# sloisel/MultiGridBarrier.jl

Hardware: AMD Instinct MI355X
Metric: Newton iters/sec + wall-clock to converge, 2D P2 p-Laplace L=9 (higher is better)
Workload: dtype f64

## Files before the change

include/mgbhip.h:

```cpp
#ifndef MGBHIP_H
#define MGBHIP_H

#include <stdint.h>

#ifdef __cplusplus
extern "C" {
#endif

#define MGBHIP_OK 0
#define MGBHIP_ERR_INVALID 1
#define MGBHIP_ERR_HIP 2
#define MGBHIP_ERR_NOT_SPD 3
#define MGBHIP_ERR_NONFINITE 4
#define MGBHIP_ERR_CONVERGENCE 5

#define MGBHIP_MAX_PIECES 4
#define MGBHIP_MAX_IDX 10
#define MGBHIP_MAX_LIN 4
#define MGBHIP_MAX_ND 13
#define MGBHIP_MAX_NU 4
#define MGBHIP_MAX_OPS 8

#define MGBHIP_KIND_EP 1
#define MGBHIP_KIND_LINEAR 2
// ... 64 lines not shown
    int (*early_stop_fn)(const double* z, double t, void* user);
    void* user;
} mgbhip_options;

typedef struct {
    int32_t k;
    int32_t L;
    int32_t failure_code;
    double t_final, t_elapsed;
    double solve_seconds;
    int64_t newton_iterations;
    int64_t f0_evals, f1_evals, f2_evals, factorizations;
    int32_t cap_steps;
    int64_t* its;
    double* ts;
    double* kappas;
    double* times;
    double* c_dot_Dz;
} mgbhip_core_result;

int mgbhip_create(mgbhip_ctx** ctx, int device_id, void* hip_stream );
int mgbhip_destroy(mgbhip_ctx* ctx);
const char* mgbhip_last_error(void);
const char* mgbhip_version(void);

int mgbhip_problem_create(mgbhip_ctx* ctx, const mgbhip_problem_desc* desc,
                          mgbhip_problem* share, mgbhip_problem** out);
int mgbhip_problem_destroy(mgbhip_problem* prob);
int mgbhip_problem_set_box(mgbhip_problem* prob, double b, double R);
int mgbhip_problem_set_barrier_weights(mgbhip_problem* prob, const double* bw );
int64_t mgbhip_level_size(const mgbhip_problem* prob, int32_t level);

int mgbhip_f0(mgbhip_problem* prob, int32_t level, const double* s, const double* c,
              const double* z0, double* value);
int mgbhip_f1(mgbhip_problem* prob, int32_t level, const double* s, const double* c,
              const double* z0, double* grad );
int mgbhip_f2(mgbhip_problem* prob, int32_t level, const double* s, const double* c,
              const double* z0, double* values );
int mgbhip_hessian_pattern(mgbhip_problem* prob, int32_t level, int64_t* nnz,
                           const int32_t** rowptr, const int32_t** colidx);
int mgbhip_solve(mgbhip_problem* prob, int32_t level, const double* g, double* x);
int mgbhip_set_hessian(mgbhip_problem* prob, int32_t level, const double* values );
int mgbhip_solve_newton(mgbhip_problem* prob, int32_t level, const double* g, double* x, double* lambda2);
typedef int (*mgbhip_allreduce_fn)(void* user, double* buf, int64_t count, int32_t op, int32_t on_device);
int mgbhip_problem_set_sharding(mgbhip_problem* prob, int32_t level, int64_t n_iface,
                                const int32_t* iface_cols, const double* own_mask );
int mgbhip_problem_set_collective(mgbhip_problem* prob, mgbhip_allreduce_fn allreduce, void* user,
                                  int32_t accepts_device_ptr);
int mgbhip_newton_direction(mgbhip_problem* prob, int32_t level, const double* s, const double* c,
                            const double* z0, double* x, double* lambda2, int32_t* condensed);
int mgbhip_node_barrier(mgbhip_problem* prob, const double* z, double* F , double* Dz );
int mgbhip_node_slack(mgbhip_problem* prob, const double* z, double* slack );

int mgbhip_mgb_core(mgbhip_problem* prob, double* z , const double* c ,
                    const mgbhip_options* opt, mgbhip_core_result* res);
int mgbhip_matched_t(mgbhip_problem* prob, const double* z, const double* c, double t_default,
                     double* t_out);
void mgbhip_default_options(mgbhip_options* opt, int64_t n_nodes);

typedef struct mgbhip_vec mgbhip_vec;
int mgbhip_vec_alloc(mgbhip_ctx* ctx, int64_t len, mgbhip_vec** out);
int mgbhip_vec_free(mgbhip_vec* v);
int64_t mgbhip_vec_len(const mgbhip_vec* v);
int mgbhip_vec_upload(mgbhip_vec* v, const double* host, int64_t len);
int mgbhip_vec_download(const mgbhip_vec* v, double* host, int64_t len);
int mgbhip_vec_fill(mgbhip_vec* v, double value);
int mgbhip_vec_copy(mgbhip_vec* dst, const mgbhip_vec* src);
int mgbhip_vec_axpy(double alpha, const mgbhip_vec* x, mgbhip_vec* y);
int mgbhip_vec_scale(double alpha, mgbhip_vec* x);
int mgbhip_vec_dot(const mgbhip_vec* a, const mgbhip_vec* b, double* out);
int mgbhip_vec_norm(const mgbhip_vec* a, double* out);
int mgbhip_vec_isfinite(const mgbhip_vec* a, int32_t* all_finite);
int mgbhip_f0_d(mgbhip_problem* prob, int32_t level, const mgbhip_vec* s, const mgbhip_vec* c,
                const mgbhip_vec* z0, double* value);
int mgbhip_f1_d(mgbhip_problem* prob, int32_t level, const mgbhip_vec* s, const mgbhip_vec* c,
                const mgbhip_vec* z0, mgbhip_vec* grad);
int mgbhip_f2_d(mgbhip_problem* prob, int32_t level, const mgbhip_vec* s, const mgbhip_vec* c,
                const mgbhip_vec* z0);
int mgbhip_solve_d(mgbhip_problem* prob, int32_t level, const mgbhip_vec* g, mgbhip_vec* x);
int mgbhip_prolong_add(mgbhip_problem* prob, int32_t level, const mgbhip_vec* s, mgbhip_vec* z);

int mgbhip_stage_ms(mgbhip_problem* prob, const char* stage, double* total_ms, int64_t* launches);
int mgbhip_reset_stage_timers(mgbhip_problem* prob, int enable);
int mgbhip_solver_stats(mgbhip_problem* prob, int32_t level, double* out8);
int mgbhip_solver_chain(mgbhip_problem* prob, int32_t level, double* out8);
enum { MGBHIP_PROJ_NONE = 0, MGBHIP_PROJ_LOOP = 1, MGBHIP_PROJ_STAGED = 2, MGBHIP_PROJ_MFMA = 3, MGBHIP_PROJ_ACCUMULATE = 4 };
int mgbhip_level_plan(mgbhip_problem* prob, int32_t level, int32_t* out16);
enum { MGBHIP_LAUNCH_ROW = 16 };
enum { MGBHIP_ASM_NONE = 0, MGBHIP_ASM_GATHER = 1, MGBHIP_ASM_COLUMNS = 2 };
enum { MGBHIP_B0_NA = 0, MGBHIP_B0_GATHER = 1, MGBHIP_B0_DIAG0 = 2, MGBHIP_B0_STEP0 = 3 };
enum { MGBHIP_BWD_NA = 0, MGBHIP_BWD_K8 = 1, MGBHIP_BWD_K16 = 2, MGBHIP_BWD_GENERAL = 3 };
int64_t mgbhip_solver_launches(mgbhip_problem* prob, int32_t level, int32_t* out, int64_t cap);

#define MGBHIP_INTERP_FEM1D 1
#define MGBHIP_INTERP_QK 2
#define MGBHIP_INTERP_P1 3
#define MGBHIP_INTERP_P2 4
#define MGBHIP_INTERP_SPECTRAL1D 5
#define MGBHIP_INTERP_SPECTRAL2D 6
int mgbhip_interpolate(mgbhip_ctx* ctx, int32_t family, int32_t d, int32_t k, int32_t p, int64_t N,
                       const double* x, const double* table, int32_t ncomp, const double* z, int64_t M,
                       const double* pts, double* out, int32_t* elem);
int mgbhip_interpolate_grad(mgbhip_ctx* ctx, int32_t family, int32_t d, int32_t k, int32_t p, int64_t N,
                            const double* x, const double* table, int32_t ncomp, const double* z, int64_t M,
                            const double* pts, double* out ,
                            double* grad , int32_t* elem );

typedef struct mgbhip_locator mgbhip_locator;
int mgbhip_locator_create(mgbhip_ctx* ctx, int32_t family, int32_t d, int32_t k, int32_t p, int64_t N,
                          const double* x, const double* table, int64_t M, const double* pts,
                          mgbhip_locator** out);
int mgbhip_locator_elements(const mgbhip_locator* loc, int32_t* elem );
int mgbhip_locator_evaluate(mgbhip_locator* loc, int32_t ncomp, const double* z ,
                            double* out ,
                            double* grad );
int mgbhip_locator_destroy(mgbhip_locator* loc);

typedef struct mgbhip_contour mgbhip_contour;
int mgbhip_contour_create(mgbhip_ctx* ctx, int32_t family, int32_t d, int32_t k, int32_t p, int64_t N,
                          const double* x, const double* table, int32_t nfield , const double* fields,
                          int32_t nlevels, const double* levels, int32_t refine,
                          mgbhip_contour** out, int64_t* nsimplices);
int mgbhip_contour_fetch(const mgbhip_contour* c, double* points, int32_t* level, int32_t* element,
                         double* carried );
int mgbhip_contour_destroy(mgbhip_contour* c);

int mgbhip_contour_create_embedded(mgbhip_ctx* ctx, int32_t family, int32_t d, int32_t e, int32_t k, int32_t p,
                                   int64_t N, const double* x , const double* table,
                                   int32_t nfield , const double* fields, int32_t nlevels,
                                   const double* levels, int32_t refine, mgbhip_contour** out, int64_t* nsimplices);

typedef struct mgbhip_tessellation mgbhip_tessellation;
int mgbhip_tessellate_create(mgbhip_ctx* ctx, int32_t family, int32_t d, int32_t e, int32_t k, int32_t p, int64_t N,
                             const double* x , const double* table, int32_t nfield ,
                             const double* fields, int32_t refine, mgbhip_tessellation** out, int64_t* ntriangles);
int mgbhip_tessellate_fetch(const mgbhip_tessellation* t, double* points, int32_t* element,
                            double* values );
int mgbhip_tessellate_destroy(mgbhip_tessellation* t);

typedef struct mgbhip_raycast mgbhip_raycast;
int mgbhip_raycast_create(mgbhip_ctx* ctx, int32_t family, int32_t d, int32_t k, int32_t p, int64_t N,
                          const double* x, const double* table, int64_t R, const double* origin, const double* dir,
                          const double* box, double step, double t_min, double t_max,
                          mgbhip_raycast** out, int64_t* nsamples);
int mgbhip_raycast_offsets(const mgbhip_raycast* rc, int64_t* offsets );
int mgbhip_raycast_samples(const mgbhip_raycast* rc, double* pts );
int mgbhip_raycast_lengths(const mgbhip_raycast* rc, double* step , double* length );
int mgbhip_raycast_integrate(mgbhip_raycast* rc, int32_t ncomp, const double* z ,
                             double* out );
int mgbhip_raycast_render(mgbhip_raycast* rc, const double* u , int32_t K, const double* transfer ,
                          double lo, double hi, double* out );
int mgbhip_raycast_destroy(mgbhip_raycast* rc);
int mgbhip_raycast_render_layers(mgbhip_raycast* rc, const double* u , int32_t K,
                                 const double* transfer , double lo, double hi, int32_t nhits,
                                 const double* t_hit , const double* layer ,
                                 double* out );

typedef struct mgbhip_surface mgbhip_surface;
int mgbhip_surface_create(mgbhip_ctx* ctx, int64_t T, const double* points , mgbhip_surface** out);
int mgbhip_surface_trace(mgbhip_surface* s, int64_t R, const double* origin, const double* dir, double t_min,
                         double t_max, int32_t K, double* t, int32_t* tri, double* u, double* v );
int mgbhip_surface_shade(mgbhip_surface* s, int64_t R, int32_t K, const double* dir, const int32_t* tri,
                         const double* u, const double* v, const double* values , int32_t Kt,
                         const double* table , double lo, double hi, double ambient,
                         double* layer );
int mgbhip_surface_destroy(mgbhip_surface* s);
// ... 46 lines not shown
```

multigridbarrier.jl_amd/csrc/api.cpp:

```cpp
#include <chrono>
#include <cmath>
#include <cstring>
#include <algorithm>
#include <limits>
#include <memory>
#include <string>

#include "contour.hpp"
#include "figure.hpp"
#include "interpolate.hpp"
#include "problem.hpp"
#include "raycast.hpp"
#include "stream.hpp"
#include "surface.hpp"
#include "tubes.hpp"

using namespace mgbhip;

mgbhip_problem* problem_create(mgbhip_ctx* ctx, const mgbhip_problem_desc* d, mgbhip_problem* share);
int core_run(mgbhip_problem* P, double* z, const double* c, const mgbhip_options* opt, mgbhip_core_result* res);
int matched_t_run(mgbhip_problem* P, const double* z, const double* c, double t_default, double* t_out);

#ifdef MGB_STEP_PROBE
namespace mgbhip { void mf_debug_probe(long long* out64); }
#endif

static thread_local std::string g_last_error;

struct DeviceGuard {
    int prev = -1, dev = -1;
    explicit DeviceGuard(int d) : dev(d) {
        if (dev < 0) return;
        if (hipGetDevice(&prev) != hipSuccess) prev = -1;
        if (prev != dev) MGB_HIP_CHECK(hipSetDevice(dev));
    }
    ~DeviceGuard() {
        if (dev >= 0 && prev >= 0 && prev != dev) (void)hipSetDevice(prev);
    }
};
static int dev_of(const mgbhip_ctx* c) { return c ? c->device : -1; }
static int dev_of(const mgbhip_problem* p) { return (p && p->ctx) ? p->ctx->device : -1; }
static int dev_of(const mgbhip_vec* v) { return (v && v->ctx) ? v->ctx->device : -1; }

struct mgbhip_locator {
    mgbhip_ctx* ctx = nullptr;
    Locator loc;
};
static int dev_of(const mgbhip_locator* l) { return (l && l->ctx) ? l->ctx->device : -1; }

struct mgbhip_contour {
    mgbhip_ctx* ctx = nullptr;
    Contour con;
};
static int dev_of(const mgbhip_contour* c) { return (c && c->ctx) ? c->ctx->device : -1; }

struct mgbhip_tessellation {
    mgbhip_ctx* ctx = nullptr;
    Tessellation tes;
};
static int dev_of(const mgbhip_tessellation* t) { return (t && t->ctx) ? t->ctx->device : -1; }

struct mgbhip_raycast {
    mgbhip_ctx* ctx = nullptr;
    RayCaster rc;
};
static int dev_of(const mgbhip_raycast* r) { return (r && r->ctx) ? r->ctx->device : -1; }

struct mgbhip_surface {
    mgbhip_ctx* ctx = nullptr;
    Surface sf;
};
static int dev_of(const mgbhip_surface* s) { return (s && s->ctx) ? s->ctx->device : -1; }

struct mgbhip_tubes {
    mgbhip_ctx* ctx = nullptr;
    Tubes tb;
};
static int dev_of(const mgbhip_tubes* s) { return (s && s->ctx) ? s->ctx->device : -1; }

struct mgbhip_stream {
    mgbhip_ctx* ctx = nullptr;
    StreamTracer tr;
};
static int dev_of(const mgbhip_stream* s) { return (s && s->ctx) ? s->ctx->device : -1; }

struct mgbhip_figure {
    mgbhip_ctx* ctx = nullptr;
    Figure fig;
};
static int dev_of(const mgbhip_figure* f) { return (f && f->ctx) ? f->ctx->device : -1; }

#define MGB_API_BEGIN try {
#define MGB_API_BEGIN_ON(h) try { DeviceGuard _guard(dev_of(h));
#define MGB_API_END                                   \
    }                                                 \
    catch (const InvalidArgument& e) {                \
        g_last_error = e.what();                      \
        return MGBHIP_ERR_INVALID;                    \
    }                                                 \
    catch (const HipError& e) {                       \
        g_last_error = e.what();                      \
        return MGBHIP_ERR_HIP;                        \
    }                                                 \
    catch (const std::exception& e) {                 \
// ... 476 lines not shown

int mgbhip_prolong_add(mgbhip_problem* P, int32_t level, const mgbhip_vec* s, mgbhip_vec* z) {
    MGB_API_BEGIN_ON(P)
    check_level(P, level);
    MGB_REQUIRE(s && z && s->ctx == P->ctx && z->ctx == P->ctx, "bad vector");
    const Level& Lv = P->levels[level];
    MGB_REQUIRE(s->len == Lv.m && z->len == Lv.rows, "prolong_add: length mismatch");
    launch_csr_matvec(Lv.rows, Lv.Rptr.p, Lv.Rcol.p, Lv.Rval.p, s->buf.p, z->buf.p, true, false, P->stream());
    P->touch();
    return MGBHIP_OK;
    MGB_API_END
}

static int node_map(mgbhip_problem* P, const double* z, double* F, double* Dz, int mode) {
    MGB_REQUIRE(P && z && F, "null argument");
    hipStream_t st = P->stream();
    P->d_z0.upload(z, (size_t)P->nu * P->n, st);
    ElemParams E = P->base_params(-1, nullptr, P->d_z0.p, nullptr);
    if (Dz) {
        P->d_nodeDz.ensure((size_t)P->n * P->nD);
        E.out_Dz = P->d_nodeDz.p;
    }
    launch_elem(E, mode, st);
    P->d_nodeF.download(F, (size_t)P->n, st);
    if (Dz) P->d_nodeDz.download(Dz, (size_t)P->n * P->nD, st);
    MGB_HIP_CHECK(hipStreamSynchronize(st));
    return MGBHIP_OK;
}

int mgbhip_node_barrier(mgbhip_problem* P, const double* z, double* F, double* Dz) {
    MGB_API_BEGIN_ON(P)
    return node_map(P, z, F, Dz, MODE_NODE_F);
    MGB_API_END
}

int mgbhip_node_slack(mgbhip_problem* P, const double* z, double* slack) {
    MGB_API_BEGIN_ON(P)
    return node_map(P, z, slack, nullptr, MODE_NODE_SLACK);
    MGB_API_END
}

void mgbhip_default_options(mgbhip_options* o, int64_t n_nodes) {
    const double eps = std::numeric_limits<double>::epsilon();
    o->tol = std::sqrt(eps);
    o->t = 0.1;
    o->kappa = 10.0;
    o->maxit = 10000;
    o->max_newton = (int32_t)std::ceil(std::log2(-std::log2(eps)) + 2);
    o->ls_beta = 0.5;
    o->ls_c1 = 0.1;
    o->line_search = 0;
    o->stop_lambda_tol = 0.25 / std::sqrt((double)n_nodes);
    o->stop_theta = 0.9;
    o->finalize = 1;
    o->finalize_theta = 0.9;
    o->early_stop = 0;
    o->stopping_criterion = nullptr;
    o->early_stop_fn = nullptr;
    o->user = nullptr;
}

int mgbhip_mgb_core(mgbhip_problem* P, double* z, const double* c, const mgbhip_options* opt, mgbhip_core_result* res) {
    MGB_API_BEGIN_ON(P)
    MGB_REQUIRE(P && z && c && opt && res, "null argument");
    MGB_REQUIRE(opt->tol > 0 && opt->t > 0 && opt->kappa > 1 && opt->maxit >= 1 && opt->max_newton >= 1, "bad options");
    int rc = core_run(P, z, c, opt, res);
    if (rc == MGBHIP_ERR_CONVERGENCE)
        g_last_error = res->failure_code == 2 ? "Convergence failure in mgb_solve: iteration_limit"
                                              : "Convergence failure in mgb_solve: stall";
    return rc;
    MGB_API_END
}

int mgbhip_matched_t(mgbhip_problem* P, const double* z, const double* c, double t_default, double* t_out) {
    MGB_API_BEGIN_ON(P)
    MGB_REQUIRE(P && z && c && t_out, "null argument");
    return matched_t_run(P, z, c, t_default, t_out);
    MGB_API_END
}

int mgbhip_stage_ms(mgbhip_problem* P, const char* stage, double* total_ms, int64_t* launches) {
    MGB_API_BEGIN_ON(P)
    MGB_REQUIRE(P && stage, "null argument");
    P->ctx->timers.collect();
    auto it = P->ctx->timers.recs.find(stage);
    if (total_ms) *total_ms = it == P->ctx->timers.recs.end() ? 0.0 : it->second.ms;
    if (launches) *launches = it == P->ctx->timers.recs.end() ? 0 : it->second.launches;
    return MGBHIP_OK;
    MGB_API_END
}

int mgbhip_solver_stats(mgbhip_problem* P, int32_t level, double* out) {
    MGB_API_BEGIN
    check_level(P, level);
    MGB_REQUIRE(out != nullptr, "null argument");
    const Level& L = P->levels[level];
    const MfPlan& pl = L.solver.plan;
    out[0] = (double)pl.fronts.size();
    out[1] = (double)pl.max_m;
    out[2] = (double)pl.arena_doubles;
    out[3] = (double)pl.factor_flops;
    out[4] = (double)pl.peeled;
    out[5] = pl.level_ptr.empty() ? 0.0 : (double)(pl.level_ptr.size() - 1);
    out[6] = (double)L.nnz;
    out[7] = (double)L.m;
    return MGBHIP_OK;
    MGB_API_END
}

int mgbhip_solver_chain(mgbhip_problem* P, int32_t level, double* out) {
    MGB_API_BEGIN
    check_level(P, level);
    MGB_REQUIRE(out != nullptr, "null argument");
    MGB_REQUIRE(P->levels[level].solver.analyzed, "mgbhip_solver_chain: the level has not been factored yet");
    P->levels[level].solver.chain_stats(out);
    return MGBHIP_OK;
    MGB_API_END
}

static_assert(MGBHIP_LAUNCH_ROW == mgbhip::MF_LAUNCH_ROW && MGBHIP_ASM_GATHER == mgbhip::MF_ASM_GATHER &&
              MGBHIP_ASM_COLUMNS == mgbhip::MF_ASM_COLS && MGBHIP_B0_GATHER == mgbhip::MF_B0_GATHER &&
              MGBHIP_B0_DIAG0 == mgbhip::MF_B0_DIAG0 && MGBHIP_B0_STEP0 == mgbhip::MF_B0_STEP0 && MGBHIP_BWD_K8 == mgbhip::MF_BWD_K8 &&
              MGBHIP_BWD_K16 == mgbhip::MF_BWD_K16 && MGBHIP_BWD_GENERAL == mgbhip::MF_BWD_GENERAL, "mgbhip.h and mf_launch_plan.hpp disagree");

int64_t mgbhip_solver_launches(mgbhip_problem* P, int32_t level, int32_t* out, int64_t cap) {
    int64_t count = 0;
    const int rc = [&]() -> int {
        MGB_API_BEGIN
        check_level(P, level);
        MGB_REQUIRE(cap >= 0 && (out != nullptr || cap == 0), "bad output buffer");
        MGB_REQUIRE(P->levels[level].solver.analyzed, "mgbhip_solver_launches: the level has not been factored yet");
        count = P->levels[level].solver.launches(out, cap);
        return MGBHIP_OK;
        MGB_API_END
    }();
    return rc == MGBHIP_OK ? count : -(int64_t)rc;
}

#ifdef MGB_STEP_PROBE
int mgbhip_debug_probe(long long* out64) { (void)hipDeviceSynchronize(); mgbhip::mf_debug_probe(out64); return 0; }
#endif

int mgbhip_reset_stage_timers(mgbhip_problem* P, int enable) {
    MGB_API_BEGIN_ON(P)
    MGB_REQUIRE(P, "null argument");
    P->ctx->timers.reset(enable != 0);
    return MGBHIP_OK;
    MGB_API_END
}

static void interpolate_check_geometry(InterpIn& in) {
    const int32_t family = in.family, d = in.d, k = in.k, p = in.p;
    const int64_t N = in.N;
    const double* x = in.x;
    const bool fem = family >= MGBHIP_INTERP_FEM1D && family <= MGBHIP_INTERP_P2;
    if (fem) {
        MGB_REQUIRE(x != nullptr && in.table != nullptr, "interpolate: FEM families need node coordinates and a table");
        MGB_REQUIRE(k >= 1 && k <= INTERP_MAX_DEGREE, "interpolate: element degree out of range");
    }
    switch (family) {
        case MGBHIP_INTERP_FEM1D:
            MGB_REQUIRE(d == 1 && p == k + 1, "interpolate: fem1d needs d = 1, p = k + 1");
            in.table_len = k + 1;
            for (int64_t e = 1; e < N && in.sorted; ++e) in.sorted = x[e * p] >= x[(e - 1) * p];
            break;
        case MGBHIP_INTERP_QK: {
            MGB_REQUIRE(d == 2 || d == 3, "interpolate: Q_k needs d = 2 or 3");
            int64_t s = 1;
            for (int a = 0; a < d; ++a) s *= k + 1;
            MGB_REQUIRE(p == s, "interpolate: Q_k needs p = (k + 1)^d");
            in.table_len = k + 1;
            break;
        }
        case MGBHIP_INTERP_P1:
        case MGBHIP_INTERP_P2:
            MGB_REQUIRE(d == 2, "interpolate: triangles need d = 2");
            MGB_REQUIRE(family == MGBHIP_INTERP_P1 ? p == 3 : (p == 6 || p == 7), "interpolate: bad nodes per triangle");
            in.table_len = (int64_t)p * 10;
            break;
        case MGBHIP_INTERP_SPECTRAL1D:
            MGB_REQUIRE(d == 1 && N == 1 && k >= 0 && p == k + 1, "interpolate: spectral1d needs d = 1, N = 1, p = n");
            in.table = nullptr;
            break;
        case MGBHIP_INTERP_SPECTRAL2D:
            MGB_REQUIRE(d == 2 && N == 1 && k >= 0 && (int64_t)p == (int64_t)(k + 1) * (k + 1),
                        "interpolate: spectral2d needs d = 2, N = 1, p = n^2");
            in.table = nullptr;
            break;
        default:
            throw InvalidArgument("interpolate: unknown family");
    }
    MGB_REQUIRE((int64_t)p * N < (int64_t)INT32_MAX && in.M < (int64_t)INT32_MAX, "interpolate: sizes exceed 32-bit indexing");
}

static void interpolate_checked(mgbhip_ctx* ctx, int32_t family, int32_t d, int32_t k, int32_t p, int64_t N,
                                const double* x, const double* table, int32_t ncomp, const double* z, int64_t M,
                                const double* pts, double* out, double* grad, int32_t* elem) {
    const bool need_out = grad == nullptr;
    MGB_REQUIRE(ctx != nullptr, "null context");
    MGB_REQUIRE(N > 0, "interpolate: no elements (N = 0)");
    MGB_REQUIRE(M >= 0 && ncomp >= 1 && p >= 1, "interpolate: bad sizes");
    MGB_REQUIRE(z != nullptr && (M == 0 || (pts != nullptr && (out != nullptr || !need_out))), "null argument");
    InterpIn in;
    in.family = family; in.d = d; in.k = k; in.p = p; in.N = N; in.ncomp = ncomp; in.M = M;
    in.x = x; in.table = table; in.z = z; in.pts = pts; in.out = out; in.grad = grad; in.elem = elem;
    interpolate_check_geometry(in);
    MGB_REQUIRE(M * ncomp * (grad ? d : 1) < (int64_t)INT32_MAX, "interpolate: sizes exceed 32-bit indexing");
    interpolate_run(in, ctx->stream);
}

int mgbhip_interpolate(mgbhip_ctx* ctx, int32_t family, int32_t d, int32_t k, int32_t p, int64_t N, const double* x,
                       const double* table, int32_t ncomp, const double* z, int64_t M, const double* pts, double* out,
                       int32_t* elem) {
    MGB_API_BEGIN_ON(ctx)
    interpolate_checked(ctx, family, d, k, p, N, x, table, ncomp, z, M, pts, out, nullptr, elem);
    return MGBHIP_OK;
    MGB_API_END
}

int mgbhip_interpolate_grad(mgbhip_ctx* ctx, int32_t family, int32_t d, int32_t k, int32_t p, int64_t N,
                            const double* x, const double* table, int32_t ncomp, const double* z, int64_t M,
                            const double* pts, double* out, double* grad, int32_t* elem) {
    MGB_API_BEGIN_ON(ctx)
    MGB_REQUIRE(grad != nullptr, "interpolate_grad: null gradient array");
    interpolate_checked(ctx, family, d, k, p, N, x, table, ncomp, z, M, pts, out, grad, elem);
    return MGBHIP_OK;
    MGB_API_END
}

// ... 576 lines not shown
```

multigridbarrier.jl_amd/csrc/driver.cpp:

```cpp
#include <chrono>
#include <cstdio>
#include <cstdlib>
#include <cmath>
#include <cstring>
#include <functional>
#include <limits>

#include "problem.hpp"

using namespace mgbhip;

namespace {

constexpr double EPS = std::numeric_limits<double>::epsilon();

bool debug_on() {
    static const bool on = [] { const char* e = getenv("MGBHIP_DEBUG"); return e && e[0] == '1'; }();
    return on;
}
#define DBG(...) do { if (debug_on()) { fprintf(stderr, __VA_ARGS__); } } while (0)

struct Stop {
    double lambda_tol;
    double theta;
    int (*fn)(double, double, double, double, double, double, void*) = nullptr;
    void* user = nullptr;
    bool operator()(double ymin, double ynext, double gmin, double gnorm_next, double ndecmin, double ndec) const {
        if (fn) return fn(ymin, ynext, gmin, gnorm_next, ndecmin, ndec, user) != 0;
        const bool exact = (ynext >= ymin) && (gnorm_next >= theta * gmin);
        if (lambda_tol >= 0) return (ndec < lambda_tol) || exact;
        return exact;
    }
};

struct NewtonResult {
    int k = 0;
    bool converged = false;
    double y = 0;
};

struct VecStats { double sumsq, bad; };

VecStats vec_stats(mgbhip_problem* P, int level, const double* d_v, int64_t len) {
    hipStream_t st = P->stream();
    launch_vec_stats(d_v, len, P->d_scratch.p, P->d_scal.p + 2, st, P->own_mask(level));
    P->read_scalars(2, 2);
    if (P->sharded()) P->allreduce_host(P->pin.d + 2, 2, 0);
    return VecStats{P->pin.d[2], P->pin.d[3]};
}

double dev_dot(mgbhip_problem* P, int level, const double* a, const double* b, int64_t len) {
    hipStream_t st = P->stream();
    launch_dot(a, b, len, P->d_scratch.p, P->d_scal.p + 4, st, P->own_mask(level));
    P->read_scalars(4, 1);
    if (P->sharded()) P->allreduce_host(P->pin.d + 4, 1, 0);
    return P->pin.d[4];
}

struct NewtonCtx {
    mgbhip_problem* P;
    int level;
    const double* d_zJ;
    const double* d_c;
    int64_t m;
    double F0(const double* d_s) { return P->eval_f0(level, d_s, d_zJ, d_c); }
    void F1(const double* d_s, double* d_out, double* d_part) { P->eval_f1(level, d_s, d_zJ, d_c, d_out, P->sharded() ? d_part : nullptr); }
    const double* rhs_of_g() const { return P->sharded() ? P->d_gpart.p : P->d_g.p; }
    void F2(const double* d_s) { P->eval_f2(level, d_s, d_zJ, d_c, false, rhs_of_g()); }
};

bool trial_values(NewtonCtx& C, double& ynext, double& gnorm_next, int32_t* moved = nullptr, const double* step = nullptr) {
    mgbhip_problem* P = C.P;
    hipStream_t st = P->stream();
    const bool onfly = step && P->can_fuse_step(C.level);
    if (step) {
        ++P->step_stamp;
        if (!onfly) launch_step(P->d_x.p, P->d_nv.p, *step, P->d_xn.p, C.m, P->d_flag.p, P->step_stamp, st);
        P->touch();
        if (onfly) { P->trial_x = P->d_x.p; P->trial_dir = P->d_nv.p; P->trial_alpha = *step; }
    }
    const bool fused = !P->dense;
    static const bool fuse_restrict = [] { const char* e = getenv("MGBHIP_NO_FUSED_RESTRICT"); return !(e && e[0] == '1'); }();
    P->trial_fuse = mgbhip_problem::TrialFuse();
    if (fused && fuse_restrict) {
        P->trial_fuse.want = true;
        if (onfly) {
            P->trial_fuse.x = P->d_x.p; P->trial_fuse.n = P->d_nv.p; P->trial_fuse.s = *step; P->trial_fuse.xn = P->d_xn.p;
            P->trial_fuse.moved = P->d_flag.p; P->trial_fuse.stamp = P->step_stamp;
        }
    }
    P->eval_f01_launch(C.level, P->d_xn.p, C.d_zJ, C.d_c, P->d_gn.p, P->sharded() ? P->d_gnpart.p : nullptr, fused);
    const bool restrict_fused = P->trial_fuse.done;
    P->trial_fuse.want = false;
    if (onfly) {
        P->trial_x = nullptr; P->trial_dir = nullptr;
        if (!restrict_fused) launch_step(P->d_x.p, P->d_nv.p, *step, P->d_xn.p, C.m, P->d_flag.p, P->step_stamp, st);
    }
    const double seq = P->next_seq();
    launch_trial_finish(P->d_gn.p, C.m, P->d_scratch.p, fused ? P->d_partials.p : nullptr, elem_grid(P->p, P->N), P->d_scal.p,
                        P->d_flag.p, P->pin.dev, st, P->own_mask(C.level), seq, restrict_fused);
    P->wait_results(seq);
    P->pin.i[0] = P->pin.d[4] == (double)P->step_stamp ? 1 : 0;
    if (P->sharded()) {
        P->pin.d[1] = (double)P->pin.i[0];
        P->allreduce_host(P->pin.d, 4, 0);
        P->pin.i[0] = P->pin.d[1] != 0.0 ? 1 : 0;
    }
    if (moved) *moved = P->pin.i[0];
    ynext = P->pin.d[0];
    if (!std::isfinite(ynext)) return false;
    if (P->pin.d[3] != 0.0 || !std::isfinite(P->pin.d[2])) return false;
    gnorm_next = std::sqrt(P->pin.d[2]);
    return true;
}

bool linesearch_backtracking(NewtonCtx& C, const mgbhip_options& opt, double y, double inc, double& ynext,
                             double& gnorm_next) {
    mgbhip_problem* P = C.P;
    hipStream_t st = P->stream();
    double s = 1.0;
    bool have = false;
    while (s > 0.0) {
        double yn, gn;
        int32_t moved = 0;
        if (trial_values(C, yn, gn, &moved, &s)) {
            have = true;
            ynext = yn;
            gnorm_next = gn;
            const bool stalled = (moved == 0);
            if (stalled || yn <= y - opt.ls_c1 * inc * s) return true;
        }
        s *= opt.ls_beta;
    }
    return have;
}

bool linesearch_illinois(NewtonCtx& C, const mgbhip_options& opt, double inc, double& ynext, double& gnorm_next) {
    mgbhip_problem* P = C.P;
    hipStream_t st = P->stream();
    struct Reject {};
    auto phi = [&](double sigma) -> double {
        launch_step(P->d_x.p, P->d_nv.p, sigma, P->d_xn.p, C.m, P->d_flag.p, ++P->step_stamp, st);
        P->touch();
        const double f = C.F0(P->d_xn.p);
        if (!std::isfinite(f)) throw Reject();
        C.F1(P->d_xn.p, P->d_gn.p, P->d_gnpart.p);
        const double v = dev_dot(P, C.level, P->d_gn.p, P->d_nv.p, C.m);
        if (!std::isfinite(v)) throw Reject();
        return v;
    };
    double s = 1.0;
    bool have = false;
    while (s > 0.0) {
        try {
            double a = 0.0, b = s, fa = inc, fb = phi(s), root = b;
            bool done = false;
            if (fa == 0) { root = a; done = true; }
            else if (fa * fb >= 0) { root = b; done = true; }
            for (int it = 0; it < 10000 && !done; ++it) {
                const double c = (a * fb - b * fa) / (fb - fa);
                const double fc = phi(c);
                if (c <= std::fmin(a, b) || c >= std::fmax(a, b) || fc * fa == 0 || fc * fb == 0) { root = c; done = true; break; }
                if (fb * fc < 0) { a = b; fa = fb; } else { fa /= 2; }
                b = c; fb = fc;
            }
            if (!done) throw Reject();
            launch_step(P->d_x.p, P->d_nv.p, root, P->d_xn.p, C.m, P->d_flag.p, ++P->step_stamp, st);
        P->touch();
            double yn, gn;
            if (!trial_values(C, yn, gn)) throw Reject();
            ynext = yn;
            gnorm_next = gn;
            return true;
        } catch (Reject&) {
        }
        s *= opt.ls_beta;
    }
    return have;
}

NewtonResult newton(NewtonCtx& C, const mgbhip_options& opt, const Stop& stop, int maxit) {
    mgbhip_problem* P = C.P;
    hipStream_t st = P->stream();
    NewtonResult R;
    P->d_x.zero(st, (size_t)C.m);
    P->touch();
    double y = C.F0(P->d_x.p);
    if (!std::isfinite(y)) throw InvalidArgument("newton: initial objective value is not finite");
    double ymin = y;
    if (P->sharded()) { P->d_gpart.ensure((size_t)C.m); P->d_gnpart.ensure((size_t)C.m); }
    C.F1(P->d_x.p, P->d_g.p, P->d_gpart.p);
    VecStats gs = vec_stats(P, C.level, P->d_g.p, C.m);
    if (gs.bad != 0.0 || !std::isfinite(gs.sumsq)) throw InvalidArgument("newton: initial gradient has non-finite entries");
    double gnorm = std::sqrt(gs.sumsq);
    double gmin = gnorm;
    double incmin = INFINITY;
    int k = 0;
    bool converged = false;
    Level& L = P->levels[C.level];
    struct RobustReset {
        MfSolver& s;
        ~RobustReset() { s.robust = false; }
    } robust_reset{L.solver};
    while (k < maxit && !converged) {
        ++k;
        C.F2(P->d_x.p);
        auto t0 = std::chrono::steady_clock::now();
        int fstatus = MGBHIP_OK;
        int leaf_flag = 0;
        for (int attempt = 0; attempt < 2; ++attempt) {
            P->factor(C.level, C.rhs_of_g());
            P->trisolve_carried(C.level, P->d_nv.p);
            const double seq = P->next_seq();
            launch_dir_finish(P->d_nv.p, P->d_g.p, C.m, P->d_scratch.p, P->d_scal.p, L.solver.status_flags_rw(), P->pin.dev, st,
                              P->own_mask(C.level), seq);
            L.solver.flags_cleared();
            P->wait_results(seq);
            P->pin.i[1] = P->pin.d[5] != 0.0 ? 1 : 0;
            leaf_flag |= P->pin.d[6] != 0.0 ? 1 : 0;
            P->pin.i[2] = leaf_flag;
            fstatus = MfSolver::status_from(P->pin.i + 1, L.solver.factored_condensed);
            if (P->sharded()) {
                P->pin.d[5] = fstatus != MGBHIP_OK ? 1.0 : 0.0;
                P->allreduce_host(P->pin.d + 2, 4, 0);
                fstatus = P->pin.d[5] != 0.0 ? MGBHIP_ERR_NOT_SPD : MGBHIP_OK;
            }
            const bool at_floor = std::fabs(P->pin.d[4]) <= EPS * std::fmax(std::fabs(y), 1.0);
            const bool suspicious = fstatus != MGBHIP_OK || P->pin.d[3] != 0.0 || !std::isfinite(P->pin.d[2]) ||
                                    (!(P->pin.d[4] > 0) && !at_floor);
            if (!suspicious || attempt == 1 || !L.solver.has_inverse_path() || L.solver.robust) break;
            DBG("newton[lev %d] k=%d: direction rejected (status %d, lambda^2=%.3e): refactoring with the substitution kernels\n",
                C.level, k, fstatus, P->pin.d[4]);
            L.solver.robust = true;
            L.factored = false;
        }
        if (fstatus != MGBHIP_OK && P->lu_fallback(C.level, P->d_g.p, P->d_nv.p)) {
            DBG("newton[lev %d] k=%d: LDL' met a zero pivot; direction from the pivoted LU fallback\n", C.level, k);
            launch_dir_finish(P->d_nv.p, P->d_g.p, C.m, P->d_scratch.p, P->d_scal.p, L.solver.status_flags_rw(), P->pin.dev, st,
                              P->own_mask(C.level));
            L.solver.flags_cleared();
            MGB_HIP_CHECK(hipStreamSynchronize(st));
            fstatus = MGBHIP_OK;
        }
        P->cnt.solve_seconds += std::chrono::duration<double>(std::chrono::steady_clock::now() - t0).count();
        if (fstatus != MGBHIP_OK) {
            DBG("newton[lev %d] k=%d: Cholesky met a non-positive pivot (y=%.17g |g|=%.6e)\n", C.level, k, y, gnorm);
            converged = false;
            break;
        }
        if (P->pin.d[3] != 0.0 || !std::isfinite(P->pin.d[2])) throw InvalidArgument("newton: Newton direction has non-finite entries");
        const double inc = P->pin.d[4];
        DBG("newton[lev %d] k=%d y=%.17g |g|=%.6e lambda^2=%.6e\n", C.level, k, y, gnorm, inc);
        if (inc <= 0) {
            converged = std::fabs(inc) <= EPS * std::fmax(std::fabs(y), 1.0);
            break;
        }
        double ynext = y, gnorm_next = gnorm;
        bool moved = (opt.line_search == 1) ? linesearch_illinois(C, opt, inc, ynext, gnorm_next)
                                            : linesearch_backtracking(C, opt, y, inc, ynext, gnorm_next);
        if (!moved) {
            ynext = y;
            gnorm_next = gnorm;
// ... 248 lines not shown
```

multigridbarrier.jl_amd/csrc/kernels.hip:

```cpp
#include <hip/hip_runtime.h>

#include <algorithm>
#include <mutex>

#include "kernels.hpp"
#include "dense.hpp"

namespace mgbhip {

namespace {

template <int CTRL>
__device__ __forceinline__ double dpp_mov_f64(double v) {
    const long long b = __double_as_longlong(v);
    const int lo = __builtin_amdgcn_mov_dpp((int)(b & 0xffffffffll), CTRL, 0xF, 0xF, true);
    const int hi = __builtin_amdgcn_mov_dpp((int)(b >> 32), CTRL, 0xF, 0xF, true);
    return __longlong_as_double(((long long)hi << 32) | (unsigned int)lo);
}
__device__ __forceinline__ double z_at(const ElemParams& P, int64_t i) {
    double v = P.z0[i];
    if (P.zsel) {
        const int32_t c = P.zsel[i];
        if (c >= 0) v += P.zx ? __builtin_fma(-P.zalpha, P.zx[c], P.zs[c]) : P.zs[c];
        if (P.zout) P.zout[i] = v;
// ... 661 lines not shown
                for (int q = 0; q < P; ++q) acc -= Xus[q * P + i] * t[q];
                up[i] = acc;
            }
#pragma unroll
            for (int q = 0; q < P; ++q) bj -= Xbeta[q] * t[q];
            if (j == PB) {
                bj -= Pm.leaf_g[ld.interior];
#pragma unroll
                for (int q = 0; q < P; ++q) corner -= Xbeta[q] * Xbeta[q] * Xinv[q];
#pragma unroll
                for (int i = 0; i < P; ++i) Xc[i] = up[i];
                Xs[0] = bj;
                Xs[1] = up[PB];
            }
        }
        __builtin_amdgcn_fence(__ATOMIC_RELEASE, "wavefront");
        __builtin_amdgcn_wave_barrier();
        __builtin_amdgcn_fence(__ATOMIC_ACQUIRE, "wavefront");
        {
            const int m = (int)(ld.packed & 15u);
            const bool pk = Pm.leaf_packed != 0;
            int pos[P];
#pragma unroll
            for (int i = 0; i < P; ++i) pos[i] = (int)((ld.packed >> (4 + 4 * i)) & 15u);
            double d7 = 1.0, bb = 0.0, inv7 = 1.0, f = 0.0, xc[P];
#pragma unroll
            for (int i = 0; i < P; ++i) xc[i] = 0.0;
            if (active) {
                d7 = Xs[1];
                bb = Xs[0];
                inv7 = 1.0 / d7;
#pragma unroll
                for (int i = 0; i < P; ++i) xc[i] = Xc[i];
                f = (j < PB) ? xc[j] * inv7 : 0.0;
                bad = bad || (j == PB && ((d7 == 0.0) || !isfinite(d7)));
            }
            double* Fg = Pm.leaf_arena + ld.F_off;
            double* S = Fg;
            if (pk) {
                __syncthreads();
                S = sh + (size_t)el * 120;
            }
            auto at = [&](int rr, int cc) -> int { return pk ? cc * m - (cc * (cc - 1)) / 2 + (rr - cc) : rr + cc * m; };
            if (active) {
                S[at(j, j)] = ssj;
#pragma unroll
                for (int rr = 0; rr < P; ++rr)
                    if (rr > j) S[at(rr, j)] = 0.0;
                S[at(P, j)] = usc[PB] * inv;
#pragma unroll
                for (int i = 0; i < PB; ++i)
                    if (pos[i] != 15) S[at(pos[i], j)] = usc[i] * inv;
                S[at(m - 1, j)] = beta * inv;
                if (j == PB) {
                    S[at(P, P)] = d7;
#pragma unroll
                    for (int i = 0; i < PB; ++i)
                        if (pos[i] != 15) S[at(pos[i], P)] = xc[i] * inv7;
                    S[at(m - 1, P)] = bb * inv7;
                    S[at(m - 1, m - 1)] = corner - bb * bb * inv7;
                } else if (pos[j] != 15) {
#pragma unroll
                    for (int i = 0; i < PB; ++i)
                        if (pos[i] != 15 && pos[i] >= pos[j]) S[at(pos[i], pos[j])] = up[i] - xc[i] * f;
                    S[at(m - 1, pos[j])] = bj - bb * f;
                }
            }
            if (pk) {
                __builtin_amdgcn_fence(__ATOMIC_RELEASE, "wavefront");
                __builtin_amdgcn_wave_barrier();
                __builtin_amdgcn_fence(__ATOMIC_ACQUIRE, "wavefront");
                if (e < Pm.N) {
                    const LeafDesc l2 = Pm.leaf_desc[e];
                    const int mm = (int)(l2.packed & 15u);
                    double* dstF = Pm.leaf_arena + l2.F_off;
                    for (int t = r; t < mm * (mm + 1) / 2; t += G) dstF[t] = S[t];
                }
            }
        }
        if (bad) atomicOr(Pm.leaf_status, 1);
    }
}

template <int NY, int P, class Sig>
__global__ __launch_bounds__(256) void elem_f01_fast(const ElemParams Pm) {
    constexpr int G = (P <= 2) ? 2 : (P <= 4) ? 4 : (P <= 8) ? 8 : (P <= 16) ? 16 : (P <= 32) ? 32 : 64;
    constexpr int EPB = 256 / G;
    constexpr int PP = P * P;
    extern __shared__ double sh[];
    const int tid = threadIdx.x;
    const int el = tid / G;
    const int r = tid % G;
    const int nu = Sig::rt ? Pm.nu : 2;
    auto DST = [&](int k) -> int { return Sig::rt ? Pm.D_state[k] : Sig::state(k); };
    auto DSG = [&](int k) -> int { return Sig::rt ? Pm.D_stage[k] : Sig::stage(k); };
    const int64_t e0 = (int64_t)blockIdx.x * EPB;
    const int64_t e = e0 + el;
    const bool active = (e < Pm.N) && (r < P);
    const int64_t n = Pm.n;
    const int64_t node = e * P + r;

    double* zl = sh;
    double* opL = zl + 256 * nu;
    double* YL = opL + (size_t)Pm.nstage * EPB * PP;
    {
        int64_t lim = (Pm.N - e0) * PP;
        if (lim > (int64_t)EPB * PP) lim = (int64_t)EPB * PP;
        constexpr int NIT = (EPB * PP + 255) / 256;
        for (int o = 0; o < Pm.nstage; ++o) {
            const double* src = Pm.stage_ptr[o] + e0 * PP;
            double* dst = opL + (size_t)o * EPB * PP;
            double v[NIT];
#pragma unroll
            for (int u = 0; u < NIT; ++u) {
                const int i = tid + 256 * u;
                v[u] = i < lim ? src[i] : 0.0;
            }
#pragma unroll
            for (int u = 0; u < NIT; ++u) {
                const int i = tid + 256 * u;
                if (i < lim) dst[i] = v[u];
            }
        }
    }
    double ck[NY];
    double wv = 0.0, bwv = 0.0;
    if (active) {
        for (int a = 0; a < nu; ++a) zl[(el * nu + a) * G + r] = z_at(Pm, (int64_t)a * n + node);
#pragma unroll
        for (int k = 0; k < NY; ++k) ck[k] = Pm.c[node + n * k];
        wv = Pm.w[node];
        bwv = Pm.bw ? Pm.bw[node] : 0.0;
    }
    __syncthreads();
    const double* opE = opL + (size_t)el * PP;
    auto OP = [&](int k, int rr, int cc) -> double { return opE[(size_t)DSG(k) * EPB * PP + cc * P + rr]; };
    double y[NY];
#pragma unroll
    for (int k = 0; k < NY; ++k) {
        double v = 0.0;
        if (active) {
            const double* za = zl + (el * nu + DST(k)) * G;
            if (DSG(k) < 0) v = za[r];
            else {
#pragma unroll
                for (int cc = 0; cc < P; ++cc) v += OP(k, r, cc) * za[cc];
            }
        }
        y[k] = v;
    }
    double val = 0.0;
    if (active) {
        double F0v, F, g[NY], H[NY * NY];
        cone_eval<NY, 0>(Pm.cone, node, n, y, F0v, g, H);
        cone_eval<NY, 1>(Pm.cone, node, n, y, F, g, H);
        const double bar = Pm.bw ? ((bwv == 0.0) ? 0.0 : bwv * F0v) : Pm.invn * F0v;
        double lin = 0.0;
#pragma unroll
        for (int k = 0; k < NY; ++k) {
            lin += ck[k] * y[k];
            const double sc = Pm.bw ? ((bwv == 0.0) ? 0.0 : bwv * g[k]) : Pm.invn * g[k];
            YL[(el * NY + k) * G + r] = sc + wv * ck[k];
        }
        val = bar + wv * lin;
    }
    __syncthreads();
    if (active) {
        const int i = r;
        for (int a = 0; a < nu; ++a) {
            double acc = 0.0;
#pragma unroll
            for (int k = 0; k < NY; ++k) {
                if (DST(k) != a) continue;
                const double* Yk = YL + (el * NY + k) * G;
                if (DSG(k) < 0) {
                    acc += Yk[i];
                } else {
#pragma unroll
                    for (int rr = 0; rr < P; ++rr) acc += OP(k, rr, i) * Yk[rr];
                }
            }
            Pm.out_ret[(int64_t)a * n + node] = acc;
        }
    }
    __syncthreads();
    const double tot = block_sum_256(val, sh);
    if (tid == 0) Pm.out_partial[blockIdx.x] = tot;
}

struct DSum {
    double s = 0.0, c = 0.0;
    __device__ __forceinline__ void add(double x) {
#ifdef MGB_PLAIN_SUMS
        s += x;
        return;
#endif
        const double t = s + x;
        const double bp = t - s;
        c += (s - (t - bp)) + (x - bp);
        s = t;
    }
    __device__ __forceinline__ void merge(double s2, double c2) { add(s2); c += c2; }
    __device__ __forceinline__ double value() const { return s + c; }
};
__device__ __forceinline__ void dsum_wave_reduce(DSum& a) {
    for (int off = 32; off > 0; off >>= 1) {
        const double s2 = __shfl_down(a.s, off, 64), c2 = __shfl_down(a.c, off, 64);
        a.merge(s2, c2);
    }
}


__global__ __launch_bounds__(256) void reduce_partials_kernel(const double* __restrict__ partials, int64_t count,
                                                              double* __restrict__ out) {
    __shared__ double red[256];
    const int tid = threadIdx.x;
    double s = 0.0;
    for (int64_t i = tid; i < count; i += 256) s += partials[i];
    red[tid] = s;
    __syncthreads();
    for (int off = 128; off > 0; off >>= 1) {
        if (tid < off) red[tid] += red[tid + off];
        __syncthreads();
    }
    if (tid == 0) out[0] = red[0];
}

template <int MODE>
__global__ __launch_bounds__(256) void block_reduce_kernel(const double* __restrict__ a, const double* __restrict__ b,
                                                           int64_t n, double* __restrict__ partials,
                                                           const double* __restrict__ mask) {
    __shared__ double red[256];
    __shared__ double red2[256];
    const int tid = threadIdx.x;
    double s = 0.0, bad = 0.0;
    for (int64_t i = (int64_t)blockIdx.x * 256 + tid; i < n; i += (int64_t)gridDim.x * 256) {
        const double v = a[i];
        const double w = mask ? mask[i] : 1.0;
        if (MODE == 0) s += mask ? w * (v * b[i]) : v * b[i];
        else {
            s += mask ? w * (v * v) : v * v;
            bad += isfinite(v) ? 0.0 : 1.0;
        }
    }
    red[tid] = s;
    red2[tid] = bad;
    __syncthreads();
    for (int off = 128; off > 0; off >>= 1) {
        if (tid < off) { red[tid] += red[tid + off]; red2[tid] += red2[tid + off]; }
        __syncthreads();
    }
    if (tid == 0) {
        partials[blockIdx.x] = red[0];
        if (MODE == 1) partials[gridDim.x + blockIdx.x] = red2[0];
    }
}

__global__ __launch_bounds__(256) void restrict_trial_kernel(int64_t rows, const int32_t* __restrict__ ptr, const int32_t* __restrict__ col,
                                                             const double* __restrict__ val, const double* __restrict__ ret,
                                                             double* __restrict__ g, double* __restrict__ partials,
                                                             const double* __restrict__ x, const double* __restrict__ nn, double s,
                                                             double* __restrict__ xn, int32_t* __restrict__ moved, int32_t stamp) {
    __shared__ double red[256];
    __shared__ double red2[256];
    __shared__ int any_moved;
    const int tid = threadIdx.x;
    if (tid == 0) any_moved = 0;
    __syncthreads();
    double ss = 0.0, bad = 0.0;
    bool m = false;
    for (int64_t i = (int64_t)blockIdx.x * 256 + tid; i < rows; i += (int64_t)gridDim.x * 256) {
        double acc = 0.0;
        for (int32_t q = ptr[i]; q < ptr[i + 1]; ++q) acc += val[q] * ret[col[q]];
        g[i] = acc;
        ss += acc * acc;
        bad += isfinite(acc) ? 0.0 : 1.0;
        if (xn) {
            const double xi = x[i];
            const double v = __builtin_fma(-s, nn[i], xi);
            xn[i] = v;
            m = m || (v != xi);
        }
    }
    red[tid] = ss;
    red2[tid] = bad;
    if (m) any_moved = 1;
    __syncthreads();
    for (int off = 128; off > 0; off >>= 1) {
        if (tid < off) { red[tid] += red[tid + off]; red2[tid] += red2[tid + off]; }
        __syncthreads();
    }
    if (tid == 0) {
        partials[blockIdx.x] = red[0];
        partials[gridDim.x + blockIdx.x] = red2[0];
        if (any_moved) *moved = stamp;
    }
}

__global__ __launch_bounds__(256) void dir_stats_kernel(const double* __restrict__ v, const double* __restrict__ g, int64_t n,
                                                        double* __restrict__ partials, const double* __restrict__ mask) {
    __shared__ double red[3][256];
    const int tid = threadIdx.x;
    double s = 0.0, bad = 0.0, d = 0.0;
    for (int64_t i = (int64_t)blockIdx.x * 256 + tid; i < n; i += (int64_t)gridDim.x * 256) {
        const double x = v[i];
        const double w = mask ? mask[i] : 1.0;
        s += mask ? w * (x * x) : x * x;
        bad += isfinite(x) ? 0.0 : 1.0;
        d += mask ? w * (g[i] * x) : g[i] * x;
    }
    red[0][tid] = s; red[1][tid] = bad; red[2][tid] = d;
    __syncthreads();
    for (int off = 128; off > 0; off >>= 1) {
        if (tid < off) {
            red[0][tid] += red[0][tid + off];
            red[1][tid] += red[1][tid + off];
            red[2][tid] += red[2][tid + off];
        }
        __syncthreads();
    }
    if (tid == 0) {
        partials[blockIdx.x] = red[0][0];
        partials[gridDim.x + blockIdx.x] = red[1][0];
        partials[2 * gridDim.x + blockIdx.x] = red[2][0];
    }
}

struct FinishJob { const double* src; int64_t count; int32_t out; };
struct FinishParams {
    FinishJob job[4];
    int32_t njobs;
    double* out;
    int32_t* ints;
    int32_t nints, ints_out, reset;
    double* host;
    int32_t host_lo, host_n;
    double seq;
};
__global__ __launch_bounds__(256) void finish_kernel(const FinishParams P) {
    __shared__ double red[256];
    __shared__ double res[16];
    const int tid = threadIdx.x;
    if (tid < P.nints) {
        res[P.ints_out + tid] = (double)P.ints[tid];
        if (P.reset) P.ints[tid] = 0;
    }
    for (int o = 0; o < P.njobs; ++o) {
        const double* __restrict__ src = P.job[o].src;
        const int64_t cnt = P.job[o].count;
        double s = 0.0;
        for (int64_t i = tid; i < cnt; i += 256) s += src[i];
        red[tid] = s;
        __syncthreads();
        for (int off = 128; off > 0; off >>= 1) {
            if (tid < off) red[tid] += red[tid + off];
            __syncthreads();
        }
        if (tid == 0) res[P.job[o].out] = red[0];
        __syncthreads();
    }
    __syncthreads();
    if (tid < 16) {
        bool mine = false;
        for (int o = 0; o < P.njobs; ++o) mine = mine || (P.job[o].out == tid);
        if (tid >= P.ints_out && tid < P.ints_out + P.nints) mine = true;
        if (mine) P.out[tid] = res[tid];
        if (P.host && tid >= P.host_lo && tid < P.host_lo + P.host_n) P.host[tid] = mine ? res[tid] : P.out[tid];
    }
    if (P.host && P.seq != 0.0) {
        __threadfence_system();
        __syncthreads();
        if (tid == 0) {
            __hip_atomic_store(P.host + 15, P.seq, __ATOMIC_RELEASE, __HIP_MEMORY_SCOPE_SYSTEM);
        }
    }
}


template <bool ADD>
__global__ __launch_bounds__(256) void csr_matvec_row_kernel(int64_t rows, const int32_t* __restrict__ ptr,
                                                             const int32_t* __restrict__ col,
                                                             const double* __restrict__ val,
                                                             const double* __restrict__ x, double* __restrict__ y) {
    const int64_t i = (int64_t)blockIdx.x * 256 + threadIdx.x;
    if (i >= rows) return;
    double s = 0.0;
    for (int32_t q = ptr[i]; q < ptr[i + 1]; ++q) s += val[q] * x[col[q]];
    y[i] = ADD ? y[i] + s : s;
}

template <bool ADD>
__global__ __launch_bounds__(256) void csr_matvec_wave_kernel(int64_t rows, const int32_t* __restrict__ ptr,
                                                              const int32_t* __restrict__ col,
                                                              const double* __restrict__ val,
                                                              const double* __restrict__ x, double* __restrict__ y) {
    const int lane = threadIdx.x & 63;
    const int64_t i = (int64_t)blockIdx.x * 4 + (threadIdx.x >> 6);
    if (i >= rows) return;
    DSum a;
    for (int32_t q = ptr[i] + lane; q < ptr[i + 1]; q += 64) a.add(val[q] * x[col[q]]);
    dsum_wave_reduce(a);
    if (lane == 0) y[i] = ADD ? y[i] + a.value() : a.value();
}

constexpr int CHUNK = 4096;
__global__ __launch_bounds__(256) void csr_matvec_chunk_kernel(const int32_t* __restrict__ ptr,
                                                               const int32_t* __restrict__ col,
                                                               const double* __restrict__ val,
                                                               const double* __restrict__ x,
                                                               double* __restrict__ partial, int nchunk) {
    __shared__ double red[256];
    const int row = blockIdx.y, ch = blockIdx.x, tid = threadIdx.x;
    const int32_t q0 = ptr[row] + ch * CHUNK;
    const int32_t q1 = min(ptr[row + 1], q0 + CHUNK);
    __shared__ double redc[256];
    DSum a;
    for (int32_t q = q0 + tid; q < q1; q += 256) a.add(val[q] * x[col[q]]);
    red[tid] = a.s;
    redc[tid] = a.c;
    __syncthreads();
    for (int off = 128; off > 0; off >>= 1) {
        if (tid < off) {
            DSum b;
            b.s = red[tid]; b.c = redc[tid];
            b.merge(red[tid + off], redc[tid + off]);
            red[tid] = b.s; redc[tid] = b.c;
        }
        __syncthreads();
    }
    if (tid == 0) {
        partial[2 * ((int64_t)row * nchunk + ch)] = red[0];
        partial[2 * ((int64_t)row * nchunk + ch) + 1] = redc[0];
    }
}

__global__ __launch_bounds__(256) void csr_matvec_chunk_sum_kernel(int64_t rows, const double* __restrict__ partial,
                                                                   int nchunk, double* __restrict__ y) {
    const int lane = threadIdx.x & 63;
    const int64_t i = (int64_t)blockIdx.x * 4 + (threadIdx.x >> 6);
    if (i >= rows) return;
    DSum a;
    for (int c = lane; c < nchunk; c += 64) a.merge(partial[2 * (i * nchunk + c)], partial[2 * (i * nchunk + c) + 1]);
    dsum_wave_reduce(a);
    if (lane == 0) y[i] = a.value();
}

__global__ __launch_bounds__(256) void prolong_kernel(int64_t rows, const int32_t* __restrict__ ptr,
                                                      const int32_t* __restrict__ col,
                                                      const double* __restrict__ val,
                                                      const double* __restrict__ s, const double* __restrict__ z0,
                                                      double* __restrict__ zfull) {
    const int64_t i = (int64_t)blockIdx.x * 256 + threadIdx.x;
    if (i >= rows) return;
    double v = z0[i];
    for (int32_t q = ptr[i]; q < ptr[i + 1]; ++q) v += val[q] * s[col[q]];
    zfull[i] = v;
}

__global__ __launch_bounds__(256) void step_kernel(const double* __restrict__ x, const double* __restrict__ nn,
                                                   double s, double* __restrict__ xn, int64_t len,
                                                   int32_t* __restrict__ moved, int32_t stamp) {
    const int64_t i = (int64_t)blockIdx.x * 256 + threadIdx.x;
    bool m = false;
    if (i < len) {
        const double xi = x[i];
        const double v = __builtin_fma(-s, nn[i], xi);
        xn[i] = v;
        m = (v != xi);
    }
    __shared__ int any_moved;
    if (threadIdx.x == 0) any_moved = 0;
    __syncthreads();
    if (m) any_moved = 1;
    __syncthreads();
    if (threadIdx.x == 0 && any_moved) *moved = stamp;
}

__global__ __launch_bounds__(256) void scale_copy_kernel(const double* __restrict__ src, double alpha,
                                                         double* __restrict__ dst, int64_t len) {
    const int64_t i = (int64_t)blockIdx.x * 256 + threadIdx.x;
    if (i < len) dst[i] = alpha * src[i];
}

__global__ __launch_bounds__(256) void border_tail_kernel(const double* __restrict__ g, double* __restrict__ tail, int64_t m) {
    const int64_t i = (int64_t)blockIdx.x * 256 + threadIdx.x;
    if (i < m) tail[i] = -1.0 * g[i];
    else if (i == m) tail[i] = -1.0;
}

__global__ __launch_bounds__(256) void axpy_kernel(double alpha, const double* __restrict__ x,
                                                   double* __restrict__ y, int64_t len) {
    const int64_t i = (int64_t)blockIdx.x * 256 + threadIdx.x;
    if (i < len) y[i] += alpha * x[i];
}

__global__ __launch_bounds__(256) void fill_kernel(double value, double* __restrict__ y, int64_t len) {
    const int64_t i = (int64_t)blockIdx.x * 256 + threadIdx.x;
    if (i < len) y[i] = value;
}


__global__ __launch_bounds__(256) void gather_assemble_kernel(int64_t nq, const int32_t* __restrict__ qmap,
                                                              const int32_t* __restrict__ cptr,
                                                              const int32_t* __restrict__ cidx,
                                                              const double* __restrict__ slab,
                                                              double* __restrict__ Hval) {
    const int64_t qi = (int64_t)blockIdx.x * 256 + threadIdx.x;
    if (qi >= nq) return;
    const int64_t q = qmap ? qmap[qi] : qi;
    const int32_t beg = cptr[q], end = cptr[q + 1];
    if (end - beg <= 4) {
        double s = 0.0;
        for (int32_t t = beg; t < end; ++t) s += slab[cidx ? cidx[t] : t];
        Hval[q] = s;
        return;
    }
    DSum a;
    for (int32_t t = beg; t < end; ++t) a.add(slab[cidx ? cidx[t] : t]);
    Hval[q] = a.value();
}

__global__ __launch_bounds__(256) void gather_shared_kernel(int64_t nshared, const int32_t* __restrict__ sh_q,
                                                            const int32_t* __restrict__ cptr, const int32_t* __restrict__ cidx,
                                                            const double* __restrict__ slab, double* __restrict__ out) {
    const int64_t i = (int64_t)blockIdx.x * 256 + threadIdx.x;
    if (i >= nshared) return;
    const int32_t q = sh_q[i];
    const int32_t beg = cptr[q], end = cptr[q + 1];
    if (end - beg <= 4) {
        double a[4];
#pragma unroll
        for (int u = 0; u < 4; ++u) a[u] = (beg + u < end) ? slab[cidx[beg + u]] : 0.0;
        double s = 0.0;
#pragma unroll
        for (int u = 0; u < 4; ++u)
            if (beg + u < end) s += a[u];
        out[i] = s;
        return;
    }
    DSum acc;
    for (int32_t t = beg; t < end; t += 4) {
        double a[4];
#pragma unroll
        for (int u = 0; u < 4; ++u) a[u] = (t + u < end) ? slab[cidx[t + u]] : 0.0;
#pragma unroll
        for (int u = 0; u < 4; ++u)
            if (t + u < end) acc.add(a[u]);
    }
    out[i] = acc.value();
}

// ... 436 lines not shown
    (void)hipFuncSetAttribute((const void*)elem_kernel<NY, MODE_F01>, hipFuncAttributeMaxDynamicSharedMemorySize, big);
    (void)hipGetLastError();
}

}

int elem_group(int p) {
    int g = 1;
    while (g < p) g <<= 1;
    return g < 2 ? 2 : g;
}

int64_t elem_grid(int p, int64_t N) {
    if (p > 64) return dense_grid((int64_t)p * N);
    const int epb = 256 / elem_group(p);
    return (N + epb - 1) / epb;
}

size_t elem_lds_bytes(const ElemParams& P, int mode) {
    const int G = elem_group(P.p);
    const int EPB = 256 / G;
    size_t d = 256 * (size_t)P.nu + (size_t)P.nstage * EPB * P.p * P.p;
    if (mode == MODE_F1 || mode == MODE_F01) d += 256 * (size_t)P.nD;
    if (mode == MODE_F2) d += 256 * (size_t)(P.nD * (P.nD + 1) / 2);
    if (d < 256) d = 256;
    return d * sizeof(double);
}

template <int NY>
static bool is_default_signature(const ElemParams& P) {
    if (P.nu != 2 || P.nD != NY || P.ymask != (((1 << NY) - 1) & ~1)) return false;
    for (int k = 0; k < NY; ++k) {
        if (P.D_state[k] != (k == NY - 1 ? 1 : 0)) return false;
        if (P.D_stage[k] != ((k == 0 || k == NY - 1) ? -1 : k - 1)) return false;
    }
    return true;
}

template <int NY, int PN>
static bool try_f2_fast(const ElemParams& P, hipStream_t st) {
    if (P.nD != NY || P.p != PN) return false;
    for (int k = 0; k < NY; ++k)
        if (P.D_stage[k] == -2) return false;
    const int G = elem_group(PN);
    const int EPB = 256 / G;
    const size_t lds = (256 * (size_t)P.nu + (size_t)P.nstage * EPB * PN * PN + (size_t)EPB * (NY * (NY + 1) / 2) * G) *
                       sizeof(double);
    if (lds > 160 * 1024) return false;
    static bool attr = [] {
        (void)hipFuncSetAttribute((const void*)elem_f2_fast<NY, PN, SigRuntime>, hipFuncAttributeMaxDynamicSharedMemorySize, 160 * 1024);
        (void)hipFuncSetAttribute((const void*)elem_f2_fast<NY, PN, SigDefault<NY>>, hipFuncAttributeMaxDynamicSharedMemorySize, 160 * 1024);
        (void)hipGetLastError();
        return true;
    }();
    (void)attr;
    if (is_default_signature<NY>(P))
        hipLaunchKernelGGL((elem_f2_fast<NY, PN, SigDefault<NY>>), dim3((unsigned)elem_grid(PN, P.N)), dim3(256), lds, st, P);
    else
        hipLaunchKernelGGL((elem_f2_fast<NY, PN, SigRuntime>), dim3((unsigned)elem_grid(PN, P.N)), dim3(256), lds, st, P);
    return true;
}

bool launch_elem_f2_condense(const ElemParams& P, hipStream_t st) {
    constexpr int NY = 4, PN = 7;
    if (P.wide || P.nD != NY || P.p != PN || P.nu != 2 || P.nstage != 2 || !is_default_signature<NY>(P)) return false;
    for (int k = 0; k < NY; ++k)
        if (P.D_stage[k] == -2) return false;
    MGB_REQUIRE(P.leaf_desc && P.leaf_arena && P.leaf_g && P.leaf_status, "condensing f2: leaf arguments missing");
    const int G = elem_group(PN);
    const int EPB = 256 / G;
    const size_t lds = (256 * (size_t)P.nu + (size_t)P.nstage * EPB * PN * PN + (size_t)EPB * (NY * (NY + 1) / 2) * G) * sizeof(double);
    static bool attr = [] {
        (void)hipFuncSetAttribute((const void*)elem_f2_fast<NY, PN, SigDefault<NY>, true>, hipFuncAttributeMaxDynamicSharedMemorySize, 160 * 1024);
        (void)hipGetLastError();
        return true;
    }();
    (void)attr;
    hipLaunchKernelGGL((elem_f2_fast<NY, PN, SigDefault<NY>, true>), dim3((unsigned)elem_grid(PN, P.N)), dim3(256), lds, st, P);
    MGB_HIP_CHECK(hipGetLastError());
    return true;
}

template <int NY, int PN>
static bool try_f01_fast(const ElemParams& P, hipStream_t st) {
    if (P.nD != NY || P.p != PN) return false;
    for (int k = 0; k < NY; ++k)
        if (P.D_stage[k] == -2) return false;
    const int G = elem_group(PN);
    const int EPB = 256 / G;
    size_t lds = (256 * (size_t)P.nu + (size_t)P.nstage * EPB * PN * PN + (size_t)EPB * NY * G) * sizeof(double);
    if (lds < 256 * sizeof(double)) lds = 256 * sizeof(double);
    if (lds > 160 * 1024) return false;
    static bool attr = [] {
        (void)hipFuncSetAttribute((const void*)elem_f01_fast<NY, PN, SigRuntime>, hipFuncAttributeMaxDynamicSharedMemorySize, 160 * 1024);
        (void)hipFuncSetAttribute((const void*)elem_f01_fast<NY, PN, SigDefault<NY>>, hipFuncAttributeMaxDynamicSharedMemorySize, 160 * 1024);
        (void)hipGetLastError();
        return true;
    }();
    (void)attr;
    if (is_default_signature<NY>(P))
        hipLaunchKernelGGL((elem_f01_fast<NY, PN, SigDefault<NY>>), dim3((unsigned)elem_grid(PN, P.N)), dim3(256), lds, st, P);
    else
        hipLaunchKernelGGL((elem_f01_fast<NY, PN, SigRuntime>), dim3((unsigned)elem_grid(PN, P.N)), dim3(256), lds, st, P);
    return true;
}

size_t wide_lds_bytes(int p, int nu, int nD, int nstage, int mode) {
    const int G = elem_group(p);
    const int threads = (mode == MODE_F2) ? WIDE_F2_THREADS : 256;
    const int EPB = threads / G;
    size_t d = (size_t)threads * nu + (size_t)nstage * EPB * p * p;
    if (mode == MODE_F1 || mode == MODE_F01) d += (size_t)threads * nD;
    if (mode == MODE_F2) d += (size_t)threads * (nD * (nD + 1) / 2);
    if (d < 256) d = 256;
    return d * sizeof(double);
}

static void launch_elem_wide(const ElemParams& P, int mode, hipStream_t st) {
    static std::once_flag once;
    std::call_once(once, [] {
        const int big = 160 * 1024;
        (void)hipFuncSetAttribute((const void*)elem_wide_kernel<MODE_F0>, hipFuncAttributeMaxDynamicSharedMemorySize, big);
        (void)hipFuncSetAttribute((const void*)elem_wide_kernel<MODE_F1>, hipFuncAttributeMaxDynamicSharedMemorySize, big);
        (void)hipFuncSetAttribute((const void*)elem_wide_kernel<MODE_F2>, hipFuncAttributeMaxDynamicSharedMemorySize, big);
        (void)hipFuncSetAttribute((const void*)elem_wide_kernel<MODE_NODE_F>, hipFuncAttributeMaxDynamicSharedMemorySize, big);
        (void)hipFuncSetAttribute((const void*)elem_wide_kernel<MODE_NODE_SLACK>, hipFuncAttributeMaxDynamicSharedMemorySize, big);
        (void)hipFuncSetAttribute((const void*)elem_wide_kernel<MODE_F01>, hipFuncAttributeMaxDynamicSharedMemorySize, big);
        (void)hipGetLastError();
    });
    const int G = elem_group(P.p);
    int lgG = 0;
    while ((1 << lgG) < G) ++lgG;
    const int threads = (mode == MODE_F2) ? WIDE_F2_THREADS : 256;
    const int EPB = threads / G;
    const dim3 grid((unsigned)((P.N + EPB - 1) / EPB)), blk((unsigned)threads);
    const size_t lds = wide_lds_bytes(P.p, P.nu, P.nD, P.nstage, mode);
    MGB_REQUIRE(lds <= 160 * 1024, "wide element kernel LDS budget exceeded");
    switch (mode) {
        case MODE_F0: hipLaunchKernelGGL((elem_wide_kernel<MODE_F0>), grid, blk, lds, st, P, lgG); break;
        case MODE_F1: hipLaunchKernelGGL((elem_wide_kernel<MODE_F1>), grid, blk, lds, st, P, lgG); break;
        case MODE_F2: hipLaunchKernelGGL((elem_wide_kernel<MODE_F2>), grid, blk, lds, st, P, lgG); break;
        case MODE_NODE_F: hipLaunchKernelGGL((elem_wide_kernel<MODE_NODE_F>), grid, blk, lds, st, P, lgG); break;
        case MODE_NODE_SLACK: hipLaunchKernelGGL((elem_wide_kernel<MODE_NODE_SLACK>), grid, blk, lds, st, P, lgG); break;
        case MODE_F01: hipLaunchKernelGGL((elem_wide_kernel<MODE_F01>), grid, blk, lds, st, P, lgG); break;
        default: throw InvalidArgument("launch_elem: bad mode");
    }
    MGB_HIP_CHECK(hipGetLastError());
}

void launch_elem(const ElemParams& P, int mode, hipStream_t st) {
    if (P.p > 64) {
        launch_dense_eval(P, mode, st);
        return;
    }
    MGB_REQUIRE(P.p >= 1 && P.p <= 64, "element kernels support 1 <= p <= 64 nodes per element");
    MGB_REQUIRE(P.nD >= 1 && P.nD <= MGBHIP_MAX_ND, "nD out of range");
    if (P.wide) {
        launch_elem_wide(P, mode, st);
        return;
    }
    MGB_REQUIRE(P.nD <= 10, "narrow element kernels: nD out of range");
    if (mode == MODE_F2) {
        if (try_f2_fast<4, 7>(P, st) || try_f2_fast<3, 2>(P, st) || try_f2_fast<5, 8>(P, st) ||
            try_f2_fast<4, 6>(P, st) || try_f2_fast<7, 7>(P, st) || try_f2_fast<6, 2>(P, st) ||
            try_f2_fast<8, 8>(P, st) || try_f2_fast<7, 6>(P, st)) {
            MGB_HIP_CHECK(hipGetLastError());
            return;
        }
    }
    if (mode == MODE_F01) {
        if (try_f01_fast<4, 7>(P, st) || try_f01_fast<3, 2>(P, st) || try_f01_fast<5, 8>(P, st) ||
            try_f01_fast<4, 6>(P, st) || try_f01_fast<7, 7>(P, st) || try_f01_fast<6, 2>(P, st) ||
            try_f01_fast<8, 8>(P, st) || try_f01_fast<7, 6>(P, st)) {
            MGB_HIP_CHECK(hipGetLastError());
            return;
        }
    }
    static std::once_flag once;
    std::call_once(once, [] {
        set_lds_attr<1>(); set_lds_attr<2>(); set_lds_attr<3>(); set_lds_attr<4>();
        set_lds_attr<5>(); set_lds_attr<6>(); set_lds_attr<7>(); set_lds_attr<8>();
        set_lds_attr<9>(); set_lds_attr<10>();
    });
    const int G = elem_group(P.p);
    int lgG = 0;
    while ((1 << lgG) < G) ++lgG;
    const dim3 grid((unsigned)elem_grid(P.p, P.N));
    const size_t lds = elem_lds_bytes(P, mode);
    MGB_REQUIRE(lds <= 160 * 1024, "element kernel LDS budget exceeded");
    switch (P.nD) {
        case 1: launch_elem_ny<1>(P, mode, lgG, grid, lds, st); break;
        case 2: launch_elem_ny<2>(P, mode, lgG, grid, lds, st); break;
        case 3: launch_elem_ny<3>(P, mode, lgG, grid, lds, st); break;
        case 4: launch_elem_ny<4>(P, mode, lgG, grid, lds, st); break;
        case 5: launch_elem_ny<5>(P, mode, lgG, grid, lds, st); break;
        case 6: launch_elem_ny<6>(P, mode, lgG, grid, lds, st); break;
        case 7: launch_elem_ny<7>(P, mode, lgG, grid, lds, st); break;
        case 8: launch_elem_ny<8>(P, mode, lgG, grid, lds, st); break;
        case 9: launch_elem_ny<9>(P, mode, lgG, grid, lds, st); break;
        case 10: launch_elem_ny<10>(P, mode, lgG, grid, lds, st); break;
    }
    MGB_HIP_CHECK(hipGetLastError());
}

void launch_reduce_partials(const double* partials, int64_t count, double* out, hipStream_t st) {
    hipLaunchKernelGGL(reduce_partials_kernel, dim3(1), dim3(256), 0, st, partials, count, out);
    MGB_HIP_CHECK(hipGetLastError());
}


static int reduce_blocks(int64_t n) {
    int64_t b = (n + 255) / 256;
    if (b > 1024) b = 1024;
    if (b < 1) b = 1;
    return (int)b;
}

int64_t reduce_scratch_doubles(int64_t n) { return 3 * (int64_t)reduce_blocks(n); }

__global__ __launch_bounds__(256) void index_gather_kernel(const double* __restrict__ v, const int32_t* __restrict__ idx,
                                                           int64_t cnt, double* __restrict__ out) {
    const int64_t i = (int64_t)blockIdx.x * 256 + threadIdx.x;
    if (i < cnt) out[i] = v[idx[i]];
}
__global__ __launch_bounds__(256) void index_scatter_kernel(const double* __restrict__ in, const int32_t* __restrict__ idx,
                                                            int64_t cnt, double* __restrict__ v) {
    const int64_t i = (int64_t)blockIdx.x * 256 + threadIdx.x;
    if (i < cnt) v[idx[i]] = in[i];
}
void launch_index_gather(const double* v, const int32_t* idx, int64_t cnt, double* out, hipStream_t st) {
    if (cnt == 0) return;
    hipLaunchKernelGGL(index_gather_kernel, dim3((unsigned)((cnt + 255) / 256)), dim3(256), 0, st, v, idx, cnt, out);
    MGB_HIP_CHECK(hipGetLastError());
}
void launch_index_scatter(const double* in, const int32_t* idx, int64_t cnt, double* v, hipStream_t st) {
    if (cnt == 0) return;
    hipLaunchKernelGGL(index_scatter_kernel, dim3((unsigned)((cnt + 255) / 256)), dim3(256), 0, st, in, idx, cnt, v);
    MGB_HIP_CHECK(hipGetLastError());
}

static void launch_finish(const FinishParams& F, hipStream_t st) {
    hipLaunchKernelGGL(finish_kernel, dim3(1), dim3(256), 0, st, F);
    MGB_HIP_CHECK(hipGetLastError());
}

void launch_vec_stats(const double* v, int64_t n, double* scratch, double* stats, hipStream_t st, const double* mask,
                      const int32_t* ints, int nints) {
    const int nb = reduce_blocks(n);
    hipLaunchKernelGGL(block_reduce_kernel<1>, dim3(nb), dim3(256), 0, st, v, (const double*)nullptr, n, scratch, mask);
    FinishParams F{};
    F.job[0] = FinishJob{scratch, nb, 0};
    F.job[1] = FinishJob{scratch + nb, nb, 1};
    F.njobs = 2;
    F.out = stats;
    F.ints = const_cast<int32_t*>(ints); F.nints = nints; F.ints_out = 2; F.reset = 0;
    launch_finish(F, st);
}

void launch_dir_stats(const double* v, const double* g, int64_t n, double* scratch, double* stats3, hipStream_t st,
                      const double* mask, const int32_t* ints, int nints) {
    const int nb = reduce_blocks(n);
    hipLaunchKernelGGL(dir_stats_kernel, dim3(nb), dim3(256), 0, st, v, g, n, scratch, mask);
    FinishParams F{};
    F.job[0] = FinishJob{scratch, nb, 0};
    F.job[1] = FinishJob{scratch + nb, nb, 1};
    F.job[2] = FinishJob{scratch + 2 * nb, nb, 2};
    F.njobs = 3;
    F.out = stats3;
    F.ints = const_cast<int32_t*>(ints); F.nints = nints; F.ints_out = 3; F.reset = 0;
    launch_finish(F, st);
}

__global__ void publish_kernel(const double* __restrict__ src, int n, double* __restrict__ host, double* __restrict__ stamp, double seq) {
    const int tid = threadIdx.x;
    if (tid < n) host[tid] = src[tid];
    __threadfence_system();
    __syncthreads();
    if (tid == 0) __hip_atomic_store(stamp, seq, __ATOMIC_RELEASE, __HIP_MEMORY_SCOPE_SYSTEM);
}

void launch_publish(const double* src, int n, double* host_block, int host_lo, double seq, hipStream_t st) {
    hipLaunchKernelGGL(publish_kernel, dim3(1), dim3(64), 0, st, src, n, host_block + host_lo, host_block + 15, seq);
    MGB_HIP_CHECK(hipGetLastError());
}

void launch_dir_finish(const double* v, const double* g, int64_t n, double* scratch, double* scal, int32_t* status2, double* host,
                       hipStream_t st, const double* mask, double seq) {
    const int nb = reduce_blocks(n);
    hipLaunchKernelGGL(dir_stats_kernel, dim3(nb), dim3(256), 0, st, v, g, n, scratch, mask);
    FinishParams F{};
    F.job[0] = FinishJob{scratch, nb, 2};
    F.job[1] = FinishJob{scratch + nb, nb, 3};
    F.job[2] = FinishJob{scratch + 2 * nb, nb, 4};
    F.njobs = 3;
    F.out = scal;
    F.ints = status2; F.nints = 2; F.ints_out = 5; F.reset = 1;
    F.host = host; F.host_lo = 2; F.host_n = 5;
    F.seq = seq;
    launch_finish(F, st);
}

void launch_trial_finish(const double* g, int64_t n, double* scratch, const double* f0_partials, int64_t f0_count, double* scal,
                         int32_t* moved, double* host, hipStream_t st, const double* mask, double seq, bool partials_ready) {
    const int nb = reduce_blocks(n);
    if (!partials_ready) hipLaunchKernelGGL(block_reduce_kernel<1>, dim3(nb), dim3(256), 0, st, g, (const double*)nullptr, n, scratch, mask);
    FinishParams F{};
    int nj = 0;
    if (f0_partials) F.job[nj++] = FinishJob{f0_partials, f0_count, 0};
    F.job[nj++] = FinishJob{scratch, nb, 2};
    F.job[nj++] = FinishJob{scratch + nb, nb, 3};
    F.njobs = nj;
    F.out = scal;
    F.ints = moved; F.nints = 1; F.ints_out = 4; F.reset = 0;
    F.host = host; F.host_lo = 0; F.host_n = 5;
    F.seq = seq;
    launch_finish(F, st);
}

void launch_dot(const double* a, const double* b, int64_t n, double* scratch, double* out, hipStream_t st, const double* mask) {
    const int nb = reduce_blocks(n);
    hipLaunchKernelGGL(block_reduce_kernel<0>, dim3(nb), dim3(256), 0, st, a, b, n, scratch, mask);
    FinishParams F{};
    F.job[0] = FinishJob{scratch, nb, 0};
    F.njobs = 1;
    F.out = out;
    launch_finish(F, st);
}

void launch_csr_matvec(int64_t rows, const int32_t* ptr, const int32_t* col, const double* val,
                       const double* x, double* y, bool add, bool long_rows, hipStream_t st) {
    if (rows == 0) return;
    if (long_rows) {
        const dim3 grid((unsigned)((rows + 3) / 4));
        if (add) hipLaunchKernelGGL(csr_matvec_wave_kernel<true>, grid, dim3(256), 0, st, rows, ptr, col, val, x, y);
        else hipLaunchKernelGGL(csr_matvec_wave_kernel<false>, grid, dim3(256), 0, st, rows, ptr, col, val, x, y);
    } else {
        const dim3 grid((unsigned)((rows + 255) / 256));
        if (add) hipLaunchKernelGGL(csr_matvec_row_kernel<true>, grid, dim3(256), 0, st, rows, ptr, col, val, x, y);
        else hipLaunchKernelGGL(csr_matvec_row_kernel<false>, grid, dim3(256), 0, st, rows, ptr, col, val, x, y);
    }
    MGB_HIP_CHECK(hipGetLastError());
}

int csr_chunks(int64_t max_row_len) { return (int)((max_row_len + CHUNK - 1) / CHUNK); }

void launch_restrict_trial(int64_t rows, const int32_t* ptr, const int32_t* col, const double* val, const double* ret, double* g,
                            double* scratch, const double* x, const double* nn, double s, double* xn, int32_t* moved, int32_t stamp,
                            hipStream_t st) {
    if (rows == 0) return;
    const int nb = reduce_blocks(rows);
    hipLaunchKernelGGL(restrict_trial_kernel, dim3(nb), dim3(256), 0, st, rows, ptr, col, val, ret, g, scratch, x, nn, s, xn, moved, stamp);
    MGB_HIP_CHECK(hipGetLastError());
}

void launch_csr_matvec_chunked(int64_t rows, const int32_t* ptr, const int32_t* col, const double* val,
                               const double* x, double* y, double* scratch, int nchunk, hipStream_t st) {
    if (rows == 0) return;
    hipLaunchKernelGGL(csr_matvec_chunk_kernel, dim3((unsigned)nchunk, (unsigned)rows), dim3(256), 0, st, ptr, col, val, x,
                       scratch, nchunk);
    hipLaunchKernelGGL(csr_matvec_chunk_sum_kernel, dim3((unsigned)((rows + 3) / 4)), dim3(256), 0, st, rows, scratch,
                       nchunk, y);
    MGB_HIP_CHECK(hipGetLastError());
}

void launch_prolong(int64_t rows, const int32_t* ptr, const int32_t* col, const double* val, const double* s,
                    const double* z0, double* zfull, hipStream_t st) {
    if (rows == 0) return;
    hipLaunchKernelGGL(prolong_kernel, dim3((unsigned)((rows + 255) / 256)), dim3(256), 0, st, rows, ptr, col, val, s,
                       z0, zfull);
    MGB_HIP_CHECK(hipGetLastError());
}

void launch_step(const double* x, const double* n, double s, double* xn, int64_t len, int32_t* moved, int32_t stamp,
                 hipStream_t st) {
    if (len == 0) return;
    hipLaunchKernelGGL(step_kernel, dim3((unsigned)((len + 255) / 256)), dim3(256), 0, st, x, n, s, xn, len, moved, stamp);
    MGB_HIP_CHECK(hipGetLastError());
}

void launch_scale_copy(const double* src, double alpha, double* dst, int64_t len, hipStream_t st) {
    if (len == 0) return;
    hipLaunchKernelGGL(scale_copy_kernel, dim3((unsigned)((len + 255) / 256)), dim3(256), 0, st, src, alpha, dst, len);
    MGB_HIP_CHECK(hipGetLastError());
}

void launch_border_tail(const double* g, double* tail, int64_t m, hipStream_t st) {
    hipLaunchKernelGGL(border_tail_kernel, dim3((unsigned)((m + 1 + 255) / 256)), dim3(256), 0, st, g, tail, m);
    MGB_HIP_CHECK(hipGetLastError());
}

void launch_axpy(double alpha, const double* x, double* y, int64_t len, hipStream_t st) {
    if (len == 0) return;
    hipLaunchKernelGGL(axpy_kernel, dim3((unsigned)((len + 255) / 256)), dim3(256), 0, st, alpha, x, y, len);
    MGB_HIP_CHECK(hipGetLastError());
}

void launch_fill(double value, double* y, int64_t len, hipStream_t st) {
    if (len == 0) return;
    hipLaunchKernelGGL(fill_kernel, dim3((unsigned)((len + 255) / 256)), dim3(256), 0, st, value, y, len);
    MGB_HIP_CHECK(hipGetLastError());
}

void launch_gather_assemble(int64_t nnz, const int32_t* cptr, const int32_t* cidx, const double* slab,
                            double* Hval, bool long_lists, hipStream_t st, int32_t chunk, int32_t nchunk, double* part,
                            const int32_t* qmap, int64_t nq) {
    if (nnz == 0) return;
    if (!qmap) nq = nnz;
    if (nq == 0) return;
    if (long_lists && nchunk > 1) {
        hipLaunchKernelGGL(gather_assemble_chunk_kernel, dim3((unsigned)((nq * nchunk + 3) / 4)), dim3(256), 0, st, nq, qmap, chunk,
                           nchunk, cptr, cidx, slab, part);
        hipLaunchKernelGGL(gather_assemble_chunk_reduce, dim3((unsigned)((nq + 3) / 4)), dim3(256), 0, st, nq, qmap, nchunk, part, Hval);
    } else if (long_lists)
        hipLaunchKernelGGL(gather_assemble_wave_kernel, dim3((unsigned)((nq + 3) / 4)), dim3(256), 0, st, nq, qmap, cptr,
                           cidx, slab, Hval);
    else
        hipLaunchKernelGGL(gather_assemble_kernel, dim3((unsigned)((nq + 255) / 256)), dim3(256), 0, st, nq, qmap, cptr,
                           cidx, slab, Hval);
    MGB_HIP_CHECK(hipGetLastError());
}

void launch_gather_shared(int64_t nshared, const int32_t* sh_q, const int32_t* cptr, const int32_t* cidx, const double* slab,
                          double* out, hipStream_t st) {
    if (nshared == 0) return;
    hipLaunchKernelGGL(gather_shared_kernel, dim3((unsigned)((nshared + 255) / 256)), dim3(256), 0, st, nshared, sh_q, cptr, cidx,
                       slab, out);
    MGB_HIP_CHECK(hipGetLastError());
}

size_t panel_accumulate_lds(int p, int nu, int ctmax) {
    const size_t per_wave = (size_t)p * ctmax + (size_t)(nu * (nu + 1) / 2) * p * p + (size_t)nu * p * ctmax + ctmax;
    return 4 * per_wave * sizeof(double);
}

bool panel_accumulate_fits(int p, int nu, int ctmax) {
    return p * ctmax <= 4 * 256 && (nu * (nu + 1) / 2) * p * p <= 3 * 256 && ctmax <= 256;
}

size_t panel_stage_doubles(int p, int nu, int ctmax) {
    return (size_t)p * ctmax + (size_t)(nu * (nu + 1) / 2) * p * p + (size_t)nu * p * ctmax + ctmax;
}

void launch_panel_accumulate(const PanelParams& P, const int32_t* ecols, int32_t m, int32_t nstream, int32_t nsplit,
                             int32_t chunk, int32_t ctmax, double* partial, double* H, hipStream_t st) {
    if (m == 0) return;
    const size_t lds = ((size_t)chunk + panel_stage_doubles(P.p, P.nu, ctmax)) * sizeof(double);
    MGB_REQUIRE(lds <= PANEL_ACC_LDS_MAX, "coarse-level accumulator + panels exceed the LDS budget");
    MGB_REQUIRE(panel_accumulate_fits(P.p, P.nu, ctmax), "coarse-level panels exceed the register staging of the accumulation kernel");
    static std::once_flag once;
    std::call_once(once, [] {
        (void)hipFuncSetAttribute((const void*)panel_accumulate_kernel, hipFuncAttributeMaxDynamicSharedMemorySize,
                                  (int)PANEL_ACC_LDS_MAX);
        (void)hipGetLastError();
    });
    hipLaunchKernelGGL(panel_accumulate_kernel, dim3((unsigned)nstream, (unsigned)nsplit), dim3(256), lds, st, P, ecols, m,
                       ctmax, chunk, partial);
    hipLaunchKernelGGL(accumulate_reduce_kernel, dim3((unsigned)(((int64_t)m * m + 255) / 256)), dim3(256), 0, st, m,
                       nstream, partial, H);
    MGB_HIP_CHECK(hipGetLastError());
// ... 53 lines not shown
```

multigridbarrier.jl_amd/csrc/kernels.hpp:

```cpp
#pragma once
#include "common.hpp"
#include "cone.hpp"

namespace mgbhip {

enum ElemMode { MODE_F0 = 0, MODE_F1 = 1, MODE_F2 = 2, MODE_NODE_F = 3, MODE_NODE_SLACK = 4,
                MODE_F01 = 5 };

struct LeafDesc {
    int64_t F_off;
    int32_t interior;
    uint32_t packed;
};

struct ElemParams {
    int32_t p, nu, nD, nstage;
    int32_t ymask;
    int64_t N, n;
    const double* ops[MGBHIP_MAX_OPS];
    const double* stage_ptr[MGBHIP_MAX_OPS];
    int32_t D_state[MGBHIP_MAX_ND];
    int32_t D_op[MGBHIP_MAX_ND];
    int32_t D_stage[MGBHIP_MAX_ND];
    const double* w;
    const double* c;
    const double* z0;
    const double* bw;
    double invn;
    ConeDev cone;
    double* out_partial;
    double* out_ret;
    double* out_hel;
    double* out_F;
    double* out_Dz;
    int32_t diag_mask;
    int64_t blk_off[MGBHIP_MAX_NU * (MGBHIP_MAX_NU + 1) / 2];
    double* dn_Dz;
    double* dn_Y;
    const LeafDesc* leaf_desc;
    double* leaf_arena;
    const double* leaf_g;
    int64_t leaf_slack0;
    int32_t* leaf_status;
    int32_t leaf_packed;
    const int32_t* zsel;
    const double* zs;
    double* zout;
    const double* zx;
    double zalpha;
    int32_t wide;
};
static_assert(sizeof(ElemParams) <= 4096 - 64, "ElemParams must stay well inside the kernel argument limit");

bool launch_elem_f2_condense(const ElemParams& P, hipStream_t st);

inline int hel_blocks(int nu) { return nu * (nu + 1) / 2; }
inline int hel_block_index(int a, int b, int nu) { return a * nu - a * (a - 1) / 2 + (b - a); }
inline int64_t hel_layout(int nu, int64_t N, int p, int diag_mask, int64_t* off) {
    int64_t total = 0;
    for (int blk = 0; blk < hel_blocks(nu); ++blk) {
        off[blk] = total;
        total += ((diag_mask >> blk) & 1) ? N * p : N * (int64_t)p * p;
    }
    return total;
}

int elem_group(int p);
constexpr int WIDE_F2_THREADS = 128;
size_t wide_lds_bytes(int p, int nu, int nD, int nstage, int mode);
int64_t elem_grid(int p, int64_t N);
size_t elem_lds_bytes(const ElemParams& P, int mode);
void launch_elem(const ElemParams& P, int mode, hipStream_t st);

void launch_reduce_partials(const double* partials, int64_t count, double* out, hipStream_t st);
void launch_vec_stats(const double* v, int64_t n, double* scratch, double* stats, hipStream_t st, const double* mask = nullptr,
                      const int32_t* ints = nullptr, int nints = 0);
void launch_dir_stats(const double* v, const double* g, int64_t n, double* scratch, double* stats3, hipStream_t st,
                      const double* mask = nullptr, const int32_t* ints = nullptr, int nints = 0);
void launch_dot(const double* a, const double* b, int64_t n, double* scratch, double* out, hipStream_t st, const double* mask = nullptr);
void launch_restrict_trial(int64_t rows, const int32_t* ptr, const int32_t* col, const double* val, const double* ret, double* g,
                            double* scratch, const double* x, const double* nn, double s, double* xn, int32_t* moved, int32_t stamp,
                            hipStream_t st);
void launch_publish(const double* src, int n, double* host_block, int host_lo, double seq, hipStream_t st);
void launch_dir_finish(const double* v, const double* g, int64_t n, double* scratch, double* scal, int32_t* status2, double* host,
                       hipStream_t st, const double* mask = nullptr, double seq = 0.0);
void launch_trial_finish(const double* g, int64_t n, double* scratch, const double* f0_partials, int64_t f0_count, double* scal,
                         int32_t* moved, double* host, hipStream_t st, const double* mask = nullptr, double seq = 0.0,
                         bool partials_ready = false);
void launch_index_gather(const double* v, const int32_t* idx, int64_t cnt, double* out, hipStream_t st);
void launch_index_scatter(const double* in, const int32_t* idx, int64_t cnt, double* v, hipStream_t st);
int64_t reduce_scratch_doubles(int64_t n);

void launch_csr_matvec(int64_t rows, const int32_t* ptr, const int32_t* col, const double* val,
                       const double* x, double* y, bool add, bool long_rows, hipStream_t st);
int csr_chunks(int64_t max_row_len);
void launch_csr_matvec_chunked(int64_t rows, const int32_t* ptr, const int32_t* col, const double* val,
                               const double* x, double* y, double* scratch, int nchunk, hipStream_t st);
void launch_prolong(int64_t rows, const int32_t* ptr, const int32_t* col, const double* val, const double* s,
                    const double* z0, double* zfull, hipStream_t st);
void launch_step(const double* x, const double* n, double s, double* xn, int64_t len, int32_t* moved, int32_t stamp,
                 hipStream_t st);
void launch_scale_copy(const double* src, double alpha, double* dst, int64_t len, hipStream_t st);
void launch_border_tail(const double* g, double* tail, int64_t m, hipStream_t st);
void launch_axpy(double alpha, const double* x, double* y, int64_t len, hipStream_t st);
void launch_fill(double value, double* y, int64_t len, hipStream_t st);

void launch_gather_shared(int64_t nshared, const int32_t* sh_q, const int32_t* cptr, const int32_t* cidx, const double* slab,
                          double* out, hipStream_t st);
void launch_gather_assemble(int64_t nnz, const int32_t* cptr, const int32_t* cidx, const double* slab,
                            double* Hval, bool long_lists, hipStream_t st, int32_t chunk = 0, int32_t nchunk = 0,
                            double* part = nullptr, const int32_t* qmap = nullptr, int64_t nq = 0);

struct PanelParams {
    int32_t p, nu;
    int64_t N;
    const int32_t* ecol_ptr;
    const double* panels;
    const int32_t* eoff;
    const double* hel;
    double* slab;
    int32_t cmax;
    int32_t upper_only;
    const int32_t* spos;
};
bool launch_panel_project_mfma(const PanelParams& P, hipStream_t st);
void launch_invert_lists(const int32_t* cidx, int64_t total, int32_t* spos, hipStream_t st);
void launch_panel_project(const PanelParams& P, hipStream_t st);
constexpr size_t PANEL_ACC_LDS_MAX = 144 * 1024;
size_t panel_accumulate_lds(int p, int nu, int ctmax);
size_t panel_stage_doubles(int p, int nu, int ctmax);
bool panel_accumulate_fits(int p, int nu, int ctmax);
void launch_panel_accumulate(const PanelParams& P, const int32_t* ecols, int32_t m, int32_t nstream, int32_t nsplit,
                             int32_t chunk, int32_t ctmax, double* partial, double* H, hipStream_t st);
void launch_panel_project_staged(const PanelParams& P, int32_t ctmax, hipStream_t st);

}
```

multigridbarrier.jl_amd/csrc/problem.cpp:

```cpp
#include "problem.hpp"
#include "plan_device.hpp"
#include "dense.hpp"

#include <algorithm>
#include <chrono>
#include <cmath>
#include <cstdio>
#include <atomic>
#include <exception>
#include <cstdlib>
#include <string>
#include <thread>
#include <cstring>
#include <numeric>

using namespace mgbhip;

static constexpr int64_t ACC_MAX_M = 384;



static void upload_csr(const mgbhip_csr& R, Level& L, hipStream_t st) {
    MGB_REQUIRE(R.rows >= 0 && R.cols >= 0 && R.rowptr && (R.rowptr[R.rows] == 0 || (R.colidx && R.values)),
                "bad prolongation CSR");
// ... 157 lines not shown
    P->cone.npieces = C.npieces;
    P->cone.feasibility = C.feasibility;
    P->cone.NC = C.NC;
    P->cone.box_b = 1.0;
    P->cone.box_R = 1.0;
    const int ny_piece = C.feasibility ? C.NC - 1 : d->nD;
    if (C.feasibility) MGB_REQUIRE(C.NC >= 2 && C.NC <= d->nD, "phase-I wrapper: bad NC");
    for (int k = 0; k < C.npieces; ++k) {
        const mgbhip_piece& s = C.pieces[k];
        PieceDev& t = P->cone.pc[k];
        MGB_REQUIRE(s.kind == MGBHIP_KIND_EP || s.kind == MGBHIP_KIND_LINEAR, "unknown functor family");
        MGB_REQUIRE(s.ni >= 1 && s.ni <= MGBHIP_MAX_IDX, "functor index list too long for this build (MGBHIP_MAX_IDX)");
        t.kind = s.kind;
        t.ni = s.ni;
        t.nc = (s.kind == MGBHIP_KIND_EP) ? s.ni : s.nc;
        MGB_REQUIRE(t.nc >= 1, "functor constraint count must be positive");
        if (s.kind == MGBHIP_KIND_LINEAR)
            MGB_REQUIRE(s.ni <= MGBHIP_MAX_LIN && t.nc <= MGBHIP_MAX_LIN,
                        "linear piece exceeds MGBHIP_MAX_LIN (4 constraint rows on 4 indexed rows)");
        if (s.kind == MGBHIP_KIND_EP) MGB_REQUIRE(s.ni >= 2, "Euclidean power cone needs nz >= 2");
        for (int c = 0; c < MGBHIP_MAX_IDX; ++c) {
            t.idx[c] = c < s.ni ? s.idx[c] : 0;
            if (c < s.ni) MGB_REQUIRE(s.idx[c] >= 0 && s.idx[c] < ny_piece, "functor index outside the D rows");
        }
        if (!s.A) MGB_REQUIRE(t.nc == t.ni, "identity A needs a square constraint matrix");
        t.A = upload_grid(P.get(), s.A, (size_t)P->n * t.nc * t.ni);
        t.b = upload_grid(P.get(), s.b, (size_t)P->n * t.nc);
        t.p = upload_grid(P.get(), s.p, (size_t)P->n);
        t.mu = upload_grid(P.get(), s.mu, (size_t)P->n);
        t.select = upload_grid(P.get(), s.select, (size_t)P->n);
        t.p_const = s.p_const;
        t.mu_const = s.mu_const;
        if (s.kind == MGBHIP_KIND_EP && !s.p) MGB_REQUIRE(s.p_const >= 1.0, "power cone exponent must be >= 1");
    }
    if (d->barrier_weights) {
        P->bw.upload(d->barrier_weights, (size_t)P->n, st);
        P->has_bw = true;
    }
    if (dbg2) fprintf(stderr, "[mgbhip] problem_create: operators, weights and cone grids on the device after %.3f s\n", since0());
    P->levels.resize(d->L);
    for (int l = 0; l < d->L; ++l) MGB_REQUIRE(d->R[l].rows == (int64_t)P->nu * P->n, "prolongation row count must be nu*n");
    {
        std::vector<std::exception_ptr> errors((size_t)d->L);
        std::atomic<int> next{0};
        auto worker = [&] {
            (void)hipSetDevice(ctx->device);
            for (int l = next.fetch_add(1); l < d->L; l = next.fetch_add(1)) {
                try {
                    const double t0 = since0();
                    upload_csr(d->R[l], P->levels[l], st);
                    if (dbg2) fprintf(stderr, "[mgbhip] problem_create: level %d (nnz %lld) %.3f -> %.3f s\n", l,
                                      (long long)d->R[l].rowptr[d->R[l].rows], t0, since0());
                } catch (...) {
                    errors[(size_t)l] = std::current_exception();
                }
            }
        };
        const int nthreads = std::min(d->L, 8);
        std::vector<std::thread> pool;
        for (int t = 1; t < nthreads; ++t) pool.emplace_back(worker);
        worker();
        for (auto& t : pool) t.join();
        for (const auto& e : errors)
            if (e) std::rethrow_exception(e);
    }
    if (dbg2) fprintf(stderr, "[mgbhip] problem_create: %d levels uploaded after %.3f s\n", d->L, since0());
    int64_t mmax = 1;
    for (auto& L : P->levels) mmax = std::max(mmax, L.m);
    const size_t zn = (size_t)P->nu * P->n;
    P->d_z.alloc(zn);
    P->d_z0.alloc(zn);
    P->d_zfull.alloc(zn);
    P->d_c.alloc((size_t)P->n * P->nD);
    P->d_c0.alloc((size_t)P->n * P->nD);
    P->d_ret.alloc(zn);
    if (P->dense) {
        P->d_dnDz.alloc((size_t)P->n * P->nD);
        P->d_dnY.alloc((size_t)P->n * (P->nD * (P->nD + 1) / 2));
        P->d_hel.alloc(1);
    } else {
        P->hel_cap = (int64_t)P->N * hel_blocks(P->nu) * P->p * P->p;
        P->d_hel.alloc((size_t)P->hel_cap);
    }
    P->d_partials.alloc((size_t)elem_grid(P->p, P->N));
    P->d_scal.alloc(16);
    P->d_scratch.alloc((size_t)reduce_scratch_doubles(std::max<int64_t>(mmax, (int64_t)zn)));
    P->d_nodeF.alloc((size_t)P->n);
    P->d_x.alloc(mmax); P->d_g.alloc(mmax); P->d_nv.alloc(mmax + 1); P->d_xn.alloc(mmax);
    P->d_gn.alloc(mmax); P->d_tmp.alloc(std::max<size_t>(mmax, zn));
    {
        size_t tch = 1;
        for (auto& L : P->levels) tch = std::max(tch, (size_t)L.T_chunks * (size_t)L.m);
        P->d_tchunk.alloc(2 * tch);
    }
    P->d_flag.alloc(4);
    MGB_HIP_CHECK(hipStreamSynchronize(st));
    if (dbg2) fprintf(stderr, "[mgbhip] problem_create: done after %.3f s\n", since0());
    return P.release();
}


void mgbhip_problem::ensure_plan_dense(int level) {
    Level& L = levels[level];
    hipStream_t st = stream();
    const int64_t m = L.m, nn = n;
    MGB_REQUIRE(m * m < (int64_t)INT32_MAX, "dense Hessian exceeds 32-bit indexing");
    L.hHptr.resize(m + 1);
    L.hHcol.resize((size_t)(m * m));
    for (int64_t i = 0; i <= m; ++i) L.hHptr[i] = (int32_t)(i * m);
    for (int64_t i = 0; i < m; ++i)
        for (int64_t j = 0; j < m; ++j) L.hHcol[i * m + j] = (int32_t)j;
    L.nnz = m * m;
    L.Hptr.upload(L.hHptr, st);
    L.Hcol.upload(L.hHcol, st);
    L.Hval.alloc((size_t)(L.nnz + L.m + 1));
    L.selection = false;
    const int64_t ld = (int64_t)nD * nn;
    L.denseDR.alloc((size_t)std::max<int64_t>(ld * m, 1));
    L.denseW.alloc((size_t)std::max<int64_t>(ld * m, 1));
    MGB_HIP_CHECK(hipMemsetAsync(L.denseW.p, 0, sizeof(double) * (size_t)std::max<int64_t>(ld * m, 1), st));
    std::vector<DevBuf<double>> Rd(nu);
    std::vector<double> host((size_t)(nn * m));
    DevBuf<double> opT;
    opT.alloc((size_t)(nn * nn));
    for (int k = 0; k < nD; ++k) {
        const int a = D_state[k];
        if (!Rd[a].p) {
            std::fill(host.begin(), host.end(), 0.0);
            for (int64_t r = 0; r < nn; ++r) {
                const int64_t row = (int64_t)a * nn + r;
                for (int32_t q = L.hRptr[row]; q < L.hRptr[row + 1]; ++q) host[(size_t)(r + nn * L.hRcol[q])] += L.hRval[q];
            }
            Rd[a].upload(host.data(), host.size(), st);
            MGB_HIP_CHECK(hipStreamSynchronize(st));
        }
        double* dst = L.denseDR.p + (int64_t)k * nn;
        const double* op = store->ops[D_op[k]].p;
        if (m == 0) continue;
        if (store->identity[D_op[k]]) {
            MGB_HIP_CHECK(hipMemcpy2DAsync(dst, sizeof(double) * ld, Rd[a].p, sizeof(double) * nn, sizeof(double) * nn,
                                           (size_t)m, hipMemcpyDeviceToDevice, st));
        } else {
            launch_dense_transpose((int)nn, op, opT.p, st);
            launch_dense_gemm_tn((int)nn, (int)m, (int)nn, opT.p, nn, nullptr, Rd[a].p, nn, dst, ld, false, false, st);
        }
    }
    MGB_HIP_CHECK(hipStreamSynchronize(st));
    L.planned = true;
}

void mgbhip_problem::ensure_plan(int level) {
    Level& L = levels[level];
    if (L.planned) return;
    if (dense) { ensure_plan_dense(level); return; }
    const auto t_plan0 = std::chrono::steady_clock::now();
    struct PlanTimer {
        std::chrono::steady_clock::time_point t0; int level;
        ~PlanTimer() {
            if (const char* dbg = getenv("MGBHIP_DEBUG"); dbg && atoi(dbg) >= 2)
                fprintf(stderr, "[mgbhip] assembly plan level %d built in %.2f s\n", level,
                        std::chrono::duration<double>(std::chrono::steady_clock::now() - t0).count());
        }
    } plan_timer{t_plan0, level};
    hipStream_t st = stream();
    const int64_t NE = N;
    const int pp = p;
    const int64_t nn = n;
// ... 367 lines not shown

void mgbhip_problem::eval_f0_launch(int level, const double* d_s, const double* d_zz, const double* d_cc) {
    hipStream_t st = stream();
    StageScope sc(ctx->timers, level + 1 == (int)levels.size() ? "f0" : "f0_coarse");
    ElemParams E = base_params(level, d_s, d_zz, d_cc);
    launch_elem(E, MODE_F0, st);
    launch_reduce_partials(d_partials.p, elem_grid(p, N), d_scal.p, st);
    cnt.f0++;
}

double mgbhip_problem::eval_f0(int level, const double* d_s, const double* d_zz, const double* d_cc) {
    hipStream_t st = stream();
    eval_f0_launch(level, d_s, d_zz, d_cc);
    read_scalars(0, 1);
    if (sharded()) allreduce_host(pin.d, 1, 0);
    return pin.d[0];
}

void mgbhip_problem::allreduce_host(double* h, int64_t count, int op) {
    MGB_REQUIRE(coll_fn != nullptr, "no collective installed");
    if (coll_fn(coll_user, h, count, op, 0) != 0) throw mgbhip::InvalidArgument("the caller's allreduce failed");
}

void mgbhip_problem::allreduce_device(double* d, int64_t count, int op) {
    MGB_REQUIRE(coll_fn != nullptr, "no collective installed");
    hipStream_t st = stream();
    if (coll_device) {
        MGB_HIP_CHECK(hipStreamSynchronize(st));
        if (coll_fn(coll_user, d, count, op, 1) != 0) throw mgbhip::InvalidArgument("the caller's allreduce failed");
        return;
    }
    coll_host.resize((size_t)count);
    MGB_HIP_CHECK(hipMemcpyAsync(coll_host.data(), d, sizeof(double) * (size_t)count, hipMemcpyDeviceToHost, st));
    MGB_HIP_CHECK(hipStreamSynchronize(st));
    allreduce_host(coll_host.data(), count, op);
    MGB_HIP_CHECK(hipMemcpyAsync(d, coll_host.data(), sizeof(double) * (size_t)count, hipMemcpyHostToDevice, st));
    MGB_HIP_CHECK(hipStreamSynchronize(st));
}

void mgbhip_problem::reduce_interface(int level, double* d_g, double* d_part) {
    Level& L = levels[level];
    if (!L.sharded) return;
    hipStream_t st = stream();
    if (d_part) MGB_HIP_CHECK(hipMemcpyAsync(d_part, d_g, sizeof(double) * (size_t)L.m, hipMemcpyDeviceToDevice, st));
    const int64_t ni = (int64_t)L.h_iface.size();
    if (ni == 0) return;
    L.iface_buf.ensure((size_t)ni);
    launch_index_gather(d_g, L.d_iface.p, ni, L.iface_buf.p, st);
    allreduce_device(L.iface_buf.p, ni, 0);
    launch_index_scatter(L.iface_buf.p, L.d_iface.p, ni, d_g, st);
}

void mgbhip_problem::eval_f1(int level, const double* d_s, const double* d_zz, const double* d_cc, double* d_gout, double* d_part) {
    hipStream_t st = stream();
    const Level& L = levels[level];
    {
        StageScope sc(ctx->timers, level + 1 == (int)levels.size() ? "f1" : "f1_coarse");
        ElemParams E = base_params(level, d_s, d_zz, d_cc);
        launch_elem(E, MODE_F1, st);
    }
    {
        StageScope sc(ctx->timers, "restrict");
        if (L.T_chunks > 0)
            launch_csr_matvec_chunked(L.m, L.Tptr.p, L.Tcol.p, L.Tval.p, d_ret.p, d_gout, d_tchunk.p, L.T_chunks, st);
        else
            launch_csr_matvec(L.m, L.Tptr.p, L.Tcol.p, L.Tval.p, d_ret.p, d_gout, false, L.T_long, st);
    }
    if (L.sharded) reduce_interface(level, d_gout, d_part);
    cnt.f1++;
}

void mgbhip_problem::eval_f01_launch(int level, const double* d_s, const double* d_zz, const double* d_cc, double* d_gout,
                                     double* d_part, bool defer_f0_sum) {
    if (dense) {
        eval_f0_launch(level, d_s, d_zz, d_cc);
        eval_f1(level, d_s, d_zz, d_cc, d_gout, d_part);
        return;
    }
    hipStream_t st = stream();
    const Level& L = levels[level];
    {
        StageScope sc(ctx->timers, level + 1 == (int)levels.size() ? "f01" : "f01_coarse");
        ElemParams E = base_params(level, d_s, d_zz, d_cc);
        launch_elem(E, MODE_F01, st);
        if (!defer_f0_sum) launch_reduce_partials(d_partials.p, elem_grid(p, N), d_scal.p, st);
    }
    {
        StageScope sc(ctx->timers, "restrict");
        trial_fuse.done = false;
        if (trial_fuse.want && L.T_chunks == 0 && !L.T_long && !sharded()) {
            launch_restrict_trial(L.m, L.Tptr.p, L.Tcol.p, L.Tval.p, d_ret.p, d_gout, d_scratch.p, trial_fuse.x, trial_fuse.n, trial_fuse.s,
                                  trial_fuse.xn, trial_fuse.moved, trial_fuse.stamp, st);
            trial_fuse.done = true;
        } else if (L.T_chunks > 0)
            launch_csr_matvec_chunked(L.m, L.Tptr.p, L.Tcol.p, L.Tval.p, d_ret.p, d_gout, d_tchunk.p, L.T_chunks, st);
        else
            launch_csr_matvec(L.m, L.Tptr.p, L.Tcol.p, L.Tval.p, d_ret.p, d_gout, false, L.T_long, st);
    }
    if (L.sharded) reduce_interface(level, d_gout, d_part);
    cnt.f0++;
    cnt.f1++;
}

bool mgbhip_problem::try_enable_condensed(int level) {
    Level& L = levels[level];
    static const bool off = [] { const char* e = getenv("MGBHIP_NO_CONDENSE"); return e && e[0] == '1'; }();
    if (off || dense || !L.selection || !L.direct || nu != 2 || p != 7 || L.hRptr.empty()) return false;
    if (!L.solver.analyzed || !L.solver.has_direct_map()) return false;
    const int64_t slack0 = L.m - n;
    if (slack0 < 0 || L.rows != 2 * n) return false;
    std::vector<int32_t> ucol((size_t)n, -1);
    for (int64_t node = 0; node < n; ++node) {
        const int32_t b = L.hRptr[node], e = L.hRptr[node + 1];
        if (e - b > 1) return false;
        if (e - b == 1) ucol[(size_t)node] = L.hRcol[b];
        const int64_t rs = n + node;
        if (L.hRptr[rs + 1] - L.hRptr[rs] != 1 || (int64_t)L.hRcol[L.hRptr[rs]] != slack0 + node) return false;
    }
    const bool ok = L.solver.enable_condensed(N, p, ucol.data(), slack0, L.nnz, hel_cap + L.nshared, stream());
    if (const char* dbg = getenv("MGBHIP_DEBUG"); dbg && atoi(dbg) >= 2)
        fprintf(stderr, "[mgbhip] level %d: condensed leaves %s\n", level, ok ? "enabled" : "not applicable");
    return ok;
}

void mgbhip_problem::eval_f2(int level, const double* d_s, const double* d_zz, const double* d_cc, bool materialize,
                             const double* rhs) {
    ensure_plan(level);
    hipStream_t st = stream();
    Level& L = levels[level];
    int E_ymask = 0;
    if (L.condense && !materialize && rhs != nullptr && L.selection && L.direct && !dense) {
        StageScope sc(ctx->timers, level + 1 == (int)levels.size() ? "f2" : "f2_coarse");
        ElemParams E = base_params(level, d_s, d_zz, d_cc);
        E.leaf_desc = L.solver.leaf_desc();
        E.leaf_arena = L.solver.arena();
        E.leaf_g = rhs;
        E.leaf_slack0 = L.m - n;
        E.leaf_status = L.solver.leaf_status();
        E.leaf_packed = L.solver.leaves_packed() ? 1 : 0;
        if (!L.solver.leaf_flag_zero()) MGB_HIP_CHECK(hipMemsetAsync(E.leaf_status, 0, sizeof(int32_t), st));
        L.solver.leaf_flag_used();
        if (launch_elem_f2_condense(E, st)) {
            L.have_H = true;
            L.H_in_slab = true;
            L.H_condensed = true;
            L.condensed_rhs = rhs;
            hel_level = level;
            L.factored = false;
            cnt.f2++;
            return;
        }
        zf_stamp = -1;
    }
    L.H_condensed = false;
    L.proj_kernel = MGBHIP_PROJ_NONE;
    {
        StageScope sc(ctx->timers, level + 1 == (int)levels.size() ? "f2" : "f2_coarse");
        ElemParams E = base_params(level, d_s, d_zz, d_cc);
        E_ymask = E.ymask;
        E.diag_mask = (L.selection && !dense) ? diag_mask_sel : 0;
        hel_layout(nu, N, p, E.diag_mask, E.blk_off);
        launch_elem(E, MODE_F2, st);
    }
    {
        StageScope sc(ctx->timers, level + 1 == (int)levels.size() ? "assemble" : "assemble_coarse");
        if (dense) {
            int klo = nD, khi = -1;
            for (int k = 0; k < nD; ++k)
                if ((E_ymask >> k) & 1) { klo = std::min(klo, k); khi = std::max(khi, k); }
            const int64_t ld = (int64_t)nD * n;
            if (khi < klo) {
                MGB_HIP_CHECK(hipMemsetAsync(L.Hval.p, 0, sizeof(double) * (size_t)L.nnz, st));
            } else {
                launch_dense_weight(nD, klo, khi, n, L.m, ld, L.denseDR.p, d_dnY.p, L.denseW.p, st);
                launch_dense_gemm_tn((int)L.m, (int)L.m, (int)((khi - klo + 1) * n), L.denseDR.p + (int64_t)klo * n, ld,
// ... 229 lines not shown
```

multigridbarrier.jl_amd/csrc/problem.hpp:

```cpp
#pragma once
#include <mutex>
#include <memory>
#include <string>
#include <vector>

#include "../../include/mgbhip.h"
#include "common.hpp"
#include "kernels.hpp"
#include "mf_solver.hpp"

struct mgbhip_ctx {
    int device = 0;
    hipStream_t stream = nullptr;
    bool own_stream = false;
    mgbhip::StageTimers timers;
    mgbhip::DevBuf<double> vscratch, vscal;
};

struct mgbhip_vec {
    mgbhip_ctx* ctx = nullptr;
    mgbhip::DevBuf<double> buf;
    int64_t len = 0;
};

namespace mgbhip {

struct OpStore {
    std::vector<DevBuf<double>> ops;
    std::vector<bool> identity;
    DevBuf<double> w;
};

struct Level {
    int64_t rows = 0, m = 0;
    std::vector<int32_t> hRptr, hRcol;
    std::vector<double> hRval;
    DevBuf<int32_t> Rptr, Rcol, Tptr, Tcol;
    DevBuf<double> Rval, Tval;
    bool T_long = false, R_long = false;
    int32_t max_row = 0, max_col = 0;
    bool R_unit = false;
    DevBuf<int32_t> Rsel;
    int32_t T_chunks = 0;
    bool planned = false;
    bool selection = false;
    bool acc = false;
    int32_t acc_waves = 0, acc_ctmax = 0;
    int32_t acc_split = 1, acc_chunk = 0;
    DevBuf<double> acc_copies;
    std::vector<int32_t> hHptr, hHcol;
    DevBuf<int32_t> Hptr, Hcol, cptr, cidx, ecol_ptr, ecols, eoff;
    DevBuf<int32_t> spos;
    bool sorted_slab = false;
    DevBuf<double> Hval, panels, slab;
    int64_t slab_doubles = 0;
    int32_t cmax = 1;
    bool long_lists = false;
    int64_t list_total = 0;
    int32_t proj_kernel = 0;
    int32_t gather_chunk = 0, gather_nchunk = 0;
    DevBuf<double> gather_part;
    DevBuf<int32_t> upq;
    int64_t nup = 0;
    int64_t nnz = 0;
    DevBuf<double> denseDR, denseW;
    MfSolver solver;
    bool have_H = false, factored = false;
    bool direct = false;
    int64_t nshared = 0;
    DevBuf<int32_t> sh_q;
    std::vector<int32_t> h_vmap;
    bool H_in_slab = false;
    bool sharded = false;
    std::vector<int32_t> h_iface;
    DevBuf<int32_t> d_iface;
    DevBuf<double> own, iface_buf;
    bool condense_tried = false, condense = false;
    bool H_condensed = false;
    const double* condensed_rhs = nullptr;
    int border_state2 = 0;
    int border_state = 0;
};

struct Counters {
    int64_t f0 = 0, f1 = 0, f2 = 0, factor = 0, newton = 0;
    double solve_seconds = 0;
};

}

struct mgbhip_problem {
    mgbhip_ctx* ctx = nullptr;
    int32_t p = 0, nu = 0, nD = 0;
    int64_t N = 0, n = 0;
    int32_t diag_mask_sel = 0;
    bool dense = false;
    bool wide = false;
    std::shared_ptr<mgbhip::OpStore> store;
    int32_t D_state[MGBHIP_MAX_ND], D_op[MGBHIP_MAX_ND], D_stage[MGBHIP_MAX_ND];
    int32_t nstage = 0;
    const double* stage_ptr[MGBHIP_MAX_OPS];
    mgbhip::ConeDev cone;
    std::vector<mgbhip::DevBuf<double>> cone_grids;
    mgbhip::DevBuf<double> bw;
    bool has_bw = false;
    std::vector<mgbhip::Level> levels;
    std::vector<double> hx;
    int32_t xdim = 0;
    mgbhip::DevBuf<double> d_z, d_z0, d_zfull, d_c, d_ret, d_hel, d_partials, d_scal, d_scratch, d_nodeF, d_nodeDz, d_dnDz, d_dnY, d_tchunk;
    mgbhip::DevBuf<double> d_x, d_g, d_nv, d_xn, d_gn, d_tmp, d_c0;
    mgbhip::DevBuf<int32_t> d_flag;
    int32_t step_stamp = 0;
    mgbhip::PinnedBuf pin;
    mgbhip::Counters cnt;
    int64_t zstamp = 0;
    mutable int64_t zf_stamp = -1;
    mutable int zf_level = -1;
    mutable const double* zf_s = nullptr;
    mutable const double* zf_z = nullptr;
    void touch() { ++zstamp; }
    mgbhip_allreduce_fn coll_fn = nullptr;
    void* coll_user = nullptr;
    bool coll_device = false;
    bool sharded() const { return coll_fn != nullptr; }
    std::vector<double> coll_host;
    void allreduce_host(double* h, int64_t count, int op);
    void allreduce_device(double* d, int64_t count, int op);
    void reduce_interface(int level, double* d_g, double* d_part);
    const double* own_mask(int level) const { return levels[level].sharded ? levels[level].own.p : nullptr; }
    mgbhip::DevBuf<double> d_gpart, d_gnpart;

    mgbhip::ElemParams base_params(int level, const double* d_s, const double* d_zz, const double* d_cc) const;
    hipStream_t stream() const { return ctx->stream; }
    void ensure_plan(int level);
    void ensure_analysis(int level);
    void ensure_direct(int level);
    void prepare_all();
    double next_seq() { return ++result_seq; }
    void wait_results(double seq);
    const double* trial_x = nullptr;
    const double* trial_dir = nullptr;
    double trial_alpha = 0.0;
    bool can_fuse_step(int level) const;
    struct TrialFuse { bool want = false, done = false; const double* x = nullptr; const double* n = nullptr; double s = 0.0;
                       double* xn = nullptr; int32_t* moved = nullptr; int32_t stamp = 0; } trial_fuse;
    void read_scalars(int lo, int n);
    double result_seq = 0.0;
    std::mutex shared_mutex;
    bool prepared = false;
    void ensure_plan_dense(int level);
    double eval_f0(int level, const double* d_s, const double* d_zz, const double* d_cc);
    void eval_f0_launch(int level, const double* d_s, const double* d_zz, const double* d_cc);
    void eval_f1(int level, const double* d_s, const double* d_zz, const double* d_cc, double* d_gout, double* d_part = nullptr);
    void eval_f01_launch(int level, const double* d_s, const double* d_zz, const double* d_cc, double* d_gout, double* d_part = nullptr,
                         bool defer_f0_sum = false);
    void eval_f2(int level, const double* d_s, const double* d_zz, const double* d_cc, bool materialize = true,
                 const double* rhs = nullptr);
    bool try_enable_condensed(int level);
    int64_t hel_cap = 0;
    int hel_level = -1;
    void factor(int level, const double* rhs = nullptr);
    void trisolve(int level, const double* d_g, double* d_xout);
    void trisolve_carried(int level, double* d_xout_np1);
    bool lu_fallback(int level, const double* d_g, double* d_xout);
    mgbhip::DevBuf<double> d_lu;
    mgbhip::DevBuf<int32_t> d_lustat;
    int64_t lu_fallbacks = 0;
};
```

multigridbarrier.jl_amd/device.py:

```python
from __future__ import annotations

import ctypes as C
import os
import weakref
from typing import List, Optional

import numpy as np
import scipy.sparse as sp

from .blockmatrices import BlockColumn, BlockDiag
from .convex import KIND_EP, KIND_LINEAR, Convex
from .multigrid import AMG
from .problem import MGBProblem

MAX_PIECES, MAX_IDX, MAX_ND, MAX_NU, MAX_OPS = 4, 10, 13, 4, 8
MAX_LIN = 4
OK, ERR_INVALID, ERR_HIP, ERR_NOT_SPD, ERR_NONFINITE, ERR_CONVERGENCE = range(6)


class Device:
    """reference: src/device.jl:18"""


class CPUDevice(Device):
    """Marker only: the native CPU path is the reference itself (src/device.jl:25)."""


class HIPDevice(Device):
    """The MI355X backend (the reference's `CUDADevice` slot, src/device.jl:32)."""


_DEFAULT = [HIPDevice]


def default_device():
    return _DEFAULT[0]


def default_device_set(D):
    _DEFAULT[0] = D
    return D



_dp = C.POINTER(C.c_double)
_ip = C.POINTER(C.c_int32)


class _Piece(C.Structure):
    _fields_ = [("kind", C.c_int32), ("ni", C.c_int32), ("nc", C.c_int32), ("idx", C.c_int32 * MAX_IDX),
                ("A", _dp), ("b", _dp), ("p", _dp), ("mu", _dp), ("p_const", C.c_double),
                ("mu_const", C.c_double), ("select", _dp)]


class _Cone(C.Structure):
    _fields_ = [("npieces", C.c_int32), ("pieces", _Piece * MAX_PIECES), ("feasibility", C.c_int32),
                ("NC", C.c_int32)]


class _CSR(C.Structure):
    _fields_ = [("rows", C.c_int64), ("cols", C.c_int64), ("rowptr", _ip), ("colidx", _ip), ("values", _dp)]


class _Desc(C.Structure):
    _fields_ = [("p", C.c_int32), ("N", C.c_int64), ("nu", C.c_int32), ("nD", C.c_int32), ("n_ops", C.c_int32),
                ("ops", _dp * MAX_OPS), ("D_state", C.c_int32 * MAX_ND), ("D_op", C.c_int32 * MAX_ND),
                ("w", _dp), ("L", C.c_int32), ("R", C.POINTER(_CSR)), ("cone", _Cone),
                ("barrier_weights", _dp), ("x", _dp), ("dim", C.c_int32)]


class Options(C.Structure):
    _fields_ = [("tol", C.c_double), ("t", C.c_double), ("kappa", C.c_double), ("maxit", C.c_int32),
                ("max_newton", C.c_int32), ("ls_beta", C.c_double), ("ls_c1", C.c_double),
                ("line_search", C.c_int32), ("stop_lambda_tol", C.c_double), ("stop_theta", C.c_double),
                ("finalize", C.c_int32), ("finalize_theta", C.c_double), ("early_stop", C.c_int32),
                ("stopping_criterion", C.c_void_p), ("early_stop_fn", C.c_void_p), ("user", C.c_void_p)]


STOP_FN = C.CFUNCTYPE(C.c_int, C.c_double, C.c_double, C.c_double, C.c_double, C.c_double, C.c_double, C.c_void_p)
EARLY_FN = C.CFUNCTYPE(C.c_int, C.POINTER(C.c_double), C.c_double, C.c_void_p)
ALLREDUCE_FN = C.CFUNCTYPE(C.c_int, C.c_void_p, C.c_void_p, C.c_int64, C.c_int32, C.c_int32)


class _CoreResult(C.Structure):
    _fields_ = [("k", C.c_int32), ("L", C.c_int32), ("failure_code", C.c_int32), ("t_final", C.c_double),
                ("t_elapsed", C.c_double), ("solve_seconds", C.c_double), ("newton_iterations", C.c_int64),
                ("f0_evals", C.c_int64), ("f1_evals", C.c_int64), ("f2_evals", C.c_int64),
                ("factorizations", C.c_int64), ("cap_steps", C.c_int32), ("its", C.POINTER(C.c_int64)),
                ("ts", _dp), ("kappas", _dp), ("times", _dp), ("c_dot_Dz", _dp)]


EXPORTS = [
    "mgbhip_create", "mgbhip_destroy", "mgbhip_last_error", "mgbhip_version", "mgbhip_problem_create",
    "mgbhip_problem_destroy", "mgbhip_problem_set_box", "mgbhip_problem_set_barrier_weights",
    "mgbhip_level_size", "mgbhip_f0", "mgbhip_f1", "mgbhip_f2", "mgbhip_hessian_pattern", "mgbhip_solve",
    "mgbhip_set_hessian", "mgbhip_solve_newton", "mgbhip_newton_direction", "mgbhip_problem_set_sharding",
    "mgbhip_problem_set_collective",
    "mgbhip_node_barrier", "mgbhip_node_slack", "mgbhip_mgb_core", "mgbhip_matched_t",
    "mgbhip_default_options", "mgbhip_stage_ms", "mgbhip_reset_stage_timers", "mgbhip_solver_stats", "mgbhip_solver_chain",
    "mgbhip_vec_alloc", "mgbhip_vec_free", "mgbhip_vec_len", "mgbhip_vec_upload", "mgbhip_vec_download",
    "mgbhip_vec_fill", "mgbhip_vec_copy", "mgbhip_vec_axpy", "mgbhip_vec_scale", "mgbhip_vec_dot",
    "mgbhip_vec_norm", "mgbhip_vec_isfinite", "mgbhip_f0_d", "mgbhip_f1_d", "mgbhip_f2_d", "mgbhip_solve_d",
    "mgbhip_prolong_add", "mgbhip_level_plan", "mgbhip_solver_launches", "mgbhip_interpolate", "mgbhip_interpolate_grad",
    "mgbhip_locator_create", "mgbhip_locator_elements", "mgbhip_locator_evaluate", "mgbhip_locator_destroy",
    "mgbhip_contour_create", "mgbhip_contour_fetch", "mgbhip_contour_destroy", "mgbhip_contour_create_embedded",
    "mgbhip_tessellate_create", "mgbhip_tessellate_fetch", "mgbhip_tessellate_destroy",
    "mgbhip_raycast_create", "mgbhip_raycast_offsets", "mgbhip_raycast_samples", "mgbhip_raycast_lengths",
    "mgbhip_raycast_integrate", "mgbhip_raycast_render", "mgbhip_raycast_destroy", "mgbhip_raycast_render_layers",
    "mgbhip_surface_create", "mgbhip_surface_trace", "mgbhip_surface_shade", "mgbhip_surface_destroy",
    "mgbhip_stream_create", "mgbhip_stream_set_field", "mgbhip_stream_trace", "mgbhip_stream_destroy",
    "mgbhip_tubes_create", "mgbhip_tubes_trace", "mgbhip_tubes_shade", "mgbhip_tubes_destroy",
    "mgbhip_figure_create", "mgbhip_figure_render", "mgbhip_figure_render_rgba8", "mgbhip_figure_counts",
    "mgbhip_figure_destroy",
]


def library_path() -> str:
    here = os.path.dirname(os.path.abspath(__file__))
    return os.environ.get("MGBHIP_LIB") or os.path.join(here, "lib", "libmgbhip.so")


_LIB = None


def load_library():
    global _LIB
    if _LIB is not None:
        return _LIB
    path = library_path()
    if not os.path.exists(path):
        raise RuntimeError(f"{path} not found: build it with `make -C multigridbarrier.jl_amd/csrc` "
                           "(or __graft_entry__.build()); this package has no CPU fallback")
    lib = C.CDLL(path)
    lib.mgbhip_last_error.restype = C.c_char_p
    lib.mgbhip_version.restype = C.c_char_p
    lib.mgbhip_level_size.restype = C.c_int64
    lib.mgbhip_level_size.argtypes = [C.c_void_p, C.c_int32]
    lib.mgbhip_create.argtypes = [C.POINTER(C.c_void_p), C.c_int, C.c_void_p]
    lib.mgbhip_destroy.argtypes = [C.c_void_p]
    lib.mgbhip_problem_create.argtypes = [C.c_void_p, C.POINTER(_Desc), C.c_void_p, C.POINTER(C.c_void_p)]
    lib.mgbhip_problem_destroy.argtypes = [C.c_void_p]
    lib.mgbhip_problem_set_box.argtypes = [C.c_void_p, C.c_double, C.c_double]
    lib.mgbhip_problem_set_barrier_weights.argtypes = [C.c_void_p, _dp]
    for name in ("mgbhip_f0", "mgbhip_f1", "mgbhip_f2"):
        getattr(lib, name).argtypes = [C.c_void_p, C.c_int32, _dp, _dp, _dp, _dp]
    lib.mgbhip_hessian_pattern.argtypes = [C.c_void_p, C.c_int32, C.POINTER(C.c_int64), C.POINTER(_ip), C.POINTER(_ip)]
    lib.mgbhip_solve.argtypes = [C.c_void_p, C.c_int32, _dp, _dp]
    lib.mgbhip_set_hessian.argtypes = [C.c_void_p, C.c_int32, _dp]
    lib.mgbhip_solve_newton.argtypes = [C.c_void_p, C.c_int32, _dp, _dp, _dp]
    lib.mgbhip_newton_direction.argtypes = [C.c_void_p, C.c_int32, _dp, _dp, _dp, _dp, _dp, _ip]
    lib.mgbhip_problem_set_sharding.argtypes = [C.c_void_p, C.c_int32, C.c_int64, _ip, _dp]
    lib.mgbhip_problem_set_collective.argtypes = [C.c_void_p, C.c_void_p, C.c_void_p, C.c_int32]
    lib.mgbhip_node_barrier.argtypes = [C.c_void_p, _dp, _dp, _dp]
    lib.mgbhip_node_slack.argtypes = [C.c_void_p, _dp, _dp]
    lib.mgbhip_mgb_core.argtypes = [C.c_void_p, _dp, _dp, C.POINTER(Options), C.POINTER(_CoreResult)]
    lib.mgbhip_matched_t.argtypes = [C.c_void_p, _dp, _dp, C.c_double, _dp]
    lib.mgbhip_default_options.argtypes = [C.POINTER(Options), C.c_int64]
    lib.mgbhip_default_options.restype = None
    lib.mgbhip_stage_ms.argtypes = [C.c_void_p, C.c_char_p, _dp, C.POINTER(C.c_int64)]
    lib.mgbhip_reset_stage_timers.argtypes = [C.c_void_p, C.c_int]
    lib.mgbhip_solver_stats.argtypes = [C.c_void_p, C.c_int32, _dp]
    lib.mgbhip_solver_chain.argtypes = [C.c_void_p, C.c_int32, _dp]
    lib.mgbhip_level_plan.argtypes = [C.c_void_p, C.c_int32, _ip]
    lib.mgbhip_solver_launches.argtypes = [C.c_void_p, C.c_int32, _ip, C.c_int64]
    lib.mgbhip_solver_launches.restype = C.c_int64
    vp = C.c_void_p
    lib.mgbhip_vec_alloc.argtypes = [vp, C.c_int64, C.POINTER(vp)]
    lib.mgbhip_vec_free.argtypes = [vp]
    lib.mgbhip_vec_len.argtypes = [vp]
    lib.mgbhip_vec_len.restype = C.c_int64
    lib.mgbhip_vec_upload.argtypes = [vp, _dp, C.c_int64]
    lib.mgbhip_vec_download.argtypes = [vp, _dp, C.c_int64]
    lib.mgbhip_vec_fill.argtypes = [vp, C.c_double]
    lib.mgbhip_vec_copy.argtypes = [vp, vp]
    lib.mgbhip_vec_axpy.argtypes = [C.c_double, vp, vp]
    lib.mgbhip_vec_scale.argtypes = [C.c_double, vp]
    lib.mgbhip_vec_dot.argtypes = [vp, vp, _dp]
    lib.mgbhip_vec_norm.argtypes = [vp, _dp]
    lib.mgbhip_vec_isfinite.argtypes = [vp, C.POINTER(C.c_int32)]
    lib.mgbhip_f0_d.argtypes = [vp, C.c_int32, vp, vp, vp, _dp]
    lib.mgbhip_f1_d.argtypes = [vp, C.c_int32, vp, vp, vp, vp]
    lib.mgbhip_f2_d.argtypes = [vp, C.c_int32, vp, vp, vp]
    lib.mgbhip_solve_d.argtypes = [vp, C.c_int32, vp, vp]
    lib.mgbhip_prolong_add.argtypes = [vp, C.c_int32, vp, vp]
    lib.mgbhip_interpolate.argtypes = [vp, C.c_int32, C.c_int32, C.c_int32, C.c_int32, C.c_int64, _dp, _dp, C.c_int32,
                                       _dp, C.c_int64, _dp, _dp, _ip]
    lib.mgbhip_interpolate_grad.argtypes = [vp, C.c_int32, C.c_int32, C.c_int32, C.c_int32, C.c_int64, _dp, _dp,
                                            C.c_int32, _dp, C.c_int64, _dp, _dp, _dp, _ip]
    lib.mgbhip_locator_create.argtypes = [vp, C.c_int32, C.c_int32, C.c_int32, C.c_int32, C.c_int64, _dp, _dp, C.c_int64,
                                          _dp, C.POINTER(vp)]
    lib.mgbhip_locator_elements.argtypes = [vp, _ip]
    lib.mgbhip_locator_evaluate.argtypes = [vp, C.c_int32, _dp, _dp, _dp]
    lib.mgbhip_locator_destroy.argtypes = [vp]
    lib.mgbhip_contour_create.argtypes = [vp, C.c_int32, C.c_int32, C.c_int32, C.c_int32, C.c_int64, _dp, _dp, C.c_int32,
                                          _dp, C.c_int32, _dp, C.c_int32, C.POINTER(vp), C.POINTER(C.c_int64)]
    lib.mgbhip_contour_create_embedded.argtypes = [vp, C.c_int32, C.c_int32, C.c_int32, C.c_int32, C.c_int32, C.c_int64, _dp,
                                                   _dp, C.c_int32, _dp, C.c_int32, _dp, C.c_int32, C.POINTER(vp),
                                                   C.POINTER(C.c_int64)]
    lib.mgbhip_tessellate_create.argtypes = [vp, C.c_int32, C.c_int32, C.c_int32, C.c_int32, C.c_int32, C.c_int64, _dp, _dp,
                                             C.c_int32, _dp, C.c_int32, C.POINTER(vp), C.POINTER(C.c_int64)]
    lib.mgbhip_tessellate_fetch.argtypes = [vp, _dp, _ip, _dp]
    lib.mgbhip_tessellate_destroy.argtypes = [vp]
    lib.mgbhip_contour_fetch.argtypes = [vp, _dp, _ip, _ip, _dp]
    lib.mgbhip_contour_destroy.argtypes = [vp]
    lib.mgbhip_raycast_create.argtypes = [vp, C.c_int32, C.c_int32, C.c_int32, C.c_int32, C.c_int64, _dp, _dp, C.c_int64,
                                          _dp, _dp, _dp, C.c_double, C.c_double, C.c_double, C.POINTER(vp),
                                          C.POINTER(C.c_int64)]
    lib.mgbhip_raycast_offsets.argtypes = [vp, C.POINTER(C.c_int64)]
    lib.mgbhip_raycast_samples.argtypes = [vp, _dp]
    lib.mgbhip_raycast_lengths.argtypes = [vp, _dp, _dp]
    lib.mgbhip_raycast_integrate.argtypes = [vp, C.c_int32, _dp, _dp]
    lib.mgbhip_raycast_render.argtypes = [vp, _dp, C.c_int32, _dp, C.c_double, C.c_double, _dp]
    lib.mgbhip_raycast_destroy.argtypes = [vp]
    lib.mgbhip_raycast_render_layers.argtypes = [vp, _dp, C.c_int32, _dp, C.c_double, C.c_double, C.c_int32, _dp, _dp, _dp]
    lib.mgbhip_surface_create.argtypes = [vp, C.c_int64, _dp, C.POINTER(vp)]
    lib.mgbhip_surface_trace.argtypes = [vp, C.c_int64, _dp, _dp, C.c_double, C.c_double, C.c_int32, _dp, _ip, _dp, _dp]
    lib.mgbhip_surface_shade.argtypes = [vp, C.c_int64, C.c_int32, _dp, _ip, _dp, _dp, _dp, C.c_int32, _dp, C.c_double,
                                         C.c_double, C.c_double, _dp]
    lib.mgbhip_surface_destroy.argtypes = [vp]
    lib.mgbhip_tubes_create.argtypes = [vp, C.c_int64, _dp, _dp, C.POINTER(vp)]
    lib.mgbhip_tubes_trace.argtypes = [vp, C.c_int64, _dp, _dp, C.c_double, C.c_double, C.c_int32, _dp, _ip, _dp]
    lib.mgbhip_tubes_shade.argtypes = [vp, C.c_int64, C.c_int32, _dp, _dp, _dp, _ip, _dp, _dp, C.c_int32, _dp, C.c_double,
                                       C.c_double, C.c_double, _dp]
    lib.mgbhip_tubes_destroy.argtypes = [vp]
    lib.mgbhip_stream_create.argtypes = [vp, C.c_int32, C.c_int32, C.c_int32, C.c_int32, C.c_int64, _dp, _dp, C.c_int32, _dp,
                                         C.POINTER(vp)]
    lib.mgbhip_stream_set_field.argtypes = [vp, _dp]
    lib.mgbhip_stream_trace.argtypes = [vp, C.c_int64, _dp, C.c_double, C.c_int32, C.c_int32, C.c_double, _dp, _ip, _ip]
    lib.mgbhip_stream_destroy.argtypes = [vp]
    lib.mgbhip_figure_create.argtypes = [vp, C.c_int32, C.c_int32, C.c_int32, C.c_int32, C.c_int64, _dp, _dp, C.c_int64,
                                         _dp, _dp, _dp, C.c_double, C.c_int32, C.c_int32, _dp, C.c_int32, _ip, _dp,
                                         C.c_int32, _dp, _dp, C.c_double, C.c_double, C.c_double, C.c_int32,
                                         C.POINTER(vp)]
    lib.mgbhip_figure_render.argtypes = [vp, _dp, _dp]
    lib.mgbhip_figure_render_rgba8.argtypes = [vp, _dp, _dp, C.POINTER(C.c_uint8)]
    lib.mgbhip_figure_counts.argtypes = [vp, C.POINTER(C.c_int64), C.POINTER(C.c_int64)]
    lib.mgbhip_figure_destroy.argtypes = [vp]
    _LIB = lib
    return lib


class MGBHipError(RuntimeError):
    def __init__(self, status, message):
# ... 299 lines not shown

    def solve_newton(self, level: int, g, check: bool = True):
        g = _f64(g)
        x = np.empty_like(g)
        lam = C.c_double()
        status = self.lib.mgbhip_solve_newton(self.handle, level, _ptr(g), _ptr(x), C.cast(C.byref(lam), _dp))
        if check:
            _check(self.lib, status)
        return x, lam.value, status

    def newton_direction(self, level: int, s, c, z0):
        s, c, z0 = _f64(s), np.asfortranarray(c, dtype=np.float64), _f64(z0)
        x = np.empty(self.level_sizes[level])
        lam, cond = C.c_double(), C.c_int32()
        _check(self.lib, self.lib.mgbhip_newton_direction(self.handle, level, _ptr(s), _ptr(c), _ptr(z0), _ptr(x),
                                                          C.cast(C.byref(lam), _dp), C.byref(cond)))
        return x, lam.value, bool(cond.value)

    def node_barrier(self, z, want_Dz: bool = False):
        z = _f64(z)
        F = np.empty(self.n)
        Dz = np.empty((self.n, self.nD), order="F") if want_Dz else None
        _check(self.lib, self.lib.mgbhip_node_barrier(self.handle, _ptr(z), _ptr(F), _ptr(Dz)))
        return (F, Dz) if want_Dz else F

    def node_slack(self, z) -> np.ndarray:
        z = _f64(z)
        out = np.empty(self.n)
        _check(self.lib, self.lib.mgbhip_node_slack(self.handle, _ptr(z), _ptr(out)))
        return out

    def set_sharding(self, shards, collective, accepts_device_ptr: bool = False):
        for level, sh in enumerate(shards):
            ic = np.ascontiguousarray(sh.iface, dtype=np.int32)
            own = _f64(sh.own)
            _check(self.lib, self.lib.mgbhip_problem_set_sharding(self.handle, level, ic.size, ic.ctypes.data_as(_ip), _ptr(own)))
        self._collective = collective
        _check(self.lib, self.lib.mgbhip_problem_set_collective(self.handle, C.cast(collective, C.c_void_p), None,
                                                               1 if accepts_device_ptr else 0))

    def set_box(self, b: float, R: float):
        _check(self.lib, self.lib.mgbhip_problem_set_box(self.handle, float(b), float(R)))

    def set_barrier_weights(self, bw):
        a = None if bw is None else _f64(bw)
        _check(self.lib, self.lib.mgbhip_problem_set_barrier_weights(self.handle, _ptr(a)))

    def default_options(self, n_nodes: Optional[int] = None) -> Options:
        o = Options()
        self.lib.mgbhip_default_options(C.byref(o), int(self.n if n_nodes is None else n_nodes))
        return o

    def mgb_core(self, z, c, opt: Options, cap_steps: int = 256):
        z = _f64(z).copy()
        c = np.asfortranarray(c, dtype=np.float64)
        L = len(self.level_sizes)
        its = np.zeros((L, cap_steps), dtype=np.int64, order="F")
        ts, kappas, times, cdz = (np.zeros(cap_steps) for _ in range(4))
        r = _CoreResult()
        r.cap_steps = cap_steps
        r.its = its.ctypes.data_as(C.POINTER(C.c_int64))
        r.ts, r.kappas, r.times, r.c_dot_Dz = _ptr(ts), _ptr(kappas), _ptr(times), _ptr(cdz)
        status = self.lib.mgbhip_mgb_core(self.handle, _ptr(z), _ptr(c), C.byref(opt), C.byref(r))
        if status not in (OK, ERR_CONVERGENCE):
            _check(self.lib, status)
        k = min(r.k, cap_steps)
        diag = dict(its=its[:, :k].copy(), ts=ts[:k].copy(), kappas=kappas[:k].copy(), times=times[:k].copy(),
                    c_dot_Dz=cdz[:k].copy(), t_elapsed=r.t_elapsed, t_final=r.t_final,
                    solve_seconds=r.solve_seconds, newton_iterations=int(r.newton_iterations),
                    f0_evals=int(r.f0_evals), f1_evals=int(r.f1_evals), f2_evals=int(r.f2_evals),
                    factorizations=int(r.factorizations), failure_code=int(r.failure_code), k=int(r.k))
        return status, z, diag

    def matched_t(self, z, c, t_default: float) -> float:
        z = _f64(z)
        c = np.asfortranarray(c, dtype=np.float64)
        out = C.c_double()
        _check(self.lib, self.lib.mgbhip_matched_t(self.handle, _ptr(z), _ptr(c), float(t_default), C.cast(C.byref(out), _dp)))
        return out.value

    def reset_stage_timers(self, enable: bool = True):
        _check(self.lib, self.lib.mgbhip_reset_stage_timers(self.handle, 1 if enable else 0))

    def stage_ms(self, stage: str):
        ms, cnt = C.c_double(), C.c_int64()
        _check(self.lib, self.lib.mgbhip_stage_ms(self.handle, stage.encode(), C.cast(C.byref(ms), _dp), C.byref(cnt)))
        return ms.value, cnt.value

    def solver_stats(self, level: int) -> dict:
        out = np.zeros(8)
        _check(self.lib, self.lib.mgbhip_solver_stats(self.handle, level, _ptr(out)))
        keys = ("fronts", "max_front", "arena_doubles", "factor_flops", "peeled", "tree_levels", "nnz", "unknowns")
        return dict(zip(keys, out.tolist()))

    def solver_chain(self, level: int) -> dict:
        out = np.zeros(8)
        _check(self.lib, self.lib.mgbhip_solver_chain(self.handle, level, _ptr(out)))
        keys = ("pivot_blocks_on_critical_path", "large_front_tree_levels", "launches_per_factorization",
                "launches_per_backward_sweep", "arena_doubles", "factor_flops", "extra_trailing_doubles", "reserved")
        return dict(zip(keys, out.tolist()))

    PLAN_KEYS = ("R_unit", "R_long", "T_long", "T_chunks", "selection", "acc", "acc_split", "long_lists", "gather_chunk",
                 "gather_nchunk", "projection", "max_row", "max_col", "cmax", "mean_list", "planned")
    PROJECTION = ("none", "loop", "staged", "mfma", "accumulate")

    def level_plan(self, level: int) -> dict:
        out = (C.c_int32 * 16)()
        _check(self.lib, self.lib.mgbhip_level_plan(self.handle, level, out))
        d = dict(zip(self.PLAN_KEYS, (int(v) for v in out)))
        d["projection"] = self.PROJECTION[d["projection"]]
        d["direct"] = bool(d["selection"] & 2)
        d["selection"] = bool(d["selection"] & 1)
        for k in ("R_unit", "R_long", "T_long", "acc", "long_lists", "planned"):
            d[k] = bool(d[k])
        return d

    LAUNCH_KEYS = ("level", "first", "count", "cls", "max_m", "max_k", "max_child", "tiny", "wave", "inv", "iface", "packed",
                   "assembly", "block0", "backward")
    ASSEMBLY = ("none", "gather", "columns")
    BLOCK0 = ("n/a", "gather", "diag0", "step0")
    BACKWARD = ("n/a", "k8", "k16", "general")

    @classmethod
    def launch_rows(cls, raw) -> list:
        rows = []
        for r in np.asarray(raw, dtype=np.int64).reshape(-1, 16):
            d = dict(zip(cls.LAUNCH_KEYS, (int(v) for v in r)))
            for k in ("tiny", "wave", "inv", "iface", "packed"):
                d[k] = bool(d[k])
            d["assembly"], d["block0"], d["backward"] = cls.ASSEMBLY[d["assembly"]], cls.BLOCK0[d["block0"]], cls.BACKWARD[d["backward"]]
            rows.append(d)
        return rows

    def solver_launches(self, level: int) -> list:
        n = self.lib.mgbhip_solver_launches(self.handle, level, None, 0)
        if n < 0:
            _check(self.lib, int(-n))
        out = (C.c_int32 * (16 * max(int(n), 1)))()
        n = self.lib.mgbhip_solver_launches(self.handle, level, out, n)
        if n < 0:
            _check(self.lib, int(-n))
        return self.launch_rows(np.frombuffer(out, dtype=np.int32)[:16 * int(n)])

    def close(self):
        if self.handle:
            self.lib.mgbhip_problem_destroy(self.handle)
            self.handle = None

    def __del__(self):
        try:
            self.close()
        except Exception:
            pass


def dense_as_block(M: AMG) -> AMG:
    if isinstance(M.D_fine[0], BlockColumn):
        return M
    n = M.w.size
    geom = M.geometry
    ops = {k: BlockDiag(np.asarray(v, dtype=np.float64).reshape(n, n, 1)) for k, v in geom.operators.items()}
    from dataclasses import replace
    g2 = replace(geom, operators=ops)
    nu = len(M.state_names)
    D_fine = [BlockColumn(ops[name], state, nu) for (state, name) in M.D_spec]
    return AMG(geometry=g2, x=M.x, w=M.w, R_fine=M.R_fine, D_fine=D_fine, state_names=M.state_names, D_spec=M.D_spec)
# ... 47 lines not shown
```

Baseline: 676.5.

## Screen backtracking line-search candidates in the same f0 evaluation launch

Each line-search trial now also evaluates the barrier objective at the next few backtracked step sizes inside the same element kernel, whether the step is applied on the fly or through a candidate prolongation kernel. Per-candidate partial sums and moved flags are reduced alongside the main trial. A new host-side walk then skips trials already known to fail the Armijo test, with deferred re-evaluation so the final state stays consistent. This cuts the number of sequential trial launches and host round trips per rejected step, at the cost of extra per-trial arithmetic, registers and shared-memory reductions in the f01 kernel.

```diff
diff --git a/include/mgbhip.h b/include/mgbhip.h
--- a/include/mgbhip.h
+++ b/include/mgbhip.h
@@ -170,6 +170,9 @@
 
 int mgbhip_stage_ms(mgbhip_problem* prob, const char* stage, double* total_ms, int64_t* launches);
 int mgbhip_reset_stage_timers(mgbhip_problem* prob, int enable);
+int mgbhip_problem_set_ls_screen(mgbhip_problem* prob, int32_t levels);
+int mgbhip_ls_trial(mgbhip_problem* prob, int32_t level, const double* x, const double* dir, const double* c, const double* z0,
+                    double s, double beta, double* out14);
 int mgbhip_solver_stats(mgbhip_problem* prob, int32_t level, double* out8);
 int mgbhip_solver_chain(mgbhip_problem* prob, int32_t level, double* out8);
 enum { MGBHIP_PROJ_NONE = 0, MGBHIP_PROJ_LOOP = 1, MGBHIP_PROJ_STAGED = 2, MGBHIP_PROJ_MFMA = 3, MGBHIP_PROJ_ACCUMULATE = 4 };
diff --git a/multigridbarrier.jl_amd/csrc/api.cpp b/multigridbarrier.jl_amd/csrc/api.cpp
--- a/multigridbarrier.jl_amd/csrc/api.cpp
+++ b/multigridbarrier.jl_amd/csrc/api.cpp
@@ -20,6 +20,7 @@
 mgbhip_problem* problem_create(mgbhip_ctx* ctx, const mgbhip_problem_desc* d, mgbhip_problem* share);
 int core_run(mgbhip_problem* P, double* z, const double* c, const mgbhip_options* opt, mgbhip_core_result* res);
 int matched_t_run(mgbhip_problem* P, const double* z, const double* c, double t_default, double* t_out);
+void ls_trial_run(mgbhip_problem* P, int level, double s, double beta, double* out14);
 
 #ifdef MGB_STEP_PROBE
 namespace mgbhip { void mf_debug_probe(long long* out64); }
@@ -662,6 +663,15 @@
 int mgbhip_stage_ms(mgbhip_problem* P, const char* stage, double* total_ms, int64_t* launches) {
     MGB_API_BEGIN_ON(P)
     MGB_REQUIRE(P && stage, "null argument");
+    const std::string name(stage);
+    const int64_t* counter = name == "ls_trial" ? &P->cnt.ls_trial[0] : name == "ls_trial_coarse" ? &P->cnt.ls_trial[1]
+                           : name == "ls_screen" ? &P->cnt.ls_screen[0] : name == "ls_screen_coarse" ? &P->cnt.ls_screen[1]
+                           : name == "ls_reject2" ? &P->cnt.ls_reject2[0] : name == "ls_reject2_coarse" ? &P->cnt.ls_reject2[1] : nullptr;
+    if (counter) {
+        if (total_ms) *total_ms = 0.0;
+        if (launches) *launches = *counter;
+        return MGBHIP_OK;
+    }
     P->ctx->timers.collect();
     auto it = P->ctx->timers.recs.find(stage);
     if (total_ms) *total_ms = it == P->ctx->timers.recs.end() ? 0.0 : it->second.ms;
@@ -725,6 +735,28 @@
     MGB_API_BEGIN_ON(P)
     MGB_REQUIRE(P, "null argument");
     P->ctx->timers.reset(enable != 0);
+    for (int i = 0; i < 2; ++i) P->cnt.ls_trial[i] = P->cnt.ls_screen[i] = P->cnt.ls_reject2[i] = 0;
+    return MGBHIP_OK;
+    MGB_API_END
+}
+
+int mgbhip_ls_trial(mgbhip_problem* P, int32_t level, const double* x, const double* dir, const double* c, const double* z0,
+                    double s, double beta, double* out) {
+    MGB_API_BEGIN_ON(P)
+    check_level(P, level);
+    MGB_REQUIRE(x && dir && c && z0 && out, "null argument");
+    stage_inputs(P, level, x, c, z0);
+    P->d_nv.upload(dir, (size_t)P->levels[level].m, P->stream());
+    ls_trial_run(P, level, s, beta, out);
+    return MGBHIP_OK;
+    MGB_API_END
+}
+
+int mgbhip_problem_set_ls_screen(mgbhip_problem* P, int32_t levels) {
+    MGB_API_BEGIN
+    MGB_REQUIRE(P, "null argument");
+    MGB_REQUIRE(levels <= 3, "mgbhip_problem_set_ls_screen: levels is a mask of bit 0 (finest level) and bit 1 (coarse levels)");
+    P->ls_screen_levels = levels < 0 ? mgbhip_problem::LS_SCREEN_DEFAULT : levels;
     return MGBHIP_OK;
     MGB_API_END
 }
diff --git a/multigridbarrier.jl_amd/csrc/driver.cpp b/multigridbarrier.jl_amd/csrc/driver.cpp
--- a/multigridbarrier.jl_amd/csrc/driver.cpp
+++ b/multigridbarrier.jl_amd/csrc/driver.cpp
@@ -7,12 +7,14 @@
 #include <limits>
 
 #include "problem.hpp"
+#include "ls_walk.hpp"
 
 using namespace mgbhip;
 
 namespace {
 
 constexpr double EPS = std::numeric_limits<double>::epsilon();
+static_assert(LS_SCREEN_T - 1 <= LS_WALK_MAX_CAND, "ls_walk.hpp has no room for the candidates of a screening launch");
 
 bool debug_on() {
     static const bool on = [] { const char* e = getenv("MGBHIP_DEBUG"); return e && e[0] == '1'; }();
@@ -69,13 +71,23 @@
     void F2(const double* d_s) { P->eval_f2(level, d_s, d_zJ, d_c, false, rhs_of_g()); }
 };
 
-bool trial_values(NewtonCtx& C, double& ynext, double& gnorm_next, int32_t* moved = nullptr, const double* step = nullptr) {
+bool trial_values(NewtonCtx& C, double& ynext, double& gnorm_next, int32_t* moved = nullptr, const double* step = nullptr,
+                  LsTrial* scr = nullptr) {
     mgbhip_problem* P = C.P;
     hipStream_t st = P->stream();
+    const int lev01 = C.level + 1 == (int)P->levels.size() ? 0 : 1;
+    P->cnt.ls_trial[lev01]++;
+    P->trial_screen = mgbhip_problem::TrialScreen();
+    if (step && scr && scr->ncand == LS_SCREEN_T - 1 && !P->dense && !P->sharded() && P->screens(C.level)) {
+        P->trial_screen.n = scr->ncand;
+        for (int t = 0; t < scr->ncand; ++t) P->trial_screen.s[t] = scr->cand_f0[t];
+        P->trial_screen.x = P->d_x.p; P->trial_screen.dir = P->d_nv.p;
+    }
+    const int nscr = P->trial_screen.n;
     const bool onfly = step && P->can_fuse_step(C.level);
     if (step) {
         ++P->step_stamp;
-        if (!onfly) launch_step(P->d_x.p, P->d_nv.p, *step, P->d_xn.p, C.m, P->d_flag.p, P->step_stamp, st);
+        if (!onfly) launch_step(P->d_x.p, P->d_nv.p, *step, P->d_xn.p, C.m, P->d_flag.p, P->step_stamp, st, nscr, P->trial_screen.s);
         P->touch();
         if (onfly) { P->trial_x = P->d_x.p; P->trial_dir = P->d_nv.p; P->trial_alpha = *step; }
     }
@@ -92,14 +104,24 @@
     P->eval_f01_launch(C.level, P->d_xn.p, C.d_zJ, C.d_c, P->d_gn.p, P->sharded() ? P->d_gnpart.p : nullptr, fused);
     const bool restrict_fused = P->trial_fuse.done;
     P->trial_fuse.want = false;
+    const int ncand = P->trial_screen.done ? nscr : 0;
+    P->trial_screen.n = 0;
     if (onfly) {
         P->trial_x = nullptr; P->trial_dir = nullptr;
-        if (!restrict_fused) launch_step(P->d_x.p, P->d_nv.p, *step, P->d_xn.p, C.m, P->d_flag.p, P->step_stamp, st);
+        if (!restrict_fused) launch_step(P->d_x.p, P->d_nv.p, *step, P->d_xn.p, C.m, P->d_flag.p, P->step_stamp, st, ncand, P->trial_screen.s);
     }
     const double seq = P->next_seq();
     launch_trial_finish(P->d_gn.p, C.m, P->d_scratch.p, fused ? P->d_partials.p : nullptr, elem_grid(P->p, P->N), P->d_scal.p,
-                        P->d_flag.p, P->pin.dev, st, P->own_mask(C.level), seq, restrict_fused);
+                        P->d_flag.p, P->pin.dev, st, P->own_mask(C.level), seq, restrict_fused, ncand, elem_grid(P->p, P->N));
     P->wait_results(seq);
+    if (scr) {
+        scr->ncand = ncand;
+        for (int t = 0; t < ncand; ++t) {
+            scr->cand_f0[t] = P->pin.d[8 + t];
+            scr->cand_moved[t] = P->pin.d[5 + t] == (double)P->step_stamp;
+        }
+    }
+    if (ncand > 0) P->cnt.ls_screen[lev01]++;
     P->pin.i[0] = P->pin.d[4] == (double)P->step_stamp ? 1 : 0;
     if (P->sharded()) {
         P->pin.d[1] = (double)P->pin.i[0];
@@ -117,21 +139,19 @@
 bool linesearch_backtracking(NewtonCtx& C, const mgbhip_options& opt, double y, double inc, double& ynext,
                              double& gnorm_next) {
     mgbhip_problem* P = C.P;
-    hipStream_t st = P->stream();
-    double s = 1.0;
-    bool have = false;
-    while (s > 0.0) {
-        double yn, gn;
+    const int ncand_max = (!P->dense && !P->sharded() && P->screens(C.level)) ? LS_SCREEN_T - 1 : 0;
+    auto trial = [&](double s, const double* cand_s, int ncand) {
+        LsTrial t;
+        t.ncand = ncand;
+        for (int i = 0; i < ncand; ++i) t.cand_f0[i] = cand_s[i];
         int32_t moved = 0;
-        if (trial_values(C, yn, gn, &moved, &s)) {
-            have = true;
-            ynext = yn;
-            gnorm_next = gn;
-            const bool stalled = (moved == 0);
-            if (stalled || yn <= y - opt.ls_c1 * inc * s) return true;
-        }
-        s *= opt.ls_beta;
-    }
+        t.ok = trial_values(C, t.y, t.gnorm, &moved, &s, &t);
+        t.moved = moved != 0;
+        return t;
+    };
+    int rejected = 0;
+    const bool have = ls_backtracking_walk(trial, ncand_max, opt.ls_beta, opt.ls_c1, y, inc, ynext, gnorm_next, &rejected);
+    if (rejected >= 2) P->cnt.ls_reject2[C.level + 1 == (int)P->levels.size() ? 0 : 1]++;
     return have;
 }
 
@@ -178,6 +198,23 @@
     }
     return have;
 }
+
+}
+
+void ls_trial_run(mgbhip_problem* P, int level, double s, double beta, double* out) {
+    NewtonCtx C{P, level, P->d_z0.p, P->d_c.p, P->levels[level].m};
+    LsTrial t;
+    for (double sc = s * beta; t.ncand < LS_SCREEN_T - 1; sc *= beta) t.cand_f0[t.ncand++] = sc;
+    double steps[LS_SCREEN_T - 1];
+    for (int i = 0; i < t.ncand; ++i) steps[i] = t.cand_f0[i];
+    int32_t moved = 0;
+    t.ok = trial_values(C, t.y, t.gnorm, &moved, &s, &t);
+    for (int i = 0; i < 14; ++i) out[i] = 0.0;
+    out[0] = t.ok ? 1.0 : 0.0; out[1] = t.y; out[2] = t.ok ? t.gnorm : 0.0; out[3] = moved != 0 ? 1.0 : 0.0; out[4] = t.ncand;
+    for (int i = 0; i < t.ncand; ++i) { out[5 + i] = steps[i]; out[8 + i] = t.cand_f0[i]; out[11 + i] = t.cand_moved[i] ? 1.0 : 0.0; }
+}
+
+namespace {
 
 NewtonResult newton(NewtonCtx& C, const mgbhip_options& opt, const Stop& stop, int maxit) {
     mgbhip_problem* P = C.P;
diff --git a/multigridbarrier.jl_amd/csrc/kernels.hip b/multigridbarrier.jl_amd/csrc/kernels.hip
--- a/multigridbarrier.jl_amd/csrc/kernels.hip
+++ b/multigridbarrier.jl_amd/csrc/kernels.hip
@@ -767,7 +767,7 @@
     }
 }
 
-template <int NY, int P, class Sig>
+template <int NY, int P, class Sig, int T = 1>
 __global__ __launch_bounds__(256) void elem_f01_fast(const ElemParams Pm) {
     constexpr int G = (P <= 2) ? 2 : (P <= 4) ? 4 : (P <= 8) ? 8 : (P <= 16) ? 16 : (P <= 32) ? 32 : 64;
     constexpr int EPB = 256 / G;
@@ -810,8 +810,36 @@
     }
     double ck[NY];
     double wv = 0.0, bwv = 0.0;
+    double zc[T > 1 ? T - 1 : 1][MGBHIP_MAX_NU];
     if (active) {
-        for (int a = 0; a < nu; ++a) zl[(el * nu + a) * G + r] = z_at(Pm, (int64_t)a * n + node);
+        if constexpr (T == 1) {
+            for (int a = 0; a < nu; ++a) zl[(el * nu + a) * G + r] = z_at(Pm, (int64_t)a * n + node);
+        } else {
+#pragma unroll
+            for (int a = 0; a < MGBHIP_MAX_NU; ++a) {
+                if (a >= nu) continue;
+                const int64_t i = (int64_t)a * n + node;
+                if (Pm.zsel) {
+                    const double z0v = Pm.z0[i];
+                    const int32_t c = Pm.zsel[i];
+                    const double xs = c >= 0 ? Pm.zs[c] : 0.0, xd = c >= 0 ? Pm.zx[c] : 0.0;
+                    double v = z0v;
+                    if (c >= 0) v += __builtin_fma(-Pm.zalpha, xd, xs);
+                    if (Pm.zout) Pm.zout[i] = v;
+                    zl[(el * nu + a) * G + r] = v;
+#pragma unroll
+                    for (int t = 0; t < T - 1; ++t) {
+                        double vc = z0v;
+                        if (c >= 0) vc += __builtin_fma(-Pm.cand_alpha[t], xd, xs);
+                        zc[t][a] = vc;
+                    }
+                } else {
+                    zl[(el * nu + a) * G + r] = Pm.z0[i];
+#pragma unroll
+                    for (int t = 0; t < T - 1; ++t) zc[t][a] = Pm.cand_z[t][i];
+                }
+            }
+        }
 #pragma unroll
         for (int k = 0; k < NY; ++k) ck[k] = Pm.c[node + n * k];
         wv = Pm.w[node];
@@ -868,9 +896,54 @@
             Pm.out_ret[(int64_t)a * n + node] = acc;
         }
     }
+    double valc[T > 1 ? T - 1 : 1];
+    if constexpr (T > 1) {
+#pragma unroll
+        for (int t = 0; t < T - 1; ++t) {
+            if (t > 0) __syncthreads();
+            if (active) {
+#pragma unroll
+                for (int a = 0; a < MGBHIP_MAX_NU; ++a)
+                    if (a < nu) zl[(el * nu + a) * G + r] = zc[t][a];
+            }
+            __syncthreads();
+            double yc[NY];
+#pragma unroll
+            for (int k = 0; k < NY; ++k) {
+                double v = 0.0;
+                if (active) {
+                    const double* za = zl + (el * nu + DST(k)) * G;
+                    if (DSG(k) < 0) v = za[r];
+                    else {
+#pragma unroll
+                        for (int cc = 0; cc < P; ++cc) v += OP(k, r, cc) * za[cc];
+                    }
+                }
+                yc[k] = v;
+            }
+            double vc = 0.0;
+            if (active) {
+                double F0v, g[NY], H[NY * NY];
+                cone_eval<NY, 0>(Pm.cone, node, n, yc, F0v, g, H);
+                const double bar = Pm.bw ? ((bwv == 0.0) ? 0.0 : bwv * F0v) : Pm.invn * F0v;
+                double lin = 0.0;
+#pragma unroll
+                for (int k = 0; k < NY; ++k) lin += ck[k] * yc[k];
+                vc = bar + wv * lin;
+            }
+            valc[t] = vc;
+        }
+    }
     __syncthreads();
     const double tot = block_sum_256(val, sh);
     if (tid == 0) Pm.out_partial[blockIdx.x] = tot;
+    if constexpr (T > 1) {
+#pragma unroll
+        for (int t = 0; t < T - 1; ++t) {
+            const double totc = block_sum_256(valc[t], sh + 4 * (t + 1));
+            if (tid == 0) Pm.out_partial[(int64_t)(t + 1) * Pm.cand_stride + blockIdx.x] = totc;
+        }
+    }
 }
 
 struct DSum {
@@ -941,19 +1014,24 @@
     }
 }
 
+struct StepCands { int32_t n; double s[LS_SCREEN_T - 1]; };
 __global__ __launch_bounds__(256) void restrict_trial_kernel(int64_t rows, const int32_t* __restrict__ ptr, const int32_t* __restrict__ col,
                                                              const double* __restrict__ val, const double* __restrict__ ret,
                                                              double* __restrict__ g, double* __restrict__ partials,
                                                              const double* __restrict__ x, const double* __restrict__ nn, double s,
-                                                             double* __restrict__ xn, int32_t* __restrict__ moved, int32_t stamp) {
+                                                             double* __restrict__ xn, int32_t* __restrict__ moved, int32_t stamp,
+                                                             const StepCands cand) {
     __shared__ double red[256];
     __shared__ double red2[256];
     __shared__ int any_moved;
+    __shared__ int cand_moved[LS_SCREEN_T - 1];
     const int tid = threadIdx.x;
     if (tid == 0) any_moved = 0;
+    if (tid < LS_SCREEN_T - 1) cand_moved[tid] = 0;
     __syncthreads();
     double ss = 0.0, bad = 0.0;
     bool m = false;
+    bool mc[LS_SCREEN_T - 1] = {};
     for (int64_t i = (int64_t)blockIdx.x * 256 + tid; i < rows; i += (int64_t)gridDim.x * 256) {
         double acc = 0.0;
         for (int32_t q = ptr[i]; q < ptr[i + 1]; ++q) acc += val[q] * ret[col[q]];
@@ -965,11 +1043,17 @@
             const double v = __builtin_fma(-s, nn[i], xi);
             xn[i] = v;
             m = m || (v != xi);
+#pragma unroll
+            for (int t = 0; t < LS_SCREEN_T - 1; ++t)
+                if (t < cand.n) mc[t] = mc[t] || (__builtin_fma(-cand.s[t], nn[i], xi) != xi);
         }
     }
     red[tid] = ss;
     red2[tid] = bad;
     if (m) any_moved = 1;
+#pragma unroll
+    for (int t = 0; t < LS_SCREEN_T - 1; ++t)
+        if (mc[t]) cand_moved[t] = 1;
     __syncthreads();
     for (int off = 128; off > 0; off >>= 1) {
         if (tid < off) { red[tid] += red[tid + off]; red2[tid] += red2[tid + off]; }
@@ -979,6 +1063,8 @@
         partials[blockIdx.x] = red[0];
         partials[gridDim.x + blockIdx.x] = red2[0];
         if (any_moved) *moved = stamp;
+        for (int t = 0; t < cand.n; ++t)
+            if (cand_moved[t]) moved[1 + t] = stamp;
     }
 }
 
@@ -1013,7 +1099,7 @@
 
 struct FinishJob { const double* src; int64_t count; int32_t out; };
 struct FinishParams {
-    FinishJob job[4];
+    FinishJob job[3 + LS_SCREEN_T];
     int32_t njobs;
     double* out;
     int32_t* ints;
@@ -1142,9 +1228,29 @@
     zfull[i] = v;
 }
 
+struct ProlongCands { int32_t n; double s[LS_SCREEN_T - 1]; double* z[LS_SCREEN_T - 1]; };
+__global__ __launch_bounds__(256) void prolong_cands_kernel(int64_t rows, const int32_t* __restrict__ ptr,
+                                                            const int32_t* __restrict__ col, const double* __restrict__ val,
+                                                            const double* __restrict__ x, const double* __restrict__ nn,
+                                                            const double* __restrict__ z0, const ProlongCands cand) {
+    const int64_t i = (int64_t)blockIdx.x * 256 + threadIdx.x;
+    if (i >= rows) return;
+    double v[LS_SCREEN_T - 1];
+#pragma unroll
+    for (int t = 0; t < LS_SCREEN_T - 1; ++t) v[t] = z0[i];
+    for (int32_t q = ptr[i]; q < ptr[i + 1]; ++q) {
+        const double a = val[q], xc = x[col[q]], nc = nn[col[q]];
+#pragma unroll
+        for (int t = 0; t < LS_SCREEN_T - 1; ++t) v[t] += a * __builtin_fma(-cand.s[t], nc, xc);
+    }
+#pragma unroll
+    for (int t = 0; t < LS_SCREEN_T - 1; ++t)
+        if (t < cand.n) cand.z[t][i] = v[t];
+}
+
 __global__ __launch_bounds__(256) void step_kernel(const double* __restrict__ x, const double* __restrict__ nn,
                                                    double s, double* __restrict__ xn, int64_t len,
-                                                   int32_t* __restrict__ moved, int32_t stamp) {
+                                                   int32_t* __restrict__ moved, int32_t stamp, const StepCands cand) {
     const int64_t i = (int64_t)blockIdx.x * 256 + threadIdx.x;
     bool m = false;
     if (i < len) {
@@ -1152,6 +1258,20 @@
         const double v = __builtin_fma(-s, nn[i], xi);
         xn[i] = v;
         m = (v != xi);
+    }
+    if (cand.n > 0) {
+        __shared__ int cand_moved[LS_SCREEN_T - 1];
+        if (threadIdx.x < LS_SCREEN_T - 1) cand_moved[threadIdx.x] = 0;
+        __syncthreads();
+        if (i < len) {
+            const double xi = x[i], ni = nn[i];
+            for (int t = 0; t < cand.n; ++t)
+                if (__builtin_fma(-cand.s[t], ni, xi) != xi) cand_moved[t] = 1;
+        }
+        __syncthreads();
+        if (threadIdx.x == 0)
+            for (int t = 0; t < cand.n; ++t)
+                if (cand_moved[t]) moved[1 + t] = stamp;
     }
     __shared__ int any_moved;
     if (threadIdx.x == 0) any_moved = 0;
@@ -1754,27 +1874,49 @@
 }
 
 template <int NY, int PN>
-static bool try_f01_fast(const ElemParams& P, hipStream_t st) {
-    if (P.nD != NY || P.p != PN) return false;
+static size_t f01_fast_lds(const ElemParams& P) {
+    if (P.nD != NY || P.p != PN) return 0;
     for (int k = 0; k < NY; ++k)
-        if (P.D_stage[k] == -2) return false;
+        if (P.D_stage[k] == -2) return 0;
     const int G = elem_group(PN);
     const int EPB = 256 / G;
     size_t lds = (256 * (size_t)P.nu + (size_t)P.nstage * EPB * PN * PN + (size_t)EPB * NY * G) * sizeof(double);
     if (lds < 256 * sizeof(double)) lds = 256 * sizeof(double);
-    if (lds > 160 * 1024) return false;
+    return lds > 160 * 1024 ? 0 : lds;
+}
+
+template <int NY, int PN>
+static bool try_f01_fast(const ElemParams& P, hipStream_t st) {
+    const size_t lds = f01_fast_lds<NY, PN>(P);
+    if (lds == 0) return false;
     static bool attr = [] {
         (void)hipFuncSetAttribute((const void*)elem_f01_fast<NY, PN, SigRuntime>, hipFuncAttributeMaxDynamicSharedMemorySize, 160 * 1024);
         (void)hipFuncSetAttribute((const void*)elem_f01_fast<NY, PN, SigDefault<NY>>, hipFuncAttributeMaxDynamicSharedMemorySize, 160 * 1024);
+        (void)hipFuncSetAttribute((const void*)elem_f01_fast<NY, PN, SigRuntime, LS_SCREEN_T>, hipFuncAttributeMaxDynamicSharedMemorySize, 160 * 1024);
+        (void)hipFuncSetAttribute((const void*)elem_f01_fast<NY, PN, SigDefault<NY>, LS_SCREEN_T>, hipFuncAttributeMaxDynamicSharedMemorySize, 160 * 1024);
         (void)hipGetLastError();
         return true;
     }();
     (void)attr;
-    if (is_default_signature<NY>(P))
-        hipLaunchKernelGGL((elem_f01_fast<NY, PN, SigDefault<NY>>), dim3((unsigned)elem_grid(PN, P.N)), dim3(256), lds, st, P);
+    const dim3 grid((unsigned)elem_grid(PN, P.N));
+    if (P.ncand > 0) {
+        MGB_REQUIRE(P.ncand == LS_SCREEN_T - 1 && P.cand_stride >= (int64_t)grid.x, "screening trial: candidate arguments");
+        MGB_REQUIRE(P.zsel ? (P.zx != nullptr) : (P.cand_z[0] != nullptr), "screening trial: candidate points missing");
+        if (is_default_signature<NY>(P))
+            hipLaunchKernelGGL((elem_f01_fast<NY, PN, SigDefault<NY>, LS_SCREEN_T>), grid, dim3(256), lds, st, P);
+        else
+            hipLaunchKernelGGL((elem_f01_fast<NY, PN, SigRuntime, LS_SCREEN_T>), grid, dim3(256), lds, st, P);
+    } else if (is_default_signature<NY>(P))
+        hipLaunchKernelGGL((elem_f01_fast<NY, PN, SigDefault<NY>>), grid, dim3(256), lds, st, P);
     else
-        hipLaunchKernelGGL((elem_f01_fast<NY, PN, SigRuntime>), dim3((unsigned)elem_grid(PN, P.N)), dim3(256), lds, st, P);
+        hipLaunchKernelGGL((elem_f01_fast<NY, PN, SigRuntime>), grid, dim3(256), lds, st, P);
     return true;
+}
+
+bool elem_f01_can_screen(const ElemParams& P) {
+    if (P.p > 64 || P.wide || P.nD > 10) return false;
+    return f01_fast_lds<4, 7>(P) || f01_fast_lds<3, 2>(P) || f01_fast_lds<5, 8>(P) || f01_fast_lds<4, 6>(P) ||
+           f01_fast_lds<7, 7>(P) || f01_fast_lds<6, 2>(P) || f01_fast_lds<8, 8>(P) || f01_fast_lds<7, 6>(P);
 }
 
 size_t wide_lds_bytes(int p, int nu, int nD, int nstage, int mode) {
@@ -1847,6 +1989,7 @@
             MGB_HIP_CHECK(hipGetLastError());
             return;
         }
+        MGB_REQUIRE(P.ncand == 0, "screening trial: no specialised trial kernel for this discretisation");
     }
     static std::once_flag once;
     std::call_once(once, [] {
@@ -1973,7 +2116,9 @@
 }
 
 void launch_trial_finish(const double* g, int64_t n, double* scratch, const double* f0_partials, int64_t f0_count, double* scal,
-                         int32_t* moved, double* host, hipStream_t st, const double* mask, double seq, bool partials_ready) {
+                         int32_t* moved, double* host, hipStream_t st, const double* mask, double seq, bool partials_ready,
+                         int ncand, int64_t cand_stride) {
+    MGB_REQUIRE(ncand >= 0 && ncand <= LS_SCREEN_T - 1 && (ncand == 0 || f0_partials != nullptr), "trial finish: candidate count");
     const int nb = reduce_blocks(n);
     if (!partials_ready) hipLaunchKernelGGL(block_reduce_kernel<1>, dim3(nb), dim3(256), 0, st, g, (const double*)nullptr, n, scratch, mask);
     FinishParams F{};
@@ -1981,10 +2126,11 @@
     if (f0_partials) F.job[nj++] = FinishJob{f0_partials, f0_count, 0};
     F.job[nj++] = FinishJob{scratch, nb, 2};
     F.job[nj++] = FinishJob{scratch + nb, nb, 3};
+    for (int t = 0; t < ncand; ++t) F.job[nj++] = FinishJob{f0_partials + (int64_t)(t + 1) * cand_stride, f0_count, 8 + t};
     F.njobs = nj;
     F.out = scal;
-    F.ints = moved; F.nints = 1; F.ints_out = 4; F.reset = 0;
-    F.host = host; F.host_lo = 0; F.host_n = 5;
+    F.ints = moved; F.nints = 1 + ncand; F.ints_out = 4; F.reset = 0;
+    F.host = host; F.host_lo = 0; F.host_n = ncand > 0 ? 8 + ncand : 5;
     F.seq = seq;
     launch_finish(F, st);
 }
@@ -2016,12 +2162,21 @@
 
 int csr_chunks(int64_t max_row_len) { return (int)((max_row_len + CHUNK - 1) / CHUNK); }
 
+static StepCands step_cands(int ncand, const double* cand_s) {
+    MGB_REQUIRE(ncand >= 0 && ncand <= LS_SCREEN_T - 1 && (ncand == 0 || cand_s != nullptr), "line-search step: candidate count");
+    StepCands c{};
+    c.n = ncand;
+    for (int t = 0; t < ncand; ++t) c.s[t] = cand_s[t];
+    return c;
+}
+
 void launch_restrict_trial(int64_t rows, const int32_t* ptr, const int32_t* col, const double* val, const double* ret, double* g,
                             double* scratch, const double* x, const double* nn, double s, double* xn, int32_t* moved, int32_t stamp,
-                            hipStream_t st) {
+                            hipStream_t st, int ncand, const double* cand_s) {
     if (rows == 0) return;
     const int nb = reduce_blocks(rows);
-    hipLaunchKernelGGL(restrict_trial_kernel, dim3(nb), dim3(256), 0, st, rows, ptr, col, val, ret, g, scratch, x, nn, s, xn, moved, stamp);
+    const StepCands cand = step_cands(xn ? ncand : 0, cand_s);
+    hipLaunchKernelGGL(restrict_trial_kernel, dim3(nb), dim3(256), 0, st, rows, ptr, col, val, ret, g, scratch, x, nn, s, xn, moved, stamp, cand);
     MGB_HIP_CHECK(hipGetLastError());
 }
 
@@ -2044,9 +2199,21 @@
 }
 
 void launch_step(const double* x, const double* n, double s, double* xn, int64_t len, int32_t* moved, int32_t stamp,
-                 hipStream_t st) {
+                 hipStream_t st, int ncand, const double* cand_s) {
     if (len == 0) return;
-    hipLaunchKernelGGL(step_kernel, dim3((unsigned)((len + 255) / 256)), dim3(256), 0, st, x, n, s, xn, len, moved, stamp);
+    hipLaunchKernelGGL(step_kernel, dim3((unsigned)((len + 255) / 256)), dim3(256), 0, st, x, n, s, xn, len, moved, stamp,
+                       step_cands(ncand, cand_s));
+    MGB_HIP_CHECK(hipGetLastError());
+}
+
+void launch_prolong_cands(int64_t rows, const int32_t* ptr, const int32_t* col, const double* val, const double* x, const double* n,
+                          const double* z0, int ncand, const double* cand_s, double* const* zcand, hipStream_t st) {
+    if (rows == 0 || ncand == 0) return;
+    MGB_REQUIRE(ncand > 0 && ncand <= LS_SCREEN_T - 1 && cand_s && zcand, "prolong candidates: candidate count");
+    ProlongCands c{};
+    c.n = ncand;
+    for (int t = 0; t < ncand; ++t) { c.s[t] = cand_s[t]; c.z[t] = zcand[t]; }
+    hipLaunchKernelGGL(prolong_cands_kernel, dim3((unsigned)((rows + 255) / 256)), dim3(256), 0, st, rows, ptr, col, val, x, n, z0, c);
     MGB_HIP_CHECK(hipGetLastError());
 }
 
diff --git a/multigridbarrier.jl_amd/csrc/kernels.hpp b/multigridbarrier.jl_amd/csrc/kernels.hpp
--- a/multigridbarrier.jl_amd/csrc/kernels.hpp
+++ b/multigridbarrier.jl_amd/csrc/kernels.hpp
@@ -12,6 +12,8 @@
     int32_t interior;
     uint32_t packed;
 };
+
+constexpr int LS_SCREEN_T = 2;
 
 struct ElemParams {
     int32_t p, nu, nD, nstage;
@@ -49,6 +51,10 @@
     const double* zx;
     double zalpha;
     int32_t wide;
+    int32_t ncand;
+    double cand_alpha[LS_SCREEN_T - 1];
+    const double* cand_z[LS_SCREEN_T - 1];
+    int64_t cand_stride;
 };
 static_assert(sizeof(ElemParams) <= 4096 - 64, "ElemParams must stay well inside the kernel argument limit");
 
@@ -71,6 +77,7 @@
 int64_t elem_grid(int p, int64_t N);
 size_t elem_lds_bytes(const ElemParams& P, int mode);
 void launch_elem(const ElemParams& P, int mode, hipStream_t st);
+bool elem_f01_can_screen(const ElemParams& P);
 
 void launch_reduce_partials(const double* partials, int64_t count, double* out, hipStream_t st);
 void launch_vec_stats(const double* v, int64_t n, double* scratch, double* stats, hipStream_t st, const double* mask = nullptr,
@@ -80,13 +87,13 @@
 void launch_dot(const double* a, const double* b, int64_t n, double* scratch, double* out, hipStream_t st, const double* mask = nullptr);
 void launch_restrict_trial(int64_t rows, const int32_t* ptr, const int32_t* col, const double* val, const double* ret, double* g,
                             double* scratch, const double* x, const double* nn, double s, double* xn, int32_t* moved, int32_t stamp,
-                            hipStream_t st);
+                            hipStream_t st, int ncand = 0, const double* cand_s = nullptr);
 void launch_publish(const double* src, int n, double* host_block, int host_lo, double seq, hipStream_t st);
 void launch_dir_finish(const double* v, const double* g, int64_t n, double* scratch, double* scal, int32_t* status2, double* host,
                        hipStream_t st, const double* mask = nullptr, double seq = 0.0);
 void launch_trial_finish(const double* g, int64_t n, double* scratch, const double* f0_partials, int64_t f0_count, double* scal,
                          int32_t* moved, double* host, hipStream_t st, const double* mask = nullptr, double seq = 0.0,
-                         bool partials_ready = false);
+                         bool partials_ready = false, int ncand = 0, int64_t cand_stride = 0);
 void launch_index_gather(const double* v, const int32_t* idx, int64_t cnt, double* out, hipStream_t st);
 void launch_index_scatter(const double* in, const int32_t* idx, int64_t cnt, double* v, hipStream_t st);
 int64_t reduce_scratch_doubles(int64_t n);
@@ -99,7 +106,9 @@
 void launch_prolong(int64_t rows, const int32_t* ptr, const int32_t* col, const double* val, const double* s,
                     const double* z0, double* zfull, hipStream_t st);
 void launch_step(const double* x, const double* n, double s, double* xn, int64_t len, int32_t* moved, int32_t stamp,
-                 hipStream_t st);
+                 hipStream_t st, int ncand = 0, const double* cand_s = nullptr);
+void launch_prolong_cands(int64_t rows, const int32_t* ptr, const int32_t* col, const double* val, const double* x, const double* n,
+                          const double* z0, int ncand, const double* cand_s, double* const* zcand, hipStream_t st);
 void launch_scale_copy(const double* src, double alpha, double* dst, int64_t len, hipStream_t st);
 void launch_border_tail(const double* g, double* tail, int64_t m, hipStream_t st);
 void launch_axpy(double alpha, const double* x, double* y, int64_t len, hipStream_t st);
diff --git a/multigridbarrier.jl_amd/csrc/ls_walk.hpp b/multigridbarrier.jl_amd/csrc/ls_walk.hpp
--- /dev/null
+++ b/multigridbarrier.jl_amd/csrc/ls_walk.hpp
@@ -0,0 +1,72 @@
+#pragma once
+#include <cmath>
+#include <vector>
+
+namespace mgbhip {
+
+constexpr int LS_WALK_MAX_CAND = 3;
+
+struct LsTrial {
+    bool ok = false;
+    double y = 0.0, gnorm = 0.0;
+    bool moved = false;
+    int ncand = 0;
+    double cand_f0[LS_WALK_MAX_CAND] = {0.0, 0.0, 0.0};
+    bool cand_moved[LS_WALK_MAX_CAND] = {false, false, false};
+};
+
+inline bool ls_known_rejected(double f0, bool moved, double s, double y, double inc, double c1) {
+    return moved && (!std::isfinite(f0) || !(f0 <= y - c1 * inc * s));
+}
+
+template <class Trial>
+bool ls_backtracking_walk(Trial&& trial, int ncand_max, double beta, double c1, double y, double inc, double& ynext,
+                          double& gnorm_next, int* nrejected = nullptr) {
+    int rejected_here = 0;
+    int& rejected = nrejected ? *nrejected : rejected_here;
+    rejected = 0;
+    double s = 1.0;
+    bool have = false;
+    std::vector<double> skipped;
+    double last_launched = 0.0, last_step = 0.0;
+    while (s > 0.0) {
+        double cs[LS_WALK_MAX_CAND];
+        int nc = 0;
+        for (double sc = s * beta; nc < ncand_max && nc < LS_WALK_MAX_CAND && sc > 0.0; sc *= beta) cs[nc++] = sc;
+        const LsTrial t = trial(s, cs, nc);
+        last_launched = last_step = s;
+        if (t.ok) {
+            have = true;
+            ynext = t.y;
+            gnorm_next = t.gnorm;
+            skipped.clear();
+            const bool stalled = !t.moved;
+            if (stalled || t.y <= y - c1 * inc * s) return true;
+        }
+        ++rejected;
+        s *= beta;
+        for (int i = 0; i < t.ncand && s > 0.0; ++i) {
+            if (!ls_known_rejected(t.cand_f0[i], t.cand_moved[i], s, y, inc, c1)) break;
+            if (std::isfinite(t.cand_f0[i])) skipped.push_back(s);
+            last_step = s;
+            ++rejected;
+            s *= beta;
+        }
+    }
+    while (!skipped.empty()) {
+        const double sk = skipped.back();
+        skipped.pop_back();
+        const LsTrial t = trial(sk, nullptr, 0);
+        last_launched = sk;
+        if (t.ok) {
+            have = true;
+            ynext = t.y;
+            gnorm_next = t.gnorm;
+            break;
+        }
+    }
+    if (last_launched != last_step) (void)trial(last_step, nullptr, 0);
+    return have;
+}
+
+}
diff --git a/multigridbarrier.jl_amd/csrc/problem.cpp b/multigridbarrier.jl_amd/csrc/problem.cpp
--- a/multigridbarrier.jl_amd/csrc/problem.cpp
+++ b/multigridbarrier.jl_amd/csrc/problem.cpp
@@ -263,7 +263,8 @@
         P->hel_cap = (int64_t)P->N * hel_blocks(P->nu) * P->p * P->p;
         P->d_hel.alloc((size_t)P->hel_cap);
     }
-    P->d_partials.alloc((size_t)elem_grid(P->p, P->N));
+    P->d_partials.alloc((size_t)LS_SCREEN_T * (size_t)elem_grid(P->p, P->N));
+    if (const char* e = getenv("MGBHIP_NO_LS_SCREEN"); e && e[0] == '1') P->ls_screen_levels = 0;
     P->d_scal.alloc(16);
     P->d_scratch.alloc((size_t)reduce_scratch_doubles(std::max<int64_t>(mmax, (int64_t)zn)));
     P->d_nodeF.alloc((size_t)P->n);
@@ -797,6 +798,25 @@
     {
         StageScope sc(ctx->timers, level + 1 == (int)levels.size() ? "f01" : "f01_coarse");
         ElemParams E = base_params(level, d_s, d_zz, d_cc);
+        trial_screen.done = false;
+        if (trial_screen.n > 0 && defer_f0_sum && !sharded() && elem_f01_can_screen(E)) {
+            const bool onfly = E.zsel != nullptr && E.zx != nullptr;
+            const bool prolonged = E.zsel == nullptr && E.z0 == d_zfull.p && !L.R_long;
+            if (onfly || prolonged) {
+                E.ncand = trial_screen.n;
+                E.cand_stride = elem_grid(p, N);
+                for (int t = 0; t < trial_screen.n; ++t) E.cand_alpha[t] = trial_screen.s[t];
+                if (prolonged) {
+                    const size_t zn = (size_t)nu * (size_t)n;
+                    d_zcand.ensure((size_t)trial_screen.n * zn);
+                    double* zc[LS_SCREEN_T - 1];
+                    for (int t = 0; t < trial_screen.n; ++t) { zc[t] = d_zcand.p + (size_t)t * zn; E.cand_z[t] = zc[t]; }
+                    launch_prolong_cands(L.rows, L.Rptr.p, L.Rcol.p, L.Rval.p, trial_screen.x, trial_screen.dir, d_zz, trial_screen.n,
+                                         trial_screen.s, zc, st);
+                }
+                trial_screen.done = true;
+            }
+        }
         launch_elem(E, MODE_F01, st);
         if (!defer_f0_sum) launch_reduce_partials(d_partials.p, elem_grid(p, N), d_scal.p, st);
     }
@@ -805,7 +825,7 @@
         trial_fuse.done = false;
         if (trial_fuse.want && L.T_chunks == 0 && !L.T_long && !sharded()) {
             launch_restrict_trial(L.m, L.Tptr.p, L.Tcol.p, L.Tval.p, d_ret.p, d_gout, d_scratch.p, trial_fuse.x, trial_fuse.n, trial_fuse.s,
-                                  trial_fuse.xn, trial_fuse.moved, trial_fuse.stamp, st);
+                                  trial_fuse.xn, trial_fuse.moved, trial_fuse.stamp, st, trial_screen.done ? trial_screen.n : 0, trial_screen.s);
             trial_fuse.done = true;
         } else if (L.T_chunks > 0)
             launch_csr_matvec_chunked(L.m, L.Tptr.p, L.Tcol.p, L.Tval.p, d_ret.p, d_gout, d_tchunk.p, L.T_chunks, st);
diff --git a/multigridbarrier.jl_amd/csrc/problem.hpp b/multigridbarrier.jl_amd/csrc/problem.hpp
--- a/multigridbarrier.jl_amd/csrc/problem.hpp
+++ b/multigridbarrier.jl_amd/csrc/problem.hpp
@@ -84,6 +84,7 @@
 
 struct Counters {
     int64_t f0 = 0, f1 = 0, f2 = 0, factor = 0, newton = 0;
+    int64_t ls_trial[2] = {0, 0}, ls_screen[2] = {0, 0}, ls_reject2[2] = {0, 0};
     double solve_seconds = 0;
 };
 
@@ -144,6 +145,12 @@
     bool can_fuse_step(int level) const;
     struct TrialFuse { bool want = false, done = false; const double* x = nullptr; const double* n = nullptr; double s = 0.0;
                        double* xn = nullptr; int32_t* moved = nullptr; int32_t stamp = 0; } trial_fuse;
+    struct TrialScreen { int n = 0; bool done = false; double s[mgbhip::LS_SCREEN_T - 1] = {}; const double* x = nullptr;
+                         const double* dir = nullptr; } trial_screen;
+    mgbhip::DevBuf<double> d_zcand;
+    int32_t ls_screen_levels = LS_SCREEN_DEFAULT;
+    static constexpr int32_t LS_SCREEN_DEFAULT = 3;
+    bool screens(int level) const { return (ls_screen_levels >> (level + 1 == (int)levels.size() ? 0 : 1)) & 1; }
     void read_scalars(int lo, int n);
     double result_seq = 0.0;
     std::mutex shared_mutex;
diff --git a/multigridbarrier.jl_amd/device.py b/multigridbarrier.jl_amd/device.py
--- a/multigridbarrier.jl_amd/device.py
+++ b/multigridbarrier.jl_amd/device.py
@@ -97,7 +97,7 @@
     "mgbhip_set_hessian", "mgbhip_solve_newton", "mgbhip_newton_direction", "mgbhip_problem_set_sharding",
     "mgbhip_problem_set_collective",
     "mgbhip_node_barrier", "mgbhip_node_slack", "mgbhip_mgb_core", "mgbhip_matched_t",
-    "mgbhip_default_options", "mgbhip_stage_ms", "mgbhip_reset_stage_timers", "mgbhip_solver_stats", "mgbhip_solver_chain",
+    "mgbhip_default_options", "mgbhip_stage_ms", "mgbhip_reset_stage_timers", "mgbhip_problem_set_ls_screen", "mgbhip_ls_trial", "mgbhip_solver_stats", "mgbhip_solver_chain",
     "mgbhip_vec_alloc", "mgbhip_vec_free", "mgbhip_vec_len", "mgbhip_vec_upload", "mgbhip_vec_download",
     "mgbhip_vec_fill", "mgbhip_vec_copy", "mgbhip_vec_axpy", "mgbhip_vec_scale", "mgbhip_vec_dot",
     "mgbhip_vec_norm", "mgbhip_vec_isfinite", "mgbhip_f0_d", "mgbhip_f1_d", "mgbhip_f2_d", "mgbhip_solve_d",
@@ -159,6 +159,8 @@
     lib.mgbhip_default_options.restype = None
     lib.mgbhip_stage_ms.argtypes = [C.c_void_p, C.c_char_p, _dp, C.POINTER(C.c_int64)]
     lib.mgbhip_reset_stage_timers.argtypes = [C.c_void_p, C.c_int]
+    lib.mgbhip_problem_set_ls_screen.argtypes = [C.c_void_p, C.c_int32]
+    lib.mgbhip_ls_trial.argtypes = [C.c_void_p, C.c_int32, _dp, _dp, _dp, _dp, C.c_double, C.c_double, _dp]
     lib.mgbhip_solver_stats.argtypes = [C.c_void_p, C.c_int32, _dp]
     lib.mgbhip_solver_chain.argtypes = [C.c_void_p, C.c_int32, _dp]
     lib.mgbhip_level_plan.argtypes = [C.c_void_p, C.c_int32, _ip]
@@ -624,6 +626,18 @@
     def reset_stage_timers(self, enable: bool = True):
         _check(self.lib, self.lib.mgbhip_reset_stage_timers(self.handle, 1 if enable else 0))
 
+    def set_ls_screen(self, levels: int = -1):
+        _check(self.lib, self.lib.mgbhip_problem_set_ls_screen(self.handle, int(levels)))
+
+    def ls_trial(self, level: int, x, direction, c, z0, s: float, beta: float) -> dict:
+        out = np.zeros(14)
+        c = np.asfortranarray(c, dtype=np.float64)
+        _check(self.lib, self.lib.mgbhip_ls_trial(self.handle, level, _ptr(_f64(x)), _ptr(_f64(direction)), _ptr(c), _ptr(_f64(z0)),
+                                                  float(s), float(beta), _ptr(out)))
+        k = int(out[4])
+        return dict(ok=bool(out[0]), value=out[1], gnorm=out[2], moved=bool(out[3]), steps=out[5:5 + k].copy(),
+                    cand_f0=out[8:8 + k].copy(), cand_moved=out[11:11 + k] != 0)
+
     def stage_ms(self, stage: str):
         ms, cnt = C.c_double(), C.c_int64()
         _check(self.lib, self.lib.mgbhip_stage_ms(self.handle, stage.encode(), C.cast(C.byref(ms), _dp), C.byref(cnt)))
```

Result: no change. 677.6 (median of 2 runs) (+0.2%).
